# dleeim/Safe-Bayesian-Optimization

Hardware: AMD Instinct MI355X
Metric: candidate-points/sec, SafeOpt posterior+safe-set sweep (higher is better)
Workload: dtype f64

## Files before the change

### include/safebo.h

```cpp
#ifndef SAFEBO_H
#define SAFEBO_H

#include <stdint.h>

#ifdef __cplusplus
extern "C" {
#endif

#define SBO_ABI_VERSION 3
#define SBO_MAX_D 8
#define SBO_MAX_Q 8
#define SBO_MAX_N 2048

enum sbo_status {
  SBO_OK = 0,
  SBO_E_INVALID = -1,
  SBO_E_NOMEM = -2,
  SBO_E_HIP = -3,
  SBO_E_NO_MODEL = -4,
  SBO_E_NO_CANDIDATES = -5,
  SBO_E_EMPTY_SAFE_SET = -6,
  SBO_E_COMM = -7,
  SBO_E_UNSUPPORTED = -8
};
// ... 37 lines not shown
  double  expander_std;
  int32_t choose_minimizer;
  double  u_star;
  double  L[SBO_MAX_Q];
  int64_t count_S, count_U, count_M;
  int64_t count_G[SBO_MAX_Q];
  int64_t n_exact_rechecks;
  int64_t guard_band;
  int64_t guard_rechecks;
  int32_t guard_passes;
  int32_t reserved_g;
} sbo_safeopt_result;

typedef struct sbo_goose_result {
  int64_t safe_min_index;
  double  safe_min_x[SBO_MAX_D];
  double  safe_min_lcb;
  int64_t target_index_c[SBO_MAX_Q];
  double  target_lcb_c[SBO_MAX_Q];
  int32_t target_best_c;
  int64_t target_index;
  double  target_x[SBO_MAX_D];
  double  target_lcb;
  int64_t explore_index;
  double  explore_x[SBO_MAX_D];
  int32_t choose_safe_min;
  double  L[SBO_MAX_Q];
  int64_t count_S, count_U;
  int64_t count_O[SBO_MAX_Q];
  int64_t n_exact_rechecks;
  int64_t guard_band, guard_rechecks;
  int32_t guard_passes, reserved_g;
} sbo_goose_result;

typedef struct sbo_tr_result {
  int64_t index;
  double  x[SBO_MAX_D];
  double  lcb;
  int64_t count_S, count_T;
  int64_t guard_band, guard_rechecks;
  int32_t guard_passes, reserved_g;
} sbo_tr_result;

typedef struct sbo_robust_result {
  int64_t index;
  double  xc[SBO_MAX_D];
  double  value;
  int64_t worst_d_index;
  double  worst_d[SBO_MAX_D];
  int64_t candidate_index;
  int64_t count_control, count_disturbance, count_safe;
  int64_t guard_band, guard_rechecks;
  int32_t guard_passes, reserved_g;
} sbo_robust_result;

typedef struct sbo_profile {
  double posterior_ms;
  double classify_ms;
  double expander_ms;
  double argreduce_ms;
  double comm_ms;
  double total_ms;
  double posterior_flops;
  int64_t candidates;
  int32_t posterior_launches;
  int32_t posterior_kernel;
  double posterior_executed_flops;
  double posterior_setup_ms;
  int64_t fp64_rechecks;
  double recheck_ms;
  double set_phase_ms;
  int32_t host_syncs;
  int32_t comm_calls;
  int64_t comm_bytes;
  double guard_dm[SBO_MAX_Q], guard_dv[SBO_MAX_Q], guard_rl[SBO_MAX_Q];
  double guard_ms;
  int32_t halo_reruns;
  int32_t set_path;
  int64_t guard_audit_samples, guard_audit_violations;
  double guard_audit_worst;
  double guard_analytic_dm[SBO_MAX_Q], guard_analytic_dv[SBO_MAX_Q], guard_probe_dm[SBO_MAX_Q], guard_probe_dv[SBO_MAX_Q];
  int64_t k1_tiles_skipped;
  int64_t k1_tiles_skipped_safe;
  int64_t guard_audit_skipped;
  double list_index_build_ms;
  int64_t list_index_leaf_pairs, list_index_nodes_skipped;
  double fp32_band_dm[SBO_MAX_Q], fp32_band_dv[SBO_MAX_Q];
} sbo_profile;

int sbo_version(void);
const char* sbo_last_error(void);
int sbo_device_count(int* count);
int sbo_init(int device_id, sbo_ctx** out);
int sbo_shutdown(sbo_ctx* ctx);
int sbo_synchronize(sbo_ctx* ctx);

#define SBO_COMM_ID_BYTES 128
int sbo_comm_unique_id(void* id_out );
int sbo_comm_init(sbo_ctx* ctx, int world_size, int rank, const void* id);
int sbo_comm_barrier(sbo_ctx* ctx);
typedef int (*sbo_relay_allreduce_fn)(void* user, void* buf, int64_t count, int elem, int op);
typedef int (*sbo_relay_allgather_fn)(void* user, const void* send, void* recv, int64_t bytes_per_rank);
int sbo_comm_init_relay(sbo_ctx* ctx, int world_size, int rank, sbo_relay_allreduce_fn allreduce,
                        sbo_relay_allgather_fn allgather, void* user);

int sbo_model_set(sbo_ctx* ctx, int dtype, const char* kernel, int n, int d, int q,
                  const double* X_mean, const double* X_std, const double* Y_mean, const double* Y_std,
                  const double* X_norm, const double* Y_norm, const double* hypopt, const double* invK);

int sbo_model_set_list(sbo_ctx* ctx, int dtype, const char* kernel, int n, int d, int q, const double* X_mean,
                       const double* X_std, const double* Y_mean, const double* Y_std, const double* X_norm,
                       const double* Y_norm, const double* hypopt, const double* const* invK_list);

int sbo_model_set_prior(sbo_ctx* ctx, int dtype, const char* kernel, int n, int d, int q, const double* X_mean,
                        const double* X_std, const double* Y_mean, const double* Y_std, const double* X_norm,
                        const double* Y_norm, const double* hypopt, const double* const* invK_list, const double* mean_prior);

int sbo_model_append(sbo_ctx* ctx, const double* x_norm_new, const double* y_norm_new);

#define SBO_MAX_APPEND 64
int sbo_model_append_batch(sbo_ctx* ctx, int k, const double* x_norm_new , const double* y_norm_new );

int sbo_model_remove(sbo_ctx* ctx, int index);

typedef struct sbo_model_loo_result {
  int32_t n, q;
  double  logdet[SBO_MAX_Q];
  double  lpd[SBO_MAX_Q];
  double  z_max[SBO_MAX_Q];
  int32_t z_argmax[SBO_MAX_Q];
  int32_t outside[SBO_MAX_Q];
} sbo_model_loo_result;

int sbo_model_loo(sbo_ctx* ctx, double b, double* resid_out , double* var_out ,
                  sbo_model_loo_result* result );

int sbo_candidates_points(sbo_ctx* ctx, const void* points, int points_dtype, int64_t n_local, int d,
                          int64_t first_index);
int sbo_candidates_grid(sbo_ctx* ctx, int d, const double* lo, const double* hi, const int64_t* count,
                        int64_t first_index, int64_t n_local);

int sbo_candidates_grid_sharded(sbo_ctx* ctx, int d, const double* lo, const double* hi, const int64_t* count,
                                int64_t* first_index_out, int64_t* n_local_out);

int sbo_posterior_run(sbo_ctx* ctx);
int sbo_posterior_get(sbo_ctx* ctx, void* mean_out, void* var_out);
int sbo_bounds(sbo_ctx* ctx, double b, int index, int kind, void* out);
int sbo_sweep_safeopt(sbo_ctx* ctx, const sbo_sweep_opts* opts, sbo_safeopt_result* result);
int sbo_sweep_goose(sbo_ctx* ctx, const sbo_sweep_opts* opts, sbo_goose_result* result);
int sbo_sweep_tr(sbo_ctx* ctx, const sbo_sweep_opts* opts, const double* x_0, double r, sbo_tr_result* result);
int sbo_sweep_robust(sbo_ctx* ctx, const sbo_sweep_opts* opts, int n_control_axes, int kind, sbo_robust_result* result);
int sbo_robust_get(sbo_ctx* ctx, double* f_out, double* g_out);
int sbo_explore_safeset(sbo_ctx* ctx, const double* target, int64_t* index_out, double* x_out);
int sbo_masks_get(sbo_ctx* ctx, int which, int c, uint8_t* out);

int sbo_nll_batch(sbo_ctx* ctx, int n, int d, const double* X_norm, const double* y, int P, const double* hyper,
                  double* out);

int sbo_fit_de(sbo_ctx* ctx, int n, int d, const double* X_norm, const double* y, int P, const double* lo, const double* hi,
               const double* init_pop, uint64_t seed, int maxiter, double tol, double atol, double* best_x, double* best_energy,
               int* generations);

int sbo_nll_grad_batch(sbo_ctx* ctx, int n, int d, const double* X_norm, const double* y, int P, const double* hyper,
                       double* nll_out, double* grad_out);

enum sbo_fit_status {
// ... 263 lines not shown
```

### safe-bayesian-optimization_amd/_lib.py

```python
from __future__ import annotations

import ctypes as C
import os

SBO_MAX_D = 8
SBO_MAX_Q = 8
SBO_MAX_N = 2048
SBO_COMM_ID_BYTES = 128
SBO_ROBUST_MAX_SCEN = 8
SBO_MAX_BATCH = 64
SBO_MAX_APPEND = 64
SBO_EXPANDER_MAX_POINTS = 65536
SBO_EXPANDER_MAX_SCRATCH = 1 << 32
SBO_MAX_PATHS = 64
SBO_MAX_FEATURES = 8192
SBO_PATHS_MAX_POINTS = 1 << 24
SBO_PATHS_MAX_VALUES = 1 << 32
SBO_REFINE_PATHS_MAX_STARTS = 64
SBO_JOINT_MAX_POINTS = 2048

SBO_F64, SBO_F32 = 0, 1
SBO_MEAN, SBO_UCB, SBO_LCB, SBO_VAR = 0, 1, 2, 3
SBO_MASK_S, SBO_MASK_U, SBO_MASK_M, SBO_MASK_G, SBO_MASK_O = 0, 1, 2, 3, 4

# ... 96 lines not shown
    _fields_ = [("output_mask", C.c_uint32), ("top", C.c_int32), ("max_eval", C.c_int32), ("reserved", C.c_int32), ("tol", C.c_double),
                ("lo", C.c_double * SBO_MAX_D), ("hi", C.c_double * SBO_MAX_D)]


class LipschitzResult(C.Structure):
    _fields_ = [("L", C.c_double * SBO_MAX_Q), ("L_seed", C.c_double * SBO_MAX_Q), ("x", (C.c_double * SBO_MAX_D) * SBO_MAX_Q),
                ("axis", C.c_int32 * SBO_MAX_Q), ("sign", C.c_int32 * SBO_MAX_Q), ("seeds_used", C.c_int64), ("evaluations", C.c_int64),
                ("problems", C.c_int32), ("converged", C.c_int32)]


class FitOpts(C.Structure):
    _fields_ = [("P", C.c_int32), ("maxiter", C.c_int32), ("tol", C.c_double), ("atol", C.c_double), ("seed", C.c_uint64),
                ("polish", C.c_int32), ("polish_maxiter", C.c_int32), ("polish_ftol", C.c_double), ("polish_gtol", C.c_double),
                ("lo", C.c_double * (SBO_MAX_D + 2)), ("hi", C.c_double * (SBO_MAX_D + 2))]


class FitReport(C.Structure):
    _fields_ = [("de_nll", C.c_double * SBO_MAX_Q), ("nll", C.c_double * SBO_MAX_Q), ("generations", C.c_int32 * SBO_MAX_Q),
                ("polish_status", C.c_int32 * SBO_MAX_Q), ("polish_evals", C.c_int32 * SBO_MAX_Q), ("polished", C.c_int32 * SBO_MAX_Q),
                ("de_ms", C.c_double), ("polish_ms", C.c_double), ("build_ms", C.c_double), ("total_ms", C.c_double),
                ("host_syncs", C.c_int32), ("reserved", C.c_int32)]


class ModelLooResult(C.Structure):
    _fields_ = [("n", C.c_int32), ("q", C.c_int32), ("logdet", C.c_double * SBO_MAX_Q), ("lpd", C.c_double * SBO_MAX_Q),
                ("z_max", C.c_double * SBO_MAX_Q), ("z_argmax", C.c_int32 * SBO_MAX_Q), ("outside", C.c_int32 * SBO_MAX_Q)]


class BatchOpts(C.Structure):
    _fields_ = [("output", C.c_int32), ("k", C.c_int32), ("n_pending", C.c_int32), ("reserved", C.c_int32), ("min_std", C.c_double)]


class BatchResult(C.Structure):
    _fields_ = [("n_selected", C.c_int32), ("reserved", C.c_int32), ("index", C.c_int64 * SBO_MAX_BATCH),
                ("std", C.c_double * SBO_MAX_BATCH)]


class ExpanderOpts(C.Structure):
    _fields_ = [("b", C.c_double), ("constraint_mask", C.c_uint32), ("reserved", C.c_int32)]


class PathsOpts(C.Structure):
    _fields_ = [("output", C.c_int32), ("n_paths", C.c_int32), ("n_features", C.c_int32), ("maximize", C.c_int32)]


class PathsResult(C.Structure):
    _fields_ = [("index", C.c_int64 * SBO_MAX_PATHS), ("value", C.c_double * SBO_MAX_PATHS)]


class RefinePathsOpts(C.Structure):
    _fields_ = [("b", C.c_double), ("output", C.c_int32), ("n_paths", C.c_int32), ("n_features", C.c_int32), ("n_starts", C.c_int32),
                ("maximize", C.c_int32), ("constraint_mask", C.c_uint32), ("max_eval", C.c_int32), ("reserved", C.c_int32),
                ("lo", C.c_double * SBO_MAX_D), ("hi", C.c_double * SBO_MAX_D), ("tol", C.c_double)]


class RefinePathsResult(C.Structure):
    _fields_ = [("best", C.c_int64 * SBO_MAX_PATHS), ("best_x", (C.c_double * SBO_MAX_D) * SBO_MAX_PATHS),
                ("best_value", C.c_double * SBO_MAX_PATHS), ("evaluations", C.c_int64), ("converged", C.c_int32),
                ("reserved", C.c_int32)]


class JointOpts(C.Structure):
    _fields_ = [("output", C.c_int32), ("n_draws", C.c_int32), ("noise", C.c_int32), ("maximize", C.c_int32), ("jitter", C.c_double)]


class JointResult(C.Structure):
    _fields_ = [("index", C.c_int64 * SBO_MAX_PATHS), ("value", C.c_double * SBO_MAX_PATHS), ("pivot_min", C.c_double),
                ("pivot_row", C.c_int64)]


class Profile(C.Structure):
    _fields_ = [
        ("posterior_ms", C.c_double), ("classify_ms", C.c_double), ("expander_ms", C.c_double),
        ("argreduce_ms", C.c_double), ("comm_ms", C.c_double), ("total_ms", C.c_double),
        ("posterior_flops", C.c_double), ("candidates", C.c_int64), ("posterior_launches", C.c_int32),
        ("posterior_kernel", C.c_int32), ("posterior_executed_flops", C.c_double), ("posterior_setup_ms", C.c_double),
        ("fp64_rechecks", C.c_int64), ("recheck_ms", C.c_double),
        ("set_phase_ms", C.c_double), ("host_syncs", C.c_int32), ("comm_calls", C.c_int32), ("comm_bytes", C.c_int64),
        ("guard_dm", C.c_double * SBO_MAX_Q), ("guard_dv", C.c_double * SBO_MAX_Q), ("guard_rl", C.c_double * SBO_MAX_Q),
        ("guard_ms", C.c_double), ("halo_reruns", C.c_int32), ("set_path", C.c_int32),
        ("guard_audit_samples", C.c_int64), ("guard_audit_violations", C.c_int64), ("guard_audit_worst", C.c_double),
        ("guard_analytic_dm", C.c_double * SBO_MAX_Q), ("guard_analytic_dv", C.c_double * SBO_MAX_Q),
        ("guard_probe_dm", C.c_double * SBO_MAX_Q), ("guard_probe_dv", C.c_double * SBO_MAX_Q),
        ("k1_tiles_skipped", C.c_int64), ("k1_tiles_skipped_safe", C.c_int64), ("guard_audit_skipped", C.c_int64),
        ("list_index_build_ms", C.c_double), ("list_index_leaf_pairs", C.c_int64), ("list_index_nodes_skipped", C.c_int64),
        ("fp32_band_dm", C.c_double * SBO_MAX_Q), ("fp32_band_dv", C.c_double * SBO_MAX_Q),
    ]


RELAY_ALLREDUCE = C.CFUNCTYPE(C.c_int, C.c_void_p, C.c_void_p, C.c_int64, C.c_int, C.c_int)
RELAY_ALLGATHER = C.CFUNCTYPE(C.c_int, C.c_void_p, C.c_void_p, C.c_void_p, C.c_int64)

_P = C.c_void_p
_DP = C.POINTER(C.c_double)
SYMBOLS = [
    ("sbo_version", C.c_int, []),
    ("sbo_last_error", C.c_char_p, []),
    ("sbo_device_count", C.c_int, [C.POINTER(C.c_int)]),
    ("sbo_init", C.c_int, [C.c_int, C.POINTER(_P)]),
    ("sbo_shutdown", C.c_int, [_P]),
    ("sbo_synchronize", C.c_int, [_P]),
    ("sbo_comm_unique_id", C.c_int, [_P]),
    ("sbo_comm_init", C.c_int, [_P, C.c_int, C.c_int, _P]),
    ("sbo_comm_barrier", C.c_int, [_P]),
    ("sbo_comm_init_relay", C.c_int, [_P, C.c_int, C.c_int, RELAY_ALLREDUCE, RELAY_ALLGATHER, _P]),
    ("sbo_model_set", C.c_int, [_P, C.c_int, C.c_char_p, C.c_int, C.c_int, C.c_int, _P, _P, _P, _P, _P, _P, _P, _P]),
    ("sbo_model_set_list", C.c_int, [_P, C.c_int, C.c_char_p, C.c_int, C.c_int, C.c_int, _P, _P, _P, _P, _P, _P, _P, _P]),
    ("sbo_model_set_prior", C.c_int, [_P, C.c_int, C.c_char_p, C.c_int, C.c_int, C.c_int, _P, _P, _P, _P, _P, _P, _P, _P, _P]),
    ("sbo_model_append", C.c_int, [_P, _P, _P]),
    ("sbo_model_append_batch", C.c_int, [_P, C.c_int, _P, _P]),
    ("sbo_model_remove", C.c_int, [_P, C.c_int]),
    ("sbo_model_loo", C.c_int, [_P, C.c_double, _P, _P, C.POINTER(ModelLooResult)]),
    ("sbo_candidates_points", C.c_int, [_P, _P, C.c_int, C.c_int64, C.c_int, C.c_int64]),
    ("sbo_candidates_grid", C.c_int, [_P, C.c_int, _P, _P, _P, C.c_int64, C.c_int64]),
    ("sbo_candidates_grid_sharded", C.c_int, [_P, C.c_int, _P, _P, _P, C.POINTER(C.c_int64), C.POINTER(C.c_int64)]),
    ("sbo_posterior_run", C.c_int, [_P]),
    ("sbo_posterior_get", C.c_int, [_P, _P, _P]),
    ("sbo_bounds", C.c_int, [_P, C.c_double, C.c_int, C.c_int, _P]),
    ("sbo_sweep_safeopt", C.c_int, [_P, C.POINTER(SweepOpts), C.POINTER(SafeOptResult)]),
    ("sbo_sweep_goose", C.c_int, [_P, C.POINTER(SweepOpts), C.POINTER(GooseResult)]),
    ("sbo_sweep_tr", C.c_int, [_P, C.POINTER(SweepOpts), _P, C.c_double, C.POINTER(TRResult)]),
    ("sbo_sweep_robust", C.c_int, [_P, C.POINTER(SweepOpts), C.c_int, C.c_int, C.POINTER(RobustResult)]),
    ("sbo_robust_get", C.c_int, [_P, _P, _P]),
    ("sbo_explore_safeset", C.c_int, [_P, _P, C.POINTER(C.c_int64), _P]),
    ("sbo_masks_get", C.c_int, [_P, C.c_int, C.c_int, _P]),
    ("sbo_nll_batch", C.c_int, [_P, C.c_int, C.c_int, _P, _P, C.c_int, _P, _P]),
    ("sbo_fit_de", C.c_int, [_P, C.c_int, C.c_int, _P, _P, C.c_int, _P, _P, _P, C.c_uint64, C.c_int, C.c_double, C.c_double, _P, _P,
                             C.POINTER(C.c_int)]),
    ("sbo_nll_grad_batch", C.c_int, [_P, C.c_int, C.c_int, _P, _P, C.c_int, _P, _P, _P]),
    ("sbo_fit_local", C.c_int, [_P, C.c_int, C.c_int, C.c_int, _P, _P, C.c_int, _P, _P, _P, C.c_int, C.c_double, C.c_double, _P, _P,
                                _P, _P, _P, _P, _P, _P]),
    ("sbo_fit_de_batch", C.c_int, [_P, C.c_int, C.c_int, C.c_int, _P, _P, C.c_int, _P, _P, _P, _P, C.c_int, C.c_double, C.c_double, _P, _P,
                                   _P]),
    ("sbo_model_fit", C.c_int, [_P, C.c_int, C.c_char_p, C.c_int, C.c_int, C.c_int, _P, _P, _P, _P, _P, _P, _P, C.POINTER(FitOpts), _P, _P,
                                C.POINTER(FitReport)]),
    ("sbo_refine", C.c_int, [_P, C.POINTER(RefineOpts), C.c_int64, _P, _P, _P, _P, C.POINTER(RefineResult)]),
    ("sbo_refine_sets", C.c_int, [_P, C.POINTER(RefineSetsOpts), C.c_int64, _P, _P, _P, _P, _P, _P, C.POINTER(RefineSetsResult)]),
    ("sbo_refine_robust", C.c_int, [_P, C.POINTER(RefineRobustOpts), _P, _P, C.POINTER(RefineRobustResult)]),
    ("sbo_mean_grad", C.c_int, [_P, C.c_int64, _P, _P, _P]),
    ("sbo_lipschitz", C.c_int, [_P, C.POINTER(LipschitzOpts), C.c_int64, _P, C.POINTER(LipschitzResult)]),
    ("sbo_batch_select", C.c_int, [_P, C.POINTER(BatchOpts), C.c_int64, _P, _P, _P, C.POINTER(BatchResult)]),
    ("sbo_expander_gain", C.c_int, [_P, C.POINTER(ExpanderOpts), C.c_int64, _P, C.c_int64, _P, _P, _P, _P]),
    ("sbo_sample_paths", C.c_int, [_P, C.POINTER(PathsOpts), _P, _P, _P, _P, C.c_int64, _P, _P, C.POINTER(PathsResult)]),
    ("sbo_refine_paths", C.c_int, [_P, C.POINTER(RefinePathsOpts), _P, _P, _P, _P, _P, _P, _P, _P, C.POINTER(RefinePathsResult)]),
    ("sbo_posterior_joint", C.c_int, [_P, C.POINTER(JointOpts), C.c_int64, _P, _P, _P, _P, _P, _P, C.POINTER(JointResult)]),
    ("sbo_plant_wo", C.c_int, [_P, C.c_int64, _P, _P]),
    ("sbo_profile_get", C.c_int, [_P, C.POINTER(Profile)]),
    ("sbo_set_option", C.c_int, [_P, C.c_char_p, C.c_int64]),
]


class SafeBOError(RuntimeError):

    def __init__(self, code, msg):
        super().__init__(f"libsafebo error {code}: {msg}")
        self.code = code


class EmptySafeSetError(SafeBOError):
    """S_t is empty on the candidate set (the reference's DE would return an infeasible point)."""


def library_path() -> str:
    return os.path.join(os.path.dirname(os.path.abspath(__file__)), "libsafebo.so")


_lib = None
# ... 32 lines not shown
```

### safe-bayesian-optimization_amd/csrc/api.hip

```cpp
#include <algorithm>
#include <cmath>
#include <cstring>
#include <limits>
#include <memory>
#include <chrono>
#include "internal.hpp"
#include "device_common.hpp"

namespace sbo {

static thread_local std::string g_err;

int fail(int code, const std::string& msg) {
  g_err = msg;
  return code;
}
int hip_fail(hipError_t e, const char* what) {
  g_err = std::string("HIP: ") + hipGetErrorString(e) + " in " + what;
  return SBO_E_HIP;
}
int ensure(DevBuf& b, size_t bytes) {
  if (bytes == 0) bytes = 16;
  if (b.bytes >= bytes) return SBO_OK;
  b.reset();
// ... 170 lines not shown

int sbo_shutdown(sbo_ctx* c) {
  if (!c) return SBO_OK;
  (void)hipSetDevice(c->device);
  guard_audit_harvest(c, true);
  drain_streams(c);
  sbo_comm_destroy_internal(c);
  delete c;
  return SBO_OK;
}

int sbo_synchronize(sbo_ctx* c) {
  if (!c) return fail(SBO_E_INVALID, "ctx is NULL");
  SBO_HIP(hipStreamSynchronize(c->stream));
  if (c->stream2) SBO_HIP(hipStreamSynchronize(c->stream2));
  if (c->stream3) SBO_HIP(hipStreamSynchronize(c->stream3));
  if (c->stream4) SBO_HIP(hipStreamSynchronize(c->stream4));
  if (c->stream_audit) SBO_HIP(hipStreamSynchronize(c->stream_audit));
  return SBO_OK;
}

}

namespace {
enum OptTake {
  kTakeBool,
  kTakeInt,
  kTakeClamp,
  kTakeScaled
};
using Options = sbo_ctx::Options;
struct OptRow {
  const char* name;
  int Options::* ifield;
  double Options::* dfield;
  OptTake take;
  const char* reject;
  int64_t lo, hi;
  int fallback;
  double scale;
  OptEffect effect;
  int (*hook)(sbo_ctx*, int64_t);
};
int hook_halo(sbo_ctx* c, int64_t) { for (auto& g : c->dist.halo_guess) g = -1; return SBO_OK; }
int hook_tensor_guess(sbo_ctx* c, int64_t) { c->tn.bump = 0; return SBO_OK; }
int hook_audit(sbo_ctx* c, int64_t) { guard_audit_harvest(c, true); return SBO_OK; }
int hook_audit_scale(sbo_ctx* c, int64_t) {
  guard_audit_harvest(c, true);
  c->audit.samples = c->audit.violations = c->audit.skipped = 0;
  c->audit.worst = 0.0;
  return SBO_OK;
}
int hook_audit_every(sbo_ctx* c, int64_t) { c->audit.tick = 0; return SBO_OK; }
int hook_selftest(sbo_ctx* c, int64_t value) {
  if (value && !c->dist.comm && !c->dist.relay_allreduce)
    return fail(SBO_E_INVALID, "comm_selftest needs a communicator: call sbo_comm_init(ctx, 1, 0, id) with a unique id first");
  return SBO_OK;
}
#define OPT_BOOL(name, effect, hook) {#name, &Options::name, nullptr, kTakeBool, nullptr, 0, 0, 0, 0.0, effect, hook}
#define OPT_RANGE(name, lo, hi, msg, effect, hook) {#name, &Options::name, nullptr, kTakeInt, msg, lo, hi, 0, 0.0, effect, hook}
#define OPT_CLAMP(name, lo, hi, fallback, effect, hook) {#name, &Options::name, nullptr, kTakeClamp, nullptr, lo, hi, fallback, 0.0, effect, hook}
#define OPT_RAW(name, effect, hook) {#name, &Options::name, nullptr, kTakeInt, nullptr, 0, 0, 0, 0.0, effect, hook}
#define OPT_SCALED(key, field, scale, lo, hi, msg, effect, hook) {key, nullptr, &Options::field, kTakeScaled, msg, lo, hi, 0, scale, effect, hook}
const OptRow kOptions[] = {
    OPT_BOOL(halo_spec, kOptNothing, hook_halo),
    OPT_BOOL(comm_events, kOptNothing, nullptr),
    OPT_SCALED("cheb_tol_e17", cheb_tol, 1e-17, 0, 0, nullptr, kOptPlans, nullptr),
    OPT_RANGE(tensor_guess_pct, 10, 400, "tensor_guess_pct must be within 10 .. 400", kOptTensor, hook_tensor_guess),
    OPT_BOOL(tensor_cheb, kOptTensor, nullptr),
    OPT_CLAMP(exact_lazy, 0, 2, 1, kOptNothing, nullptr),
    OPT_BOOL(chol_async, kOptNothing, nullptr),
    OPT_RANGE(bilinear, 0, 2, "bilinear must be 0 (off), 1 (on; a model's first sweep by node interpolation) or 2 (on, K1b's plan from the first sweep)", kOptPlans, nullptr),
    OPT_BOOL(phase_events, kOptNothing, nullptr),
    OPT_RAW(scan_waves, kOptNothing, nullptr),
    OPT_BOOL(set_lanes, kOptNothing, nullptr),
    OPT_BOOL(result_mirror, kOptNothing, nullptr),
    OPT_BOOL(set_fuse, kOptNothing, nullptr),
    OPT_RANGE(col_path, 0, 2, "col_path must be 0 (never), 1 (auto) or 2 (whenever the grid's shape allows)", kOptNothing, nullptr),
    OPT_RANGE(guard_audit, 0, 1 << 20, "guard_audit: samples per sweep, 0 (off) .. 1048576", kOptNothing, hook_audit),
    OPT_SCALED("guard_audit_scale_ppm", audit_scale, 1e-6, 1, 1000000000, "guard_audit_scale_ppm: 1 .. 1e9", kOptNothing, hook_audit_scale),
    OPT_RANGE(guard_audit_every, 1, 1 << 20, "guard_audit_every: 1 .. 1048576 sweeps", kOptNothing, hook_audit_every),
    OPT_RANGE(grad_defer, 0, 3, "grad_defer must be 0 .. 3", kOptInterp, nullptr),
    OPT_BOOL(k1_sched, kOptNothing, nullptr),
    OPT_BOOL(k1_skip_safe, kOptNothing, nullptr),
    OPT_BOOL(col_overlap, kOptNothing, nullptr),
    OPT_RANGE(col_queue, 64, 128, "col_queue must be within 64 .. 128 (the default)", kOptNothing, nullptr),
    OPT_BOOL(scan_blocks, kOptNothing, nullptr),
    OPT_RANGE(fuse_classify, -1, 1, "fuse_classify must be -1 (auto), 0 or 1", kOptNothing, nullptr),
    OPT_BOOL(goose_pairs, kOptNothing, nullptr),
    OPT_RANGE(guard_band, 0, 2, "guard_band must be 0 (off), 1 (on) or 2 (re-evaluate on every sweep)", kOptPlansBand, nullptr),
    OPT_BOOL(fp64_recheck, kOptNothing, nullptr),
    OPT_BOOL(comm_selftest, kOptNothing, hook_selftest),
    OPT_RANGE(refine_lds, 0, 1, "refine_lds must be 0 (stream M) or 1 (LDS when it fits)", kOptNothing, nullptr),
    OPT_RANGE(lipschitz_lds, 0, 1, "lipschitz_lds must be 0 (stream X_norm and alpha) or 1 (LDS when they fit)", kOptNothing, nullptr),
    OPT_RANGE(list_index, -1, 1, "list_index must be -1 (auto), 0 (never) or 1 (always)", kOptNothing, nullptr),
    OPT_RANGE(posterior_path, 0, 2, "posterior_path must be 0 (auto), 1 (generic) or 2 (generic, chunked)", kOptPosterior, nullptr),
};
#undef OPT_BOOL
#undef OPT_RANGE
#undef OPT_CLAMP
#undef OPT_RAW
#undef OPT_SCALED
}

int sbo_set_option(sbo_ctx* c, const char* key, int64_t value) {
  if (!c || !key) return fail(SBO_E_INVALID, "ctx/key is NULL");
  for (const OptRow& r : kOptions) {
    if (strcmp(key, r.name)) continue;
    const bool inside = value >= r.lo && value <= r.hi;
    if (r.reject && !inside) return fail(SBO_E_INVALID, r.reject);
    if (r.hook) {
      const int rc = r.hook(c, value);
      if (rc) return rc;
    }
    switch (r.take) {
      case kTakeBool: c->opt.*r.ifield = value ? 1 : 0; break;
      case kTakeInt: c->opt.*r.ifield = (int)value; break;
      case kTakeClamp: c->opt.*r.ifield = inside ? (int)value : r.fallback; break;
      case kTakeScaled: c->opt.*r.dfield = (double)value * r.scale; break;
    }
    option_changed(c, r.effect);
    return SBO_OK;
  }
  return fail(SBO_E_INVALID, std::string("unknown option ") + key);
}

extern "C" {

static int model_set_impl(sbo_ctx* c, int dtype, const char* kernel, int n, int d, int q, const double* X_mean,
                          const double* X_std, const double* Y_mean, const double* Y_std, const double* X_norm,
                          const double* Y_norm, const double* hypopt, const double* const* invK, const double* mean_prior = nullptr) {
  if (c) guard_audit_harvest(c, true);
  if (!c) return fail(SBO_E_INVALID, "ctx is NULL");
  if (!kernel || strcmp(kernel, "RBF") != 0)
    return fail(SBO_E_INVALID, std::string("ERROR no kernel with name ") + (kernel ? kernel : "(null)"));
  if (dtype != SBO_F64 && dtype != SBO_F32) return fail(SBO_E_INVALID, "dtype must be SBO_F64 or SBO_F32");
  if (n < 1 || n > SBO_MAX_N) return fail(SBO_E_INVALID, "n out of range [1, SBO_MAX_N]");
  if (d < 1 || d > SBO_MAX_D) return fail(SBO_E_INVALID, "d out of range [1, SBO_MAX_D]");
  if (q < 1 || q > SBO_MAX_Q) return fail(SBO_E_INVALID, "q out of range [1, SBO_MAX_Q]");
  if (!X_mean || !X_std || !Y_mean || !Y_std || !X_norm || !Y_norm || !hypopt)
    return fail(SBO_E_INVALID, "NULL model array");
  SBO_HIP(hipSetDevice(c->device));
  c->has_model = false;
  model_changed(c);
  ModelConst& mc = c->mc;
  memset(&mc, 0, sizeof(mc));
  mc.n = n; mc.d = d; mc.q = q;
  mc.npad = (n + 15) / 16 * 16;
  mc.dpad = d <= 2 ? 2 : (d <= 4 ? 4 : 8);
  mc.factor = invK ? SBO_FACTOR_INVK : SBO_FACTOR_CHOL;
  for (int a = 0; a < kMaxD; ++a) { mc.X_mean[a] = a < d ? X_mean[a] : 0.0; mc.X_std[a] = a < d ? X_std[a] : 1.0; mc.X_rstd[a] = 1.0 / mc.X_std[a]; }
  c->h_Xnorm.assign(X_norm, X_norm + (size_t)n * d);
  c->h_Ynorm.assign(Y_norm, Y_norm + (size_t)n * q);
  const double f32eps = (double)std::numeric_limits<float>::epsilon();
  for (int o = 0; o < q; ++o) {
    mc.Y_mean[o] = Y_mean[o];
    mc.Y_std[o] = Y_std[o];
    mc.mp[o] = (o == 0) ? 0.0 : (-2.0 * Y_mean[o]) / Y_std[o];
    if (mean_prior) mc.mp[o] = mean_prior[o];
    mc.sf2[o] = std::exp(2.0 * hypopt[(size_t)d * q + o]);
    mc.sn2[o] = std::exp(2.0 * hypopt[(size_t)(d + 1) * q + o]) + f32eps;
    for (int a = 0; a < d; ++a) {
      const double ell = std::exp(2.0 * hypopt[(size_t)a * q + o]);
      mc.vinv[o][a] = std::pow(ell, -0.5);
      mc.inv_ell[o][a] = 1.0 / ell;
    }
// ... 435 lines not shown
```

### safe-bayesian-optimization_amd/csrc/bilinear.hip

```cpp
#include <stdio.h>
#include <stdlib.h>
#include <string.h>
#include <algorithm>
#include <chrono>
#include <cmath>
#include <vector>
#include <type_traits>
#include <hip/hip_ext.h>
#include "device_common.hpp"

namespace sbo {

template <int S, int TRI, int OMODE>
__global__ __launch_bounds__(256) void k_bgemm(const double* __restrict__ A, size_t a_stride_o, const double* __restrict__ Bf,
                                               size_t b_stride_o, int KB, int nrb, int ncs, double* __restrict__ out,
                                               size_t out_stride_o, double* __restrict__ out2, long long ld) {
  const int o = blockIdx.z;
  const int lane = threadIdx.x & 63, wave = threadIdx.x >> 6;
  const int rb = blockIdx.y * 4 + wave;
  if (rb >= nrb) return;
  const int cs0 = blockIdx.x * S;
  const double* Ablk = A + (size_t)o * a_stride_o + (TRI ? (size_t)rb * (rb + 1) / 2 : (size_t)rb * KB) * 256;
  const double* Bo = Bf + (size_t)o * b_stride_o;
  const int kend = TRI ? rb + 1 : KB;
// ... 1294 lines not shown
    const double x0 = axis_position(c, a, 0), x1 = axis_position(c, a, c->cs.count[a] - 1);
    ab[2 * a] = std::min(x0, x1);
    ab[2 * a + 1] = std::max(x0, x1);
    if (!(ab[2 * a + 1] > ab[2 * a])) return false;
  }
  return true;
}

int bilinear_basis_enqueue(sbo_ctx* c, hipStream_t st, bool force_big) {
  const ModelConst& mc = c->mc;
  const int n = mc.n, q = mc.q;
  double ab[4];
  c->bl_basis_ok = false;
  if (!basis_intervals(c, ab)) return SBO_OK;
  const BasisLayout L = basis_layout(n, q);
  int rc;
  if ((rc = ensure(c->bl_basis, sizeof(double) * L.total))) return rc;
  double* base = (double*)c->bl_basis.p;
  {
    BlJobs jb;
    memset(&jb, 0, sizeof(jb));
    jb.n = n;
    jb.dpad = mc.dpad;
    for (int o = 0; o < q; ++o)
      for (int a = 0; a < 2; ++a) jb.vinv[2 * o + a] = mc.vinv[o][a];
    for (int a = 0; a < 2; ++a) { jb.a[a] = ab[2 * a]; jb.b[a] = ab[2 * a + 1]; }
    const bool small = !force_big && n <= kBasisResLds / 64;
    const size_t dyn = sizeof(double) * (kBasisQLds + (small ? kBasisResLds : 0));
    DevBuf dbgbuf;
    const bool phases = getenv("SBO_BL_TIMING") != nullptr;
    long long* dbg = phases && ensure(dbgbuf, sizeof(long long) * 81) == SBO_OK ? (long long*)dbgbuf.p : nullptr;
    int* rcjob = (int*)(base + L.rcjob);
    SBO_HIP(hipMemsetAsync(rcjob, 0, sizeof(double) * 5 * q, st));
    hipLaunchKernelGGL(k_bl_degree, dim3((unsigned)((n + 63) / 64), (unsigned)(2 * q)), dim3(256), 0, st, jb, (const double*)c->Xn.p, rcjob);
    hipLaunchKernelGGL(k_bl_coef, dim3((unsigned)((n + kCoefRows - 1) / kCoefRows), (unsigned)(2 * q)), dim3(256), 0, st, jb,
                       (const double*)c->Xn.p, (const int*)rcjob, base + L.work, L.work_stride, base + L.eps);
    for (int rep = 0; rep < (dbg ? 2 : 1); ++rep) {
      long long* dg = rep ? dbg : nullptr;
      if (rep)
        hipLaunchKernelGGL(k_bl_coef, dim3((unsigned)((n + kCoefRows - 1) / kCoefRows), (unsigned)(2 * q)), dim3(256), 0, st, jb,
                           (const double*)c->Xn.p, (const int*)rcjob, base + L.work, L.work_stride, base + L.eps);
      if (small) {
        SBO_HIP(hipFuncSetAttribute(reinterpret_cast<const void*>(k_bl_basis<256, true>), hipFuncAttributeMaxDynamicSharedMemorySize, (int)dyn));
        hipLaunchKernelGGL((k_bl_basis<256, true>), dim3((unsigned)(2 * q)), dim3(256), dyn, st, jb, (const double*)c->Xn.p, base + L.work,
                           L.work_stride, base + L.U, base + L.Vs, base + L.sig, (int*)(base + L.info), dg, (const int*)rcjob, 0, base + L.eps);
      } else {
        SBO_HIP(hipFuncSetAttribute(reinterpret_cast<const void*>(k_bl_basis<1024, false>), hipFuncAttributeMaxDynamicSharedMemorySize, (int)dyn));
        hipLaunchKernelGGL((k_bl_basis<1024, false>), dim3((unsigned)(2 * q)), dim3(1024), dyn, st, jb, (const double*)c->Xn.p, base + L.work,
                           L.work_stride, base + L.U, base + L.Vs, base + L.sig, (int*)(base + L.info), dg, (const int*)rcjob, 0, base + L.eps);
      }
    }
    SBO_HIP(hipGetLastError());
    if (dbg) {
      long long h[81];
      if (hipMemcpyAsync(h, dbg, sizeof(h), hipMemcpyDeviceToHost, st) == hipSuccess && hipStreamSynchronize(st) == hipSuccess) {
        fprintf(stderr, "[k_bl_basis] job 0 phases (us):");
        for (int i = 1; i < (int)h[80]; ++i) fprintf(stderr, " %.1f", (double)(h[i] - h[i - 1]) / 100.0);
        fprintf(stderr, "\n");
      }
    }
  }
  SBO_HIP(hipMemcpyAsync(c->h_back->basis_info, base + L.info, sizeof(int) * 8 * q, hipMemcpyDeviceToHost, st));
  for (int t = 0; t < 4; ++t) c->bl_basis_ab[t] = ab[t];
  c->bl_basis_serial = c->model_serial;
  c->bl_basis_ok = true;
  return SBO_OK;
}

static bool basis_current(const sbo_ctx* c) {
  double ab[4];
  if (!c->bl_basis_ok || c->bl_basis_serial != c->model_serial || !basis_intervals(c, ab)) return false;
  for (int t = 0; t < 4; ++t)
    if (ab[t] != c->bl_basis_ab[t]) return false;
  return true;
}

int bilinear_setup(sbo_ctx* c) {
  BilinearPlan& pl = c->bl;
  pl.valid = true;
  pl.usable = false;
  pl.ops = GemmOps();
  GemmOps& g = pl.ops;
  pl.encl_ready = false;
  pl.bt_ready = false;
  pl.setup_ms = 0.0;
  const auto t_begin = std::chrono::steady_clock::now();
  const bool timing = getenv("SBO_BL_TIMING") != nullptr;
  auto lap = [&](const char* what) {
    if (timing) fprintf(stderr, "[K1b setup] %-12s %8.2f ms\n", what,
                        std::chrono::duration<double, std::milli>(std::chrono::steady_clock::now() - t_begin).count());
  };
  const ModelConst& mc = c->mc;
  const CandSpec& cs = c->cs;
  const int n = mc.n, q = mc.q;
  const long long cnt0 = cs.count[0], nlines = cs.n_local / cnt0, line0 = cs.first / cnt0;
  int rc;
  if (!basis_current(c)) {
    if ((rc = bilinear_basis_enqueue(c, c->stream, false))) return rc;
    if (!c->bl_basis_ok) return SBO_OK;
    SBO_HIP(hipStreamSynchronize(c->stream));
  }
  const int* inf = c->h_back->basis_info;
  for (int t = 0; t < 2 * q; ++t)
    if (inf[4 * t] == 2) {
      if ((rc = bilinear_basis_enqueue(c, c->stream, true))) return rc;
      SBO_HIP(hipStreamSynchronize(c->stream));
      break;
    }
  lap("bases");
  BlDims dm;
  memset(&dm, 0, sizeof(dm));
  int r0u = 0, r1u = 0, K0 = 0, K1 = 0, Rmax = 0, rc0m = 0, rc1m = 0;
  for (int o = 0; o < q; ++o) {
    if (inf[8 * o] != 1 || inf[8 * o + 4] != 1) return SBO_OK;
    dm.r0[o] = inf[8 * o + 1]; dm.rc0[o] = inf[8 * o + 2];
    dm.r1[o] = inf[8 * o + 5]; dm.rc1[o] = inf[8 * o + 6];
    if (dm.r0[o] < 1 || dm.r0[o] > kBlMaxR || dm.r1[o] < 1 || dm.r1[o] > kBlMaxR) return SBO_OK;
    r0u = std::max(r0u, dm.r0[o]);
    r1u = std::max(r1u, dm.r1[o]);
    K0 = std::max(K0, pair_count(dm.r0[o]));
    K1 = std::max(K1, pair_count(dm.r1[o]));
    Rmax = std::max(Rmax, dm.r0[o] * dm.r1[o]);
    rc0m = std::max(rc0m, dm.rc0[o]);
    rc1m = std::max(rc1m, dm.rc1[o]);
    dm.sf2[o] = mc.sf2[o];
    pl.r0[o] = dm.r0[o];
    pl.r1[o] = dm.r1[o];
    if (timing) fprintf(stderr, "[K1b setup] output %d: r0 %d (degree %d), r1 %d (degree %d)\n", o, dm.r0[o], dm.rc0[o], dm.r1[o], dm.rc1[o]);
  }
  const int K0m = K0, K1m = K1;
  K0 = 2 * rc0m - 1;
  K1 = 2 * rc1m - 1;
  const int KB0 = (K0 + 15) / 16, KB1 = (K1 + 15) / 16;
  const int ncs0 = (int)((cnt0 + 15) / 16), nrb = (int)((nlines + 15) / 16);
  {
    const double gemm = (double)nlines * KB0 * 16.0 * KB1 * 16.0 + (double)cs.n_local * (KB0 * 16.0 + 3.0 * r0u);
    const double tri = 0.5 * (double)mc.npad * (mc.npad + 16.0) * (double)cs.n_local;
    if (gemm > 0.7 * tri) return SBO_OK;
  }
  const long long nlines_pad = (long long)nrb * 16;
  pl.r0u = r0u; pl.nlines_pad = nlines_pad;
  g.KB0 = KB0; g.KB1 = KB1; g.ncs0 = ncs0; g.nrb = nrb;
  g.sP0f = g.sP1A = 0;
  const size_t nP0f = (size_t)ncs0 * KB0 * 4 * 64, nP1A = (size_t)nrb * KB1 * 256;
  g.sT4f = (size_t)KB0 * KB1 * 4 * 64;
  g.sBtA = g.sBt1 = (size_t)nrb * KB0 * 256;
  const int r0p = (r0u + 3) / 4 * 4;
  const int KBm = (r0p + 15) / 16, KBm2 = (2 * r0p + 15) / 16;
  g.KBm = KBm; g.KBm2 = KBm2; g.KSm = r0p / 4; g.KS0 = KB0 * 4;
  g.sVA = (size_t)nrb * (2 * KBm + KBm2) * 256;
  g.sSBf = (size_t)ncs0 * (KBm + KBm2) * 256;
  if ((rc = ensure(c->bl_P0f, sizeof(double) * nP0f))) return rc;
  if ((rc = ensure(c->bl_P1A, sizeof(double) * nP1A))) return rc;
  const size_t D0m = (size_t)KB0 * 16, D1m = (size_t)KB1 * 16;
  const int KBp0 = (K0m + 15) / 16, KBp1 = (K1m + 15) / 16;
  const size_t nPC0 = D0m * (size_t)KBp0 * 16, nPC1 = D1m * (size_t)KBp1 * 16, nT4p = (size_t)KBp0 * KBp1 * 256, nYt = D1m * (size_t)KBp0 * 16,
               nCh = D0m * D1m;
  if ((rc = ensure(c->bl_cheb, sizeof(double) * (size_t)q * (nPC0 + nPC1 + nT4p + nYt + nCh) + 256))) return rc;
  if ((rc = ensure(c->bl_T4f, sizeof(double) * g.sT4f * q))) return rc;
  if ((rc = ensure(c->bl_SBf, sizeof(double) * g.sSBf * q))) return rc;
  if ((rc = ensure(c->bl_VA, sizeof(double) * g.sVA * q))) return rc;
  if ((rc = ensure(c->bl_BtA, sizeof(double) * g.sBtA * q))) return rc;
  g.BtA = (double*)c->bl_BtA.p; g.P0f = (double*)c->bl_P0f.p; g.VA = (double*)c->bl_VA.p; g.SBf = (double*)c->bl_SBf.p;
  const int KBn = mc.npad / 16, ncsR = (Rmax + 15) / 16;
  const size_t nZf = (size_t)ncsR * KBn * 256;
  const size_t ldg = (size_t)ncsR * 16;
// ... 167 lines not shown
```

### safe-bayesian-optimization_amd/csrc/bilinear_post.inc.hpp

```cpp


constexpr int kFuseRow = 4 + 2 * kMaxQ;
constexpr int kFuseVmin = 4, kFuseRmax = 4 + kMaxQ;
struct PostCtx {
  double* lds;
  int tid, lane, wave, rb0, cs0, nrb, ncs;
  int st_rb, st_cs, st_off, a_lo, b_st, a_rd;
  unsigned int ucnt0;
  long long nlines;
  bool full;
  bool imode;
  const double* var_rd;
  uint8_t *S, *U;
  double bconf, bb;
  int cS, cU;
  double rmax;
  LcbBand lband;
  bool gb_on;
  double vminS;
  int cB;
  int role;
  unsigned int bw[8];
  unsigned int* lds_bits;
  double umin;
// ... 398 lines not shown
      rb0v = *reinterpret_cast<const d4_t*>(Bp + (size_t)(kb + 1) * 256);
      rb1v = *reinterpret_cast<const d4_t*>(Bp + (size_t)(kb + 1) * 256 + 4);
    }
    constexpr int BUF = RB == 2 ? 4096 : 3072, BOFF = RB == 2 ? 2048 : 1024;
    const double* LA = lds + cur * BUF + (RB * cx.wave) * 256 + cx.a_rd;
    const double* LB = lds + cur * BUF + BOFF + cx.lane;
    const int kkn = KS - kb * 4 < 4 ? KS - kb * 4 : 4;
    d4_t fa[2][RB];
    double fb[2][8];
    auto ld = [&](int kk, d4_t (&a)[RB], double (&b)[8]) {
#pragma unroll
      for (int i = 0; i < RB; ++i) {
        const d2_t l = *reinterpret_cast<const d2_t*>(LA + i * 256 + kk * 64), h = *reinterpret_cast<const d2_t*>(LA + i * 256 + kk * 64 + 32);
        a[i] = d4_t{l[0], l[1], h[0], h[1]};
      }
#pragma unroll
      for (int s2 = 0; s2 < 8; ++s2) b[s2] = LB[(s2 * 4 + kk) * 64];
    };
    auto mm = [&](const d4_t (&a)[RB], const double (&b)[8]) {
#pragma unroll
      for (int s2 = 0; s2 < 8; ++s2)
#pragma unroll
        for (int i = 0; i < RB; ++i) acc[i][s2] = MM<double>::mfma(a[i], b[s2], acc[i][s2]);
    };
    if constexpr (RB == 2) {
      ld(0, fa[0], fb[0]);
      int kk = 0;
#pragma unroll 1
      for (; kk + 1 < kkn; kk += 2) {
        ld(kk + 1, fa[1], fb[1]);
        mm(fa[0], fb[0]);
        if (kk + 2 < kkn) ld(kk + 2, fa[0], fb[0]);
        mm(fa[1], fb[1]);
      }
      if (kk < kkn) mm(fa[0], fb[0]);
    } else {
#pragma unroll 1
      for (int kk = 0; kk < kkn; ++kk) {
        ld(kk, fa[0], fb[0]);
        mm(fa[0], fb[0]);
      }
    }
    if (kb + 1 < nkb) stage(lds + (cur ^ 1) * BUF, ra0, ra1, rb0v, rb1v);
    __syncthreads();
  }
  if (RB == 2 && An) {
    const double* Apn = An + (size_t)cx.st_rb * KBn * 256 + cx.st_off;
    const double* Bpn = Bn + (size_t)cx.st_cs * KBn * 256 + cx.st_off;
    if (stage_a) { ra0 = *reinterpret_cast<const d4_t*>(Apn); ra1 = *reinterpret_cast<const d4_t*>(Apn + 4); }
    rb0v = *reinterpret_cast<const d4_t*>(Bpn);
    rb1v = *reinterpret_cast<const d4_t*>(Bpn + 4);
  }
  post_epilogue<PH, RB, ROLE>(cx, outp, c0, c1, c2, gmax, acc);
}

#ifdef SBO_PHASE_CLOCKS
constexpr int kPhaseClkRows = 1 << 14;
__device__ unsigned long long g_phase_clk[kPhaseClkRows][8];
constexpr int kWgTraceRows = 1 << 13;
__device__ unsigned long long g_wg_trace[2][kWgTraceRows][8];
__device__ __forceinline__ void wg_trace_row(int o, unsigned long long t0, unsigned long long t1, unsigned long long t2, unsigned int tile, unsigned int kind) {
  unsigned int hw, xcc;
  asm volatile("s_getreg_b32 %0, hwreg(HW_REG_HW_ID)" : "=s"(hw));
  asm volatile("s_getreg_b32 %0, hwreg(HW_REG_XCC_ID)" : "=s"(xcc));
  unsigned long long* r = g_wg_trace[o & 1][(blockIdx.y * gridDim.x + blockIdx.x) & (kWgTraceRows - 1)];
  r[0] = t0; r[1] = t1; r[2] = t2;
  r[3] = (unsigned long long)(tile & 0xffffffu) | ((unsigned long long)kind << 24) | (1ull << 31);
  r[4] = hw; r[5] = xcc;
}
#define SBO_CLK(i)                                                                                \
  do {                                                                                           \
    __syncthreads();                                                                             \
    if (threadIdx.x == 0) {                                                                      \
      const unsigned long long now_ = wall_clock64();                                            \
      g_phase_clk[clk_row_ & (kPhaseClkRows - 1)][i] += now_ - clk_;                             \
      clk_ = now_;                                                                               \
    }                                                                                            \
  } while (0)
#else
#define SBO_CLK(i) do { } while (0)
#endif

__global__ __launch_bounds__(128) void k_bl_enclose(const double* __restrict__ mean, const double* __restrict__ var, long long cnt0,
                                                    double* __restrict__ encl) {
  const int cell = threadIdx.x, cr = cell >> 4, cc = cell & 15;
  const size_t tile = (size_t)blockIdx.y * gridDim.x + blockIdx.x;
  const size_t base = ((size_t)blockIdx.y * 64 + (size_t)cr * 8) * (size_t)cnt0 + (size_t)blockIdx.x * 128 + (size_t)cc * 8;
  double mlo = 1e308, mhi = -1e308, vlo = 1e308, vhi = -1e308;
  bool fin = true;
  for (int r = 0; r < 8; ++r) {
#pragma unroll
    for (int k = 0; k < 8; ++k) {
      const double m = mean[base + (size_t)r * cnt0 + k], v = var[base + (size_t)r * cnt0 + k];
      fin = fin && fabs(m) <= 1e308 && fabs(v) <= 1e308;
      mlo = fmin(mlo, m); mhi = fmax(mhi, m); vlo = fmin(vlo, v); vhi = fmax(vhi, v);
    }
  }
  const double nan = __longlong_as_double(0x7ff8000000000000ll);
  double4 e = fin ? double4{mlo, mhi, vlo, vhi} : double4{nan, nan, nan, nan};
  reinterpret_cast<double4*>(encl)[tile * 128 + cell] = e;
}

constexpr int kSchedWaves = 8;
__global__ __launch_bounds__(64 * kSchedWaves) void k_bl_sched_tiles1(const ModelConst mc, const double* __restrict__ encl, int ntiles, int tgx, int tgy,
                                                         unsigned int cnt0, double bconf, const GuardBand* __restrict__ gb,
                                                         const double* __restrict__ gtmax, const unsigned long long* __restrict__ gkey, int q,
                                                         uint8_t* __restrict__ skip, unsigned int* __restrict__ list, int cap, unsigned long long* __restrict__ Sw,
                                                         unsigned long long* __restrict__ Uw, unsigned long long* __restrict__ Usum,
                                                         unsigned long long* __restrict__ slots, double* __restrict__ Lpart,
                                                         unsigned long long* __restrict__ cpart, int pcap, int skip_safe ) {
  __shared__ unsigned long long sh_key[kSchedWaves];
  __shared__ unsigned int sh_cnt[kSchedWaves];
  __shared__ unsigned long long sh_vmin[kSchedWaves], sh_rmax[kSchedWaves];
  const int lane = threadIdx.x & 63, wave = (int)(threadIdx.x >> 6), tile = (int)blockIdx.x * kSchedWaves + wave;
  unsigned long long my_key = 0ull, my_vmin = ~0ull, my_rmax = 0ull;
  unsigned int my_cnt = 0u;
  if (tile < ntiles) {
    const double bb = bconf * bconf;
    const bool gb_on = gb != nullptr;
    const LcbBand lb = gb_on ? lcb_band(bb, gb->dm[1], gb->dv[1]) : LcbBand{0.0, 0.0};
    bool ok = true, oks = skip_safe != 0;
    double kv = 1e300, ku = -1.0, kl = 1e300;
#pragma unroll
    for (int h = 0; h < 2; ++h) {
      const double4 e = reinterpret_cast<const double4*>(encl)[(size_t)tile * 128 + h * 64 + lane];
      ok = ok && encl_unsafe(e.x, e.y, e.z, e.w, bconf, bb, gb_on, lb);
      oks = oks && encl_safe(e.x, e.y, e.z, e.w, bconf, bb, gb_on, lb);
      if (oks) {
        const EnclKeys ek = encl_keys(e.x, e.y, e.z, e.w, bconf);
        kv = ek.vlo < kv ? ek.vlo : kv;
        ku = ek.up > ku ? ek.up : ku;
        kl = ek.lo < kl ? ek.lo : kl;
      }
    }
    const bool dec = __ballot(!ok) == 0ull;
    const bool sdec = !dec && __ballot(!oks) == 0ull;
    bool run2 = true, run3 = true;
    double gfold = 0.0;
    if (gtmax) {
      const size_t nt = (size_t)ntiles;
      const double* slack = gtmax + (size_t)q * 2 * nt;
      const double ystd = mc.Y_std[1];
      const double cg0 = ystd * mc.inv_ell[1][0] * mc.X_rstd[0], cg1 = ystd * mc.inv_ell[1][1] * mc.X_rstd[1];
      const double t0 = gtmax[(size_t)2 * nt + tile], t1 = gtmax[(size_t)3 * nt + tile];
      const double G0 = __longlong_as_double((long long)gkey[2]), G1 = __longlong_as_double((long long)gkey[3]);
      run2 = !(t0 + slack[2] < G0 * (1.0 - 1e-12));
      run3 = !(t1 + slack[3] < G1 * (1.0 - 1e-12));
      gfold = fmax(fabs(cg0 * t0), fabs(cg1 * t1));
    }
    const bool grad = run2 || run3;
    const unsigned int k = dec ? (grad ? 2u : 0u) : (sdec ? (grad ? 5u : 4u) : (grad ? 1u : 3u));
    if (lane == 0) skip[tile] = dec ? kSkipUnsafe : (sdec ? kSkipSafe : 0);
    my_cnt = k == 0u ? 3u : (k == 2u ? 2u : (k == 4u ? 12u : (k == 5u ? 8u : 0u)));
    if (k != 0u && k != 4u) {
      if (lane == 0) {
        const unsigned int sh = ((unsigned int)tile + 3u * ((unsigned int)tile >> kTlistShift)) & (kTlistShards - 1);
        const unsigned int p = atomicAdd(&list[sh * kTlistHead + (k == 3u ? 1 : 0)], 1u);
        if (p < (unsigned int)cap)
          list[kTlistShards * kTlistHead + sh * cap + (k == 3u ? (unsigned int)(cap - 1) - p : p)] =
              (unsigned int)tile | (k == 2u ? kTlistUnsafe : (k == 5u ? kTlistSafe : 0u));
      }
    } else if (k == 4u) {
#pragma unroll
      for (int off = 32; off > 0; off >>= 1) {
        const double ov = __shfl_xor(kv, off), ou = __shfl_xor(ku, off), ol = __shfl_xor(kl, off);
        kv = ov < kv ? ov : kv;
        ku = ou > ku ? ou : ku;
        kl = ol < kl ? ol : kl;
      }
      const int bx = tile % tgx, by = tile / tgx;
      const size_t w0 = (size_t)by * cnt0 + (size_t)bx * 128;
#pragma unroll
      for (int h = 0; h < 2; ++h) {
        Sw[w0 + h * 64 + lane] = ~0ull;
        Uw[w0 + h * 64 + lane] = 0ull;
      }
      const double lrow = fmax(0.0, gfold);
      my_key = (unsigned long long)__double_as_longlong(lrow);
      my_vmin = kv < 1e300 ? ord_key(kv) : ~0ull;
      my_rmax = ku >= 0.0 ? ord_key(ku) : 0ull;
      if (lane == 0) {
        Lpart[((size_t)tgy + by) * tgx + bx] = lrow;
        atomicOr(&slots[(size_t)kSlotRowMask * kColSlots + by], 1ull << bx);
      }
      if (lane < kFuseRow) {
        unsigned long long v = 0ull;
        if (lane == 0) v = kl < 1e300 ? ord_key(kl) : ~0ull;
        else if (lane == 1) v = 64ull * 128ull;
        else if (lane >= kFuseVmin && lane < kFuseRmax) v = lane == kFuseVmin + 1 ? my_vmin : ~0ull;
        else if (lane == kFuseRmax + 1) v = my_rmax;
        cpart[(size_t)lane * pcap + tile] = v;
      }
    } else {
      const int bx = tile % tgx, by = tile / tgx;
      const size_t w0 = (size_t)by * cnt0 + (size_t)bx * 128;
#pragma unroll
      for (int h = 0; h < 2; ++h) {
        Sw[w0 + h * 64 + lane] = 0ull;
        Uw[w0 + h * 64 + lane] = ~0ull;
        atomicOr(&Usum[(size_t)bx * 128 + h * 64 + lane], 1ull << by);
      }
      const double lrow = fmax(0.0, gfold);
      my_key = (unsigned long long)__double_as_longlong(lrow);
      if (lane == 0) Lpart[((size_t)tgy + by) * tgx + bx] = lrow;
      if (lane < kFuseRow) {
        unsigned long long v = 0ull;
        if (lane == 0) v = ~0ull;
        else if (lane == 2) v = 64ull * 128ull;
        else if (lane >= kFuseVmin && lane < kFuseRmax) v = ~0ull;
        cpart[(size_t)lane * pcap + tile] = v;
      }
    }
  }
  if (lane == 0) { sh_key[wave] = my_key; sh_cnt[wave] = my_cnt; sh_vmin[wave] = my_vmin; sh_rmax[wave] = my_rmax; }
  __syncthreads();
  if (threadIdx.x < 7) {
    unsigned long long key = 0ull, n0 = 0ull, nskip = 0ull, n4 = 0ull, nsafe = 0ull, vmin = ~0ull, rmax = 0ull;
#pragma unroll
    for (int w = 0; w < kSchedWaves; ++w) {
      key = sh_key[w] > key ? sh_key[w] : key;
      n0 += sh_cnt[w] & 1u;
      nskip += (sh_cnt[w] >> 1) & 1u;
      n4 += (sh_cnt[w] >> 2) & 1u;
      nsafe += (sh_cnt[w] >> 3) & 1u;
      vmin = sh_vmin[w] < vmin ? sh_vmin[w] : vmin;
      rmax = sh_rmax[w] > rmax ? sh_rmax[w] : rmax;
    }
    const int slot = (int)(blockIdx.x & (kColSlots - 1));
    if (threadIdx.x == 0 && n0) atomicAdd(&slots[(size_t)kSlotU * kColSlots + slot], 64ull * 128ull * n0);
    if (threadIdx.x == 1 && (n0 || n4)) atomicMax(&slots[(size_t)kSlotL1 * kColSlots + slot], key);
    if (threadIdx.x == 2 && nskip) atomicAdd(&slots[(size_t)kSlotSkip * kColSlots + slot], nskip);
    if (threadIdx.x == 3 && n4) atomicAdd(&slots[(size_t)kSlotS * kColSlots + slot], 64ull * 128ull * n4);
    if (threadIdx.x == 4 && nsafe) atomicAdd(&slots[(size_t)kSlotSkipSafe * kColSlots + slot], nsafe);
    if (threadIdx.x == 5 && vmin != ~0ull) atomicMin(&slots[(size_t)kSlotVmin1 * kColSlots + slot], vmin);
    if (threadIdx.x == 6 && rmax != 0ull) atomicMax(&slots[(size_t)kSlotRmax1 * kColSlots + slot], rmax);
  }
}

__device__ __forceinline__ unsigned int sched_rank3(int k, unsigned int (&base)[3], unsigned int* __restrict__ sh ) {
  const int lane = threadIdx.x & 63, wave = threadIdx.x >> 6;
  const unsigned long long below = (1ull << lane) - 1ull;
  unsigned int rank = 0u;
#pragma unroll
  for (int j = 0; j < 3; ++j) {
    const unsigned long long m = __ballot(k == j);
    if (k == j) rank = (unsigned int)__popcll(m & below);
    if (lane == 0) sh[j * 16 + wave] = (unsigned int)__popcll(m);
  }
  __syncthreads();
  unsigned int pos = 0u, tot[3] = {0u, 0u, 0u};
#pragma unroll
  for (int j = 0; j < 3; ++j)
    for (int w = 0; w < 16; ++w) {
      const unsigned int c = sh[j * 16 + w];
      if (k == j && w < wave) pos += c;
      tot[j] += c;
    }
  __syncthreads();
  const unsigned int r = k >= 0 ? base[k] + pos + rank : 0u;
#pragma unroll
  for (int j = 0; j < 3; ++j) base[j] += tot[j];
  return r;
}

__global__ __launch_bounds__(1024) void k_bl_sched_list2(unsigned long long* __restrict__ cpart, int pcap, int ntiles, unsigned int* __restrict__ list,
                                                         double* __restrict__ Lpart0, unsigned int* __restrict__ head1) {
  __shared__ unsigned int sh[3 * 16];
  const int t = threadIdx.x;
  const unsigned long long* nS = cpart + (size_t)1 * pcap;
  unsigned long long* orow = cpart + ntiles;
  unsigned int base[3] = {0u, 0u, 0u};
  for (int r = 0; r * 1024 < ntiles; ++r) {
    const int i = r * 1024 + t;
    const bool in = i < ntiles, has = in && nS[i] != 0ull;
    const unsigned int p = sched_rank3(has ? 0 : -1, base, sh);
    if (has) {
      list[kTlistHead + p] = (unsigned int)i;
    } else if (in) {
      Lpart0[i] = 0.0;
#pragma unroll
      for (int lane = 0; lane < kFuseRow; ++lane)
        orow[(size_t)lane * pcap + i] = (lane <= 1 || (lane >= kFuseVmin && lane < kFuseRmax)) ? ~0ull : 0ull;
    }
  }
  if (t == 0) {
    list[0] = base[0];
    list[1] = 0u;
  }
  if (t < kTlistShards) head1[t * kTlistHead] = head1[t * kTlistHead + 1] = 0u;
}

template <int RB, int ROLE = 0 >
__global__ __launch_bounds__(256, (RB == 2 ? 2 : 3)) void k_bpost(const ModelConst mc, const CandSpec cs, const double* __restrict__ BtA, size_t sBtA,
                                                  const double* __restrict__ P0f, size_t sP0f, const double* __restrict__ VA,
                                                  size_t sVA, const double* __restrict__ SBf, size_t sSBf, int KB0, int KS0, int KBm,
                                                  int KSm, int KBm2, int nrb, int ncs, long long nlines, double* __restrict__ mean_out,
                                                  double* __restrict__ var_out, double* __restrict__ Lpart,
                                                  const double* __restrict__ xn0, uint8_t* __restrict__ Sfuse, uint8_t* __restrict__ Ufuse,
                                                  double bconf, unsigned long long* __restrict__ cpart ,
                                                  int pcap,
                                                  const GuardBand* __restrict__ gb ,
                                                  const int* __restrict__ eff ,
                                                  const double* __restrict__ gtmax ,
                                                  const unsigned long long* __restrict__ gkey ,
                                                  int imode ,
                                                  const PostExtra px ) {
  extern __shared__ double lds[];
  const int o = px.o0 + (int)blockIdx.z;
  const bool listed = ROLE != 0 && px.tlist != nullptr;
  unsigned int ent = 0u;
  if (listed) {
    const unsigned int sh = blockIdx.x & ((1u << px.tshift) - 1u), at = blockIdx.x >> px.tshift;
    const unsigned int nfront = px.tlist[sh * kTlistHead], nback = px.tlist[sh * kTlistHead + 1];
    if (at >= nfront + nback) {
#ifdef SBO_PHASE_CLOCKS
      if (threadIdx.x == 0) { const unsigned long long t_ = wall_clock64(); wg_trace_row(o, t_, t_, t_, 0xffffffu, 3u); }
#endif
      return;
    }
    ent = px.tlist[(kTlistHead << px.tshift) + sh * (unsigned int)px.tcap + (at < nfront ? at : (unsigned int)px.tcap - 1u - (at - nfront))];
  }
  const unsigned int tgx = listed ? (unsigned int)px.tgx : gridDim.x, tgy = listed ? (unsigned int)px.tgy : gridDim.y;
  const unsigned int bx = listed ? (ent & 0xffffffu) % tgx : blockIdx.x, by = listed ? (ent & 0xffffffu) / tgx : blockIdx.y;
  PostCtx cx;
  cx.lds = lds;
  cx.tid = threadIdx.x; cx.lane = cx.tid & 63; cx.wave = cx.tid >> 6;
  cx.rb0 = by * (4 * RB); cx.cs0 = bx * 8; cx.nrb = nrb; cx.ncs = ncs;
  cx.ucnt0 = (unsigned int)cs.count[0];
  cx.nlines = nlines;
  cx.full = (long long)(cx.rb0 + 4 * RB) * 16 <= nlines && (long long)(cx.cs0 + 8) * 16 <= cs.count[0];
  cx.imode = imode != 0;
  const int st_i = cx.tid >> 5, st_j = cx.tid & 31;
  cx.st_off = st_j * 8;
  cx.st_rb = cx.rb0 + st_i < nrb ? cx.rb0 + st_i : nrb - 1;
  cx.st_cs = cx.cs0 + st_i < ncs ? cx.cs0 + st_i : ncs - 1;
  cx.a_lo = st_i < 4 * RB ? st_i * 256 + (st_j >> 3) * 64 + (st_j & 7) * 4 : -1;
  cx.b_st = (RB == 2 ? 2048 : 1024) + st_i * 256 + cx.st_off;
  cx.a_rd = (((cx.lane >> 4) << 2) + (cx.lane & 3)) * 2;
  const double* VAo = VA + (size_t)o * sVA;
  const double* SBo = SBf + (size_t)o * sSBf;
  const double sf2 = mc.sf2[o], ystd = mc.Y_std[o];
  double* const vo = var_out + (size_t)o * cs.n_local;
  double* const mo = mean_out + (size_t)o * cs.n_local;
  const bool fuse = Sfuse != nullptr && o >= 1;
  const bool fmulti = px.fstride != 0;
  cx.var_rd = vo;
  cx.S = fuse ? Sfuse + (size_t)(o - 1) * (size_t)px.fstride : nullptr;
  cx.U = fuse ? Ufuse + (size_t)(o - 1) * (size_t)px.fstride : Ufuse;
  cx.bconf = bconf;
  cx.bb = bconf * bconf;
  cx.cS = cx.cU = cx.cB = 0;
  cx.rmax = -1.0;
  const bool cbits = RB == 1 && ROLE == 1 && px.cb.Sw != nullptr && o == 1, obits = RB == 1 && ROLE == 2 && px.cb.Sw != nullptr && o == 0;
  const size_t ctile = (size_t)by * tgx + bx, ntile = (size_t)tgx * tgy;
  const unsigned long long tile_nS = obits ? cpart[(size_t)1 * pcap + ctile] : 0ull;
  cx.role = cbits ? 1 : ((obits && tile_nS != 0ull) ? 2 : 0);
  cx.skip_store = obits && tile_nS == 0ull && px.lean != 0;
  cx.lds_bits = reinterpret_cast<unsigned int*>(lds + 2 * (RB == 2 ? 4096 : 3072));
  cx.umin = 1e300;
  cx.xmin = 1e300;
#pragma unroll
  for (int s2 = 0; s2 < 8; ++s2) cx.bw[s2] = 0u;
  cx.gb_on = (fuse || cbits) && gb != nullptr;
  cx.lband = cx.gb_on ? lcb_band(cx.bb, gb->dm[o >= 1 ? o : 1], gb->dv[o >= 1 ? o : 1]) : LcbBand{0.0, 0.0};
  cx.vminS = 1e300;
  double gmax = 0.0;
  d4_t acc[RB][8];
  d4_t pre[4];
  const double* const A2 = VAo + (size_t)nrb * KBm * 256;
  const double* const B2 = imode ? SBo : SBo + (size_t)ncs * KBm * 256;
  const double* const A3 = VAo + (size_t)nrb * (KBm + KBm2) * 256;
  const int es = imode ? 4 : 1;
  const int KS1 = imode ? eff[4 * (4 * o + 1)] : KSm, KS2 = imode ? eff[4 * (4 * o + 2)] : KSm, KS3 = imode ? eff[4 * (4 * o + 3)] : KSm;
#ifdef SBO_PHASE_CLOCKS
  unsigned long long clk_ = wall_clock64();
  const unsigned long long clk_in_ = clk_;
  unsigned long long clk_part_ = clk_;
  const unsigned int clk_row_ = ((unsigned int)o * tgy + by) * tgx + bx;
#endif
  const double cg0 = ystd * mc.inv_ell[o][0] * mc.X_rstd[0], cg1 = ystd * mc.inv_ell[o][1] * mc.X_rstd[1];
  bool run2 = true, run3 = true;
  double gfold = 0.0;
  if (gtmax) {
    const size_t nt = ntile, tile = ctile;
    const double* slack = gtmax + (size_t)px.q * 2 * nt;
    const double t0 = gtmax[((size_t)o * 2 + 0) * nt + tile], t1 = gtmax[((size_t)o * 2 + 1) * nt + tile];
    const double G0 = __longlong_as_double((long long)gkey[2 * o + 0]), G1 = __longlong_as_double((long long)gkey[2 * o + 1]);
    run2 = !(t0 + slack[2 * o + 0] < G0 * (1.0 - 1e-12));
    run3 = !(t1 + slack[2 * o + 1] < G1 * (1.0 - 1e-12));
    const double f0 = fabs(cg0 * t0), f1 = fabs(cg1 * t1);
    gfold = fmax(f0, f1);
  }
  if (px.nograd) { run2 = run3 = false; gfold = 0.0; }
  if (ROLE == 2 && px.lean) { run2 = run3 = false; gfold = 0.0; }
  bool cskip = false, csafe = false;
  if (ROLE == 1 && cbits && px.lean >= 2 && px.encl != nullptr) {
    if (listed) {
      cskip = (ent & kTlistUnsafe) != 0u;
      csafe = (ent & kTlistSafe) != 0u;
    } else {
      bool dec = true, sdec = px.skip_safe != 0;
      if (cx.tid < 128) {
        const double4 e = reinterpret_cast<const double4*>(px.encl)[ctile * 128 + cx.tid];
        dec = encl_unsafe(e.x, e.y, e.z, e.w, cx.bconf, cx.bb, cx.gb_on, cx.lband);
        sdec = sdec && encl_safe(e.x, e.y, e.z, e.w, cx.bconf, cx.bb, cx.gb_on, cx.lband);
      }
      cskip = __syncthreads_and(dec ? 1 : 0) != 0;
      csafe = __syncthreads_and(sdec ? 1 : 0) != 0 && !cskip;
      if (cx.tid == 0) px.skip[ctile] = cskip ? kSkipUnsafe : (csafe ? kSkipSafe : 0);
      if (cskip && cx.tid == 0) atomicAdd(&px.cb.slots[(size_t)kSlotSkip * kColSlots + (ctile & (kColSlots - 1))], 1ull);
      if (csafe && cx.tid == 0) atomicAdd(&px.cb.slots[(size_t)kSlotSkipSafe * kColSlots + (ctile & (kColSlots - 1))], 1ull);
    }
    if (cskip) {
      cx.role = 0;
      cx.skip_store = true;
      cx.cU = 64 * 128 / 256;
      for (int i = cx.tid; i < 4 * 128; i += 256) cx.lds_bits[i] = 0xffff0000u;
    }
    if (csafe) {
      cx.role = 0;
      cx.skip_store = true;
      cx.cS = 64 * 128 / 256;
      for (int i = cx.tid; i < 4 * 128; i += 256) cx.lds_bits[i] = 0x0000ffffu;
      if (cx.tid < 128) {
        const double4 e = reinterpret_cast<const double4*>(px.encl)[ctile * 128 + cx.tid];
        const EnclKeys ek = encl_keys(e.x, e.y, e.z, e.w, cx.bconf);
        cx.vminS = ek.vlo;
        cx.rmax = ek.up;
        cx.xmin = ek.lo;
      }
    }
  }
  const bool skip_tile = (ROLE == 2 && obits && tile_nS == 0ull && px.lean >= 2) || cskip || csafe;
  if (!skip_tile)
    post_phase<0, RB, ROLE>(cx, BtA + (size_t)o * sBtA, P0f + (size_t)o * sP0f, KB0, eff ? eff[4 * o * es] : KS0, vo, sf2, ystd * ystd, 0.0, gmax, acc, xn0, pre,
                            VAo, SBo, KBm);
  SBO_CLK(0);
  if (ROLE == 2 && cx.role == 2) {
#pragma unroll
    for (int s2 = 0; s2 < 8; ++s2) {
      const unsigned long long w = px.cb.Sw[(size_t)by * cx.ucnt0 + (unsigned int)(cx.cs0 + s2) * 16u + (cx.lane & 15)];
      cx.bw[s2] = (unsigned int)(w >> (16 * cx.wave + (cx.lane >> 4))) & 0x1111u;
    }
  }
  if (!skip_tile || (run2 && !imode))
    post_phase<1, RB, ROLE>(cx, VAo, SBo, KBm, KS1, mo, mc.mp[o], ystd, mc.Y_mean[o], gmax, acc, xn0, pre, run2 ? A2 : A3, run2 ? B2 : SBo,
                            run2 ? KBm2 : KBm);
  SBO_CLK(1);
  if (run2) post_phase<2, RB, ROLE>(cx, A2, B2, KBm2, KS2, nullptr, cg0, 0.0, 0.0, gmax, acc, xn0, pre, A3, SBo, KBm);
  if (run3) post_phase<3, RB, ROLE>(cx, A3, SBo, KBm, KS3, nullptr, cg1, 0.0, 0.0, gmax, acc, xn0, pre, nullptr, nullptr, 0);
  gmax = fmax(gmax, gfold);
  SBO_CLK(2);
#ifdef SBO_PHASE_CLOCKS
  clk_part_ = clk_;
#endif
#pragma unroll
  for (int off = 32; off > 0; off >>= 1) {
    const double other = __shfl_xor(gmax, off);
    gmax = other > gmax ? other : gmax;
  }
  post_partials<4>(cx.lds, cx.lane, cx.wave, gmax, fuse || cbits, cx.cS, cx.cU, obits ? -cx.umin : cx.rmax, cx.cB, cx.vminS,
                   Lpart + ((size_t)o * tgy + by) * tgx + bx,
                   cpart + (obits ? ntile : (fmulti && o >= 1 ? (size_t)(o - 1) * ntile : (size_t)0)) + ctile, pcap, obits,
                   (cbits || obits) ? px.cb.slots : nullptr, (int)(ctile & (kColSlots - 1)), o, cbits ? (int)by : -1, (int)bx, cx.xmin, fmulti);
  if (cbits && cx.tid < 128) {
    unsigned long long sw = 0ull, uw = 0ull;
#pragma unroll
    for (int w = 0; w < 4; ++w) {
      const unsigned int pc = cx.lds_bits[w * 128 + cx.tid];
      sw |= (unsigned long long)(pc & 0xffffu) << (16 * w);
      uw |= (unsigned long long)(pc >> 16) << (16 * w);
    }
    const size_t col = (size_t)cx.cs0 * 16u + cx.tid;
    px.cb.Sw[(size_t)by * cx.ucnt0 + col] = sw;
    px.cb.Uw[(size_t)by * cx.ucnt0 + col] = uw;
    if (uw != 0ull) atomicOr(&px.cb.Usum[col], 1ull << by);
  }
  SBO_CLK(3);
#ifdef SBO_PHASE_CLOCKS
  if (threadIdx.x == 0) {
    g_phase_clk[clk_row_ & (kPhaseClkRows - 1)][4] += (unsigned long long)((run2 ? 1 : 0) + (run3 ? 1 : 0));
    g_phase_clk[clk_row_ & (kPhaseClkRows - 1)][5] += 1ull;
    if (ROLE != 0)
      wg_trace_row(o, clk_in_, clk_part_, clk_, (unsigned int)ctile, skip_tile ? ((!(cskip || csafe) || !(run2 || run3)) ? 1u : 2u) : 0u);
  }
#endif
}
#ifdef SBO_PHASE_CLOCKS
extern "C" int sbo_debug_phase_clocks(unsigned long long* out , int reset, int split) {
  std::vector<unsigned long long> h((size_t)kPhaseClkRows * 8);
  if (hipMemcpyFromSymbol(h.data(), HIP_SYMBOL(g_phase_clk), sizeof(unsigned long long) * h.size()) != hipSuccess) return 1;
  for (int k = 0; k < 16; ++k) out[k] = 0;
  for (size_t r = 0; r < (size_t)kPhaseClkRows; ++r)
    for (int k = 0; k < 8; ++k) out[(r < (size_t)split ? 0 : 8) + k] += h[r * 8 + k];
  if (reset) {
    std::fill(h.begin(), h.end(), 0ull);
    if (hipMemcpyToSymbol(HIP_SYMBOL(g_phase_clk), h.data(), sizeof(unsigned long long) * h.size()) != hipSuccess) return 1;
  }
  return 0;
}
extern "C" int sbo_debug_wg_trace(unsigned long long* out , int rows, int reset) {
  if (rows != kWgTraceRows) return 2;
  const size_t bytes = sizeof(unsigned long long) * 2 * kWgTraceRows * 8;
  if (hipDeviceSynchronize() != hipSuccess || hipMemcpyFromSymbol(out, HIP_SYMBOL(g_wg_trace), bytes) != hipSuccess) return 1;
  if (reset) {
    std::vector<unsigned long long> z(bytes / sizeof(unsigned long long), 0ull);
    if (hipMemcpyToSymbol(HIP_SYMBOL(g_wg_trace), z.data(), bytes) != hipSuccess) return 1;
  }
  return 0;
}
#endif


__global__ __launch_bounds__(256, 3) void k_bgrad(const ModelConst mc, const CandSpec cs, const double* __restrict__ VA, size_t sVA,
                                                  const double* __restrict__ P0f, int KB, int nrb, int ncs, long long nlines, int gx, int gy,
                                                  const int* __restrict__ eff, const double* __restrict__ gtmax,
                                                  const unsigned long long* __restrict__ gkey, const double* __restrict__ xn0, int q,
                                                  double* __restrict__ Lpart, unsigned long long* __restrict__ slots,
                                                  int o_first ) {
  extern __shared__ double lds[];
  PostCtx cx;
  cx.lds = lds;
  cx.tid = threadIdx.x; cx.lane = cx.tid & 63; cx.wave = cx.tid >> 6;
  cx.nrb = nrb; cx.ncs = ncs;
  cx.ucnt0 = (unsigned int)cs.count[0];
  cx.nlines = nlines;
  cx.imode = true;
  const int st_i = cx.tid >> 5, st_j = cx.tid & 31;
  cx.st_off = st_j * 8;
  cx.a_lo = st_i < 4 ? st_i * 256 + (st_j >> 3) * 64 + (st_j & 7) * 4 : -1;
  cx.b_st = 1024 + st_i * 256 + cx.st_off;
  cx.a_rd = (((cx.lane >> 4) << 2) + (cx.lane & 3)) * 2;
  cx.var_rd = nullptr; cx.S = nullptr; cx.U = nullptr;
  cx.bconf = 0.0; cx.bb = 0.0; cx.cS = cx.cU = cx.cB = 0; cx.rmax = -1.0;
  cx.lband = LcbBand{0.0, 0.0}; cx.gb_on = false; cx.vminS = 1e300;
  cx.role = 0; cx.lds_bits = nullptr; cx.umin = 1e300; cx.xmin = 1e300; cx.skip_store = false;
#pragma unroll
  for (int s2 = 0; s2 < 8; ++s2) cx.bw[s2] = 0u;
  const size_t nt = (size_t)gx * gy;
  const double* slack = gtmax ? gtmax + (size_t)q * 2 * nt : nullptr;
  d4_t acc[1][8];
  d4_t pre[4];
  for (size_t tile = blockIdx.x; o_first > 0 && tile < nt; tile += gridDim.x)
    if (cx.tid == 0) Lpart[tile] = 0.0;
  for (int o = o_first; o < q; ++o) {
    const double ystd = mc.Y_std[o];
    const double cg0 = ystd * mc.inv_ell[o][0] * mc.X_rstd[0], cg1 = ystd * mc.inv_ell[o][1] * mc.X_rstd[1];
    const double G0 = gtmax ? __longlong_as_double((long long)gkey[2 * o + 0]) : 0.0, G1 = gtmax ? __longlong_as_double((long long)gkey[2 * o + 1]) : 0.0;
    const double s0 = gtmax ? slack[2 * o + 0] : 0.0, s1 = gtmax ? slack[2 * o + 1] : 0.0;
    const int KS2 = eff[4 * (4 * o + 2)], KS3 = eff[4 * (4 * o + 3)];
    const double* VAo = VA + (size_t)o * sVA;
    const double* A2 = VAo + (size_t)nrb * KB * 256;
    const double* A3 = VAo + (size_t)nrb * (2 * KB) * 256;
    double wg_max = 0.0;
    for (size_t tile = blockIdx.x; tile < nt; tile += gridDim.x) {
      const double t0 = gtmax ? gtmax[((size_t)o * 2 + 0) * nt + tile] : 0.0, t1 = gtmax ? gtmax[((size_t)o * 2 + 1) * nt + tile] : 0.0;
      const bool run2 = !(t0 + s0 < G0 * (1.0 - 1e-12)), run3 = !(t1 + s1 < G1 * (1.0 - 1e-12));
      double g = fmax(fabs(cg0 * t0), fabs(cg1 * t1));
      if (run2 || run3) {
        const int bx = (int)(tile % (size_t)gx), by = (int)(tile / (size_t)gx);
        cx.rb0 = by * 4; cx.cs0 = bx * 8;
        cx.full = (long long)(cx.rb0 + 4) * 16 <= nlines && (long long)(cx.cs0 + 8) * 16 <= cs.count[0];
        cx.st_rb = cx.rb0 + st_i < nrb ? cx.rb0 + st_i : nrb - 1;
        cx.st_cs = cx.cs0 + st_i < ncs ? cx.cs0 + st_i : ncs - 1;
        double gmax = 0.0;
        if (run2) post_phase<2, 1, 0>(cx, A2, P0f, KB, KS2, nullptr, cg0, 0.0, 0.0, gmax, acc, xn0, pre, nullptr, nullptr, 0);
        if (run3) post_phase<3, 1, 0>(cx, A3, P0f, KB, KS3, nullptr, cg1, 0.0, 0.0, gmax, acc, xn0, pre, nullptr, nullptr, 0);
#pragma unroll
        for (int off = 32; off > 0; off >>= 1) {
          const double other = __shfl_xor(gmax, off);
          gmax = other > gmax ? other : gmax;
        }
        __syncthreads();
        if (cx.lane == 0) lds[cx.wave] = gmax;
        __syncthreads();
        gmax = fmax(fmax(lds[0], lds[1]), fmax(lds[2], lds[3]));
        __syncthreads();
        g = fmax(g, gmax);
      }
      if (cx.tid == 0) Lpart[(size_t)o * nt + tile] = g;
      wg_max = fmax(wg_max, g);
    }
    if (slots && cx.tid == 0)
      atomicMax(&slots[(size_t)(o == 0 ? kSlotL0 : kSlotL1) * kColSlots + (blockIdx.x & (kColSlots - 1))], (unsigned long long)__double_as_longlong(wg_max));
  }
}

__global__ __launch_bounds__(256) void k_lmax_reduce(const double* __restrict__ Lpart, int per_out, unsigned long long* __restrict__ Lmax) {
  __shared__ double sh[4];
  lmax_reduce_body((int)blockIdx.x, sh, Lpart, per_out, Lmax);
}

static bool col_words_ok(const sbo_ctx* c, const PostRequest& req, long long cnt0, long long nlines) {
  if (!req.col || !c->opt.col_path) return false;
  const bool shape = c->mc.q == 2 && c->cs.kind == 1 && c->cs.d == 2 && c->cs.first == 0 && cnt0 % 128 == 0 && nlines % 64 == 0 &&
                     nlines / 64 <= 64 && nlines >= 64 && cnt0 >= 128 && cnt0 <= 4096 && c->dist.world == 1 && !c->opt.comm_selftest;
  const long long tiles = (cnt0 / 128) * (nlines / 64);
  return shape && (c->opt.col_path == 2 || tiles >= 4ll * c->n_cu);
}
static_assert(kFuseRmax + 1 == kColRowRmax1, "ColPartRows::tumax is the radius key of constraint 1");

struct GemmLaunch {
  sbo_ctx* c;
  bool interp;
  const PostRequest& req;
  PostOutcome& out;
  const GemmOps& g;
  int q;
  long long cnt0, nlines;
  bool defer;
  bool run_stage1;
  unsigned gx = 0, gy = 0, rows_out = 0;
  size_t lds = 0, ntiles = 0;
  bool fuse = false, colw = false;
  PostExtra px;
  double* encl = nullptr;
  bool record_encl = false;
  unsigned int *sched_l1 = nullptr, *sched_l2 = nullptr;
  int sched_cap1 = 0;
  const GuardBand* gb_fused = nullptr;
  double* lrows = nullptr;
};

static void gemm_stage1(const GemmLaunch& L) {
  constexpr int S1 = 3;
  sbo_ctx* c = L.c;
  const GemmOps& g = L.g;
  const dim3 grid((unsigned)((g.KB0 + S1 - 1) / S1), (unsigned)((g.nrb + 3) / 4), (unsigned)(g.sets * L.q));
  if (L.defer)
    hipExtLaunchKernelGGL((k_bstage1<S1>), grid, dim3(256), 0, c->stream, nullptr, c->ev_grad[1], 0, (const double*)c->bl_P1A.p, g.sP1A,
                          (const double*)c->bl_T4f.p, g.sT4f, g.KB1, g.nrb, g.KB0, g.BtA, g.sBt1, (const int*)g.eff);
  else
    hipLaunchKernelGGL((k_bstage1<S1>), grid, dim3(256), 0, c->stream, (const double*)c->bl_P1A.p, g.sP1A, (const double*)c->bl_T4f.p,
                       g.sT4f, g.KB1, g.nrb, g.KB0, g.BtA, g.sBt1, (const int*)g.eff);
}

static int gemm_shape(GemmLaunch& L) {
  L.gx = (unsigned)((L.g.ncs0 + 7) / 8);
  L.gy = (unsigned)((L.g.nrb + 3) / 4);
  L.rows_out = L.gx * L.gy;
  L.ntiles = (size_t)L.gx * L.gy;
  L.lds = sizeof(double) * 2 * 3072 + 2048;
  return ensure(L.c->bl_lpart, sizeof(double) * (size_t)L.rows_out * L.q * (L.interp ? 2 : 1));
}

static int gemm_classify_plan(GemmLaunch& L) {
  sbo_ctx* c = L.c;
  const CandSpec& cs = c->cs;
  const int q = L.q;
  const bool fuse_wanted = L.req.fuse == 1 || (L.req.fuse == 2 && ((long long)L.gx * L.gy * q >= 4ll * c->n_cu || q > 2));
  L.fuse = fuse_wanted && q >= 2 && c->maskS.p && c->maskU.p && c->maskS.bytes >= (size_t)cs.n_local && c->maskU.bytes >= (size_t)cs.n_local &&
           (q == 2 || (c->fuseS.bytes >= (size_t)cs.n_local * (q - 1) && c->fuseU.bytes >= (size_t)cs.n_local * (q - 1)));
  L.colw = L.fuse && col_words_ok(c, L.req, L.cnt0, L.nlines);
  memset(&L.px, 0, sizeof(L.px));
  L.px.q = q;
  if (!L.fuse) return SBO_OK;
  L.out.fuse_rows = (int)L.rows_out * (L.colw ? 2 : (q - 1));
  L.px.fstride = q > 2 ? (long long)cs.n_local : 0ll;
  if (int rc = ensure(c->cpart, sizeof(unsigned long long) * kFuseRow * ((size_t)L.out.fuse_rows + 4 * (size_t)c->n_cu + 64))) return rc;
  c->cpart_cap = (int)(c->cpart.bytes / (sizeof(unsigned long long) * kFuseRow));
  if (L.colw) L.out.col_rows = ColPartRows{(unsigned long long*)c->cpart.p, c->cpart_cap, (int)L.rows_out};
  return SBO_OK;
}

static int col_words_prepare(sbo_ctx* c, long long cnt0, long long nlines, ColBits* cb) {
  const size_t words = (size_t)(nlines / 64) * (size_t)cnt0;
  int rc;
  if ((rc = ensure(c->col.S, 8 * words)) || (rc = ensure(c->col.U, 8 * words)) || (rc = ensure(c->col.M, 8 * words)) || (rc = ensure(c->col.G, 8 * words))) return rc;
  DevBuf& usum = c->col.Usum.buf;
  if ((rc = c->col.Usum.acquire(8 * (size_t)cnt0, [&]() -> int {
        SBO_HIP(hipMemsetAsync(usum.p, 0, usum.bytes, c->stream));
        return SBO_OK;
      })))
    return rc;
  const size_t sbytes = sizeof(unsigned long long) * kColSlotFields * kColSlots;
  if ((rc = c->col.slots.acquire(sbytes, [&]() -> int {
        unsigned long long init[kColSlotFields * kColSlots];
        for (int f = 0; f < kColSlotFields; ++f)
          for (int k = 0; k < kColSlots; ++k) init[f * kColSlots + k] = col_slot_is_min(f) ? ~0ull : 0ull;
        SBO_HIP(hipMemcpyAsync(c->col.slots.buf.p, init, sbytes, hipMemcpyHostToDevice, c->stream));
        SBO_HIP(hipStreamSynchronize(c->stream));
        return SBO_OK;
      })))
    return rc;
  cb->Sw = (unsigned long long*)c->col.S.p;
  cb->Uw = (unsigned long long*)c->col.U.p;
  cb->Usum = (unsigned long long*)usum.p;
  cb->slots = (unsigned long long*)c->col.slots.buf.p;
  return SBO_OK;
}

static int col_enclosures(GemmLaunch& L) {
  sbo_ctx* c = L.c;
  const size_t ebytes = sizeof(double) * 4 * 128 * L.ntiles;
  const void* was = c->bl_encl.p;
  if (int rc = ensure(c->bl_encl, ebytes + L.ntiles)) return rc;
  if (c->bl_encl.p != was) c->bl.encl_ready = false;
  L.encl = (double*)c->bl_encl.p;
  L.record_encl = !c->bl.encl_ready;
  c->k1_audit.encl_tiles = L.ntiles;
  c->k1_audit.encl_check = !L.record_encl;
  if (!L.record_encl && L.req.col_lean >= 2) {
    L.px.encl = L.encl;
    L.px.skip = (uint8_t*)c->bl_encl.p + ebytes;
    L.px.skip_safe = (c->opt.k1_skip_safe && c->bl.vals_ready) ? 1 : 0;
    c->k1_audit.skip_armed = true;
  }
  return SBO_OK;
}

static int col_tile_lists(GemmLaunch& L) {
  sbo_ctx* c = L.c;
  if (L.interp || !c->opt.k1_sched || L.req.col_lean < 2) {
    c->bl_sched.in_use();
    return SBO_OK;
  }
  L.sched_cap1 = (int)((L.ntiles + kTlistShards - 1) / kTlistShards);
  const size_t words1 = (size_t)kTlistShards * (kTlistHead + (size_t)L.sched_cap1);
  if (int rc = c->bl_sched.acquire(sizeof(unsigned int) * (words1 + kTlistHead + L.ntiles), [&]() -> int {
        if (L.px.encl) SBO_HIP(hipMemsetAsync(c->bl_sched.buf.p, 0, sizeof(unsigned int) * kTlistShards * kTlistHead, c->stream));
        return SBO_OK;
      }))
    return rc;
  L.sched_l1 = (unsigned int*)c->bl_sched.buf.p;
  L.sched_l2 = L.sched_l1 + words1;
  return SBO_OK;
}

static int gemm_grad_deferred(GemmLaunch& L) {
  sbo_ctx* c = L.c;
  const GemmOps& g = L.g;
  hipStream_t gs = c->stream3;
  SBO_HIP(hipStreamWaitEvent(gs, c->ev_grad[1], 0));
  SBO_HIP(hipFuncSetAttribute(reinterpret_cast<const void*>(k_bgrad), hipFuncAttributeMaxDynamicSharedMemorySize, (int)L.lds));
  hipLaunchKernelGGL(k_bgrad, dim3((unsigned)std::min<long long>((long long)L.rows_out, 2ll * c->n_cu)), dim3(256), L.lds, gs, c->mc, c->cs, g.VA,
                     g.sVA, g.P0f, g.KB0, g.nrb, g.ncs0, L.nlines, (int)L.gx, (int)L.gy, (const int*)g.eff, g.gtmax, g.gkey,
                     (const double*)c->bl_small.p, L.q, L.lrows, L.colw ? L.px.cb.slots : (unsigned long long*)nullptr, (L.req.sweep_lean && L.q >= 2) ? 1 : 0);
  SBO_HIP(hipEventRecord(c->ev_grad[2], gs));
  c->grad_pending = true;
  L.px.nograd = 1;
  return SBO_OK;
}

static void gemm_post_part(GemmLaunch& L, int part) {
  sbo_ctx* c = L.c;
  const GemmOps& g = L.g;
  const CandSpec& cs = c->cs;
  const bool colw = L.colw, fuse = L.fuse;
  const int q = L.q;
  const ColPartRows& rows = L.out.col_rows;
  PostExtra& px = L.px;
  px.o0 = colw ? 1 - part : 0;
  const bool last = !colw || part == 1;
  const decltype(&k_bpost<1, 0>) kposts[3] = {k_bpost<1, 0>, k_bpost<1, 1>, k_bpost<1, 2>};
  const auto kpost = kposts[colw ? 1 + part : 0];
  px.tlist = nullptr;
  if (L.sched_l1 && part == 0 && px.encl) {
    hipLaunchKernelGGL(k_bl_sched_tiles1, dim3((L.gx * L.gy + kSchedWaves - 1) / kSchedWaves), dim3(64 * kSchedWaves), 0, c->stream, c->mc, (const double*)px.encl, (int)(L.gx * L.gy), (int)L.gx,
                       (int)L.gy, (unsigned int)L.cnt0, L.req.fuse_b, L.gb_fused, g.gtmax, g.gkey, q, px.skip, L.sched_l1, L.sched_cap1, px.cb.Sw, px.cb.Uw,
                       px.cb.Usum, px.cb.slots, L.lrows, rows.base, rows.cap, px.skip_safe);
    px.tlist = L.sched_l1;
    px.tshift = kTlistShift;
    px.tcap = L.sched_cap1;
  }
  if (L.sched_l2 && part == 1) {
    hipLaunchKernelGGL(k_bl_sched_list2, dim3(1), dim3(1024), 0, c->stream, rows.base, rows.cap, (int)(L.gx * L.gy), L.sched_l2,
                       L.lrows, L.sched_l1);
    px.tlist = L.sched_l2;
    px.tshift = 0;
    px.tcap = (int)(L.gx * L.gy);
    L.out.col_sched = true;
  }
  px.tgx = (int)L.gx;
  px.tgy = (int)L.gy;
  const dim3 grid = px.tlist ? dim3((unsigned)px.tcap << px.tshift) : dim3(L.gx, L.gy, (unsigned)(colw ? 1 : q));
  hipExtLaunchKernelGGL(kpost, grid, dim3(256), L.lds, c->stream, nullptr,
                        (L.req.lmax_defer && last) ? c->ev[1] : ((colw && part == 0) ? c->col.ev[0] : nullptr), 0,
                        c->mc, cs, g.BtA, g.sBtA, g.P0f, g.sP0f, g.VA, g.sVA, g.SBf, g.sSBf, g.KB0, g.KS0, g.KBm, g.KSm, g.KBm2, g.nrb, g.ncs0,
                        L.nlines, (double*)c->mean.p, (double*)c->var.p, L.defer ? L.lrows + (size_t)L.rows_out * q : L.lrows,
                        (const double*)c->bl_small.p , fuse ? (uint8_t*)(q > 2 ? c->fuseS.p : c->maskS.p) : (uint8_t*)nullptr,
                        fuse ? (uint8_t*)(q > 2 ? c->fuseU.p : c->maskU.p) : (uint8_t*)nullptr, L.req.fuse_b, (unsigned long long*)c->cpart.p,
                        c->cpart_cap, L.gb_fused, (const int*)g.eff, g.gtmax, g.gkey, g.imode, px);
  if (colw && part == 0 && L.record_encl) {
    hipLaunchKernelGGL(k_bl_enclose, dim3(L.gx, L.gy), dim3(128), 0, c->stream, (const double*)c->mean.p + (size_t)cs.n_local,
                       (const double*)c->var.p + (size_t)cs.n_local, L.cnt0, L.encl);
    c->bl.encl_ready = true;
  }
  if (colw && part == 0 && !L.interp && c->bl.encl_ready && !px.encl) c->bl.vals_ready = true;
}

static void gemm_flops(const GemmLaunch& L) {
  sbo_ctx* c = L.c;
  const GemmOps& g = L.g;
  const int q = L.q;
  const double tiles2 = (double)g.nrb * g.ncs0;
  if (L.interp) {
    c->last_k1_flops = (double)q * 2.0 * 1024.0 * 4.0 * (4.0 * (double)g.nrb * g.KB0 * g.KB0 + tiles2 * g.KB0 * 4);
    return;
  }
  const double s1 = L.run_stage1 ? 1.0 : 0.0;
  c->last_k1_flops = (double)q * 2.0 * 1024.0 * (s1 * 4.0 * (double)g.nrb * g.KB0 * g.KB1 + tiles2 * (g.KS0 + 3 * g.KSm));
  const int* he = c->h_back->tile_eff;
  double f = 0.0;
  for (int o = 0; o < q; ++o) {
    const int ks = he[4 * o], kb0 = he[4 * o + 1], kb1 = he[4 * o + 2];
    if (ks < 1 || ks > g.KS0 || kb0 < 1 || kb0 > g.KB0 || kb1 < 1 || kb1 > g.KB1) return;
    f += 2.0 * 1024.0 * (s1 * 4.0 * (double)g.nrb * kb0 * kb1 + tiles2 * (ks + (g.gtmax ? 1 : 3) * g.KSm));
  }
  c->last_k1_flops = f;
}

int launch_posterior_gemm(sbo_ctx* c, bool interp, const PostRequest& req, PostOutcome& out) {
  GemmLaunch L{c, interp, req, out, interp ? c->bi.ops : c->bl.ops, c->mc.q, c->cs.count[0], c->cs.n_local / c->cs.count[0]};
  const GemmOps& g = L.g;
  if (interp) c->bi.used = true;
  L.defer = interp && c->bi.grad_deferred && c->stream3 != nullptr;
  L.run_stage1 = interp || !c->bl.bt_ready;
  if (interp) c->bl.bt_ready = false;
  if (!interp && L.run_stage1) {
    gemm_stage1(L);
    c->bl.bt_ready = true;
  }
  int rc;
  if ((rc = gemm_shape(L)) || (rc = gemm_classify_plan(L))) return rc;
  if (L.colw) {
    if ((rc = col_words_prepare(c, L.cnt0, L.nlines, &L.px.cb))) return rc;
    L.px.lean = req.col_lean;
    out.col_active = true;
    out.col_forked = true;
    out.col_lean = req.col_lean;
    L.fuse = false;
    if (!interp && (rc = col_enclosures(L))) return rc;
    if ((rc = col_tile_lists(L))) return rc;
  }
  if (!interp && !L.colw) post_regions_written(c);
  if (interp) gemm_stage1(L);
  if (L.defer && g.band_ready) SBO_HIP(hipStreamWaitEvent(c->stream, c->ev_grad[3], 0));
  L.gb_fused = (c->opt.guard_band && !c->is_shadow && g.band_ready && c->gb.buf.p) ? (const GuardBand*)c->gb.buf.p : nullptr;
  for (auto k : {k_bpost<1, 0>, k_bpost<1, 1>, k_bpost<1, 2>})
    SBO_HIP(hipFuncSetAttribute(reinterpret_cast<const void*>(k), hipFuncAttributeMaxDynamicSharedMemorySize, (int)L.lds));
  L.lrows = (double*)c->bl_lpart.p;
  if (L.defer && (rc = gemm_grad_deferred(L))) return rc;
  for (int part = 0; part < (L.colw ? 2 : 1); ++part) gemm_post_part(L, part);
  if (L.defer && !L.colw) {
    SBO_HIP(hipStreamWaitEvent(c->stream, c->ev_grad[2], 0));
    c->grad_pending = false;
  }
  if (req.lmax_defer) {
    out.lmax_pending = true;
    out.lmax_per_out = (int)L.rows_out;
  } else {
    hipExtLaunchKernelGGL(k_lmax_reduce, dim3((unsigned)L.q), dim3(256), 0, c->stream, nullptr, c->ev[1], 0, (const double*)L.lrows,
                          (int)L.rows_out, c->Lmax);
  }
  out.stop_attached = true;
  c->gb.active = c->opt.guard_band && !c->is_shadow && g.band_ready;
  gemm_flops(L);
  SBO_HIP(hipGetLastError());
  return SBO_OK;
}
```

### safe-bayesian-optimization_amd/csrc/internal.hpp

```cpp
#pragma once
#include <hip/hip_runtime.h>
#include <stddef.h>
#include <stdint.h>
#include <cmath>
#include <string>
#include <type_traits>
#include <vector>
#include "../../include/safebo.h"

namespace sbo {

constexpr int kGuardRefMaxNpad = 1008;
constexpr int kMaxD = SBO_MAX_D;
constexpr int kMaxQ = SBO_MAX_Q;

struct RcScal {
  unsigned long long ulo_key, uhi_key, vmax_key;
  long long count;
};
struct RcHead {
  RcScal sc;
  unsigned long long deferred;
  unsigned long long lmin_key;
  unsigned long long all_ranks;
// ... 46 lines not shown
  const void* pts;
  long long n_local, first;
  double lo[kMaxD], hi[kMaxD], step[kMaxD];
  long long count[kMaxD];
};

struct DevBuf;
int ensure(DevBuf& b, size_t bytes);
struct DevBuf {
  void* p = nullptr;
  size_t bytes = 0;
  DevBuf() = default;
  DevBuf(const DevBuf&) = delete;
  DevBuf& operator=(DevBuf&& o) noexcept {
    if (this != &o) { reset(); p = o.p; bytes = o.bytes; o.p = nullptr; o.bytes = 0; }
    return *this;
  }
  ~DevBuf() { reset(); }
  void reset() { if (p) (void)hipFree(p); p = nullptr; bytes = 0; }
};
struct ResetBuf {
  DevBuf buf;
  template <class Fill> int acquire(size_t bytes, Fill&& fill, long long key = 0) {
    const bool fresh = buf.bytes < bytes;
    if (int rc = ensure(buf, bytes)) return rc;
    const bool stale = fresh || !neutral_ || key != key_;
    neutral_ = false;
    key_ = key;
    return stale ? fill() : SBO_OK;
  }
  void reset_enqueued() { neutral_ = true; }
  void in_use() { neutral_ = false; }

 private:
  bool neutral_ = false;
  long long key_ = 0;
};
struct Event {
  hipEvent_t e = nullptr;
  Event() = default;
  Event(const Event&) = delete;
  ~Event() { if (e) (void)hipEventDestroy(e); }
};
struct Stream {
  hipStream_t s = nullptr;
  Stream() = default;
  Stream(const Stream&) = delete;
  ~Stream() { if (s) (void)hipStreamDestroy(s); }
};
struct Pinned {
  void* p = nullptr;
  size_t bytes = 0;
  Pinned() = default;
  Pinned(const Pinned&) = delete;
  ~Pinned() { reset(); }
  void reset() { if (p) (void)hipHostFree(p); p = nullptr; bytes = 0; }
};

struct ListIndex {
  bool valid = false;
  bool built_now = false;
  bool ran = false;
  long long n = 0;
  int d = 0;
  int perm_half = 0;
  DevBuf box;
  DevBuf keys, vals, hist;
  DevBuf xs;
  DevBuf stats;
  Event ev0, ev1;
};

struct ColBits {
  unsigned long long* Sw;
  unsigned long long* Uw;
  unsigned long long* Usum;
  unsigned long long* slots;
};
constexpr int kColSlots = 64;
enum ColSlotField { kSlotUmin = 0 , kSlotS, kSlotU, kSlotB , kSlotVmin0, kSlotVmin1 ,
                    kSlotRmax1 , kSlotL0, kSlotL1 ,
                    kSlotRowMask ,
                    kSlotSkip ,
                    kSlotSkipSafe , kColSlotFields };
__host__ __device__ inline bool col_slot_is_min(int f) { return f == kSlotUmin || f == kSlotVmin0 || f == kSlotVmin1; }
constexpr unsigned int kTlistUnsafe = 0x80000000u, kTlistSafe = 0x40000000u;
constexpr unsigned char kSkipUnsafe = 1, kSkipSafe = 2;
constexpr int kTlistShift = 5, kTlistShards = 1 << kTlistShift, kTlistHead = 32;
struct PostExtra {
  int o0;
  int q;
  int lean;
  long long fstride;
  int nograd;
  ColBits cb;
  const double* encl;
  uint8_t* skip;
  int skip_safe;
  const unsigned int* tlist;
  int tshift, tcap;
  int tgx, tgy;
};

struct GemmOps {
  int sets = 1;
  int KB1 = 0;
  size_t sP1A = 0, sT4f = 0, sBt1 = 0;
  double *BtA = nullptr, *P0f = nullptr, *VA = nullptr, *SBf = nullptr;
  size_t sBtA = 0, sP0f = 0, sVA = 0, sSBf = 0;
  int KB0 = 0, KS0 = 0, KBm = 0, KSm = 0, KBm2 = 0;
  int ncs0 = 0, nrb = 0;
  int* eff = nullptr;
  const double* gtmax = nullptr;
  const unsigned long long* gkey = nullptr;
  bool band_ready = false;
  int imode = 0;
};

struct BilinearPlan {
  bool valid = false;
  bool usable = false;
  int r0u = 0;
  long long nlines_pad = 0;
  int r0[kMaxQ] = {0}, r1[kMaxQ] = {0};
  double setup_ms = 0.0;
  GemmOps ops;
  bool encl_ready = false;
  bool vals_ready = false;
  bool bt_ready = false;
};

struct PostRequest {
  int fuse = 0;
  double fuse_b = 0.0;
  bool lmax_defer = false;
  bool col = false;
  int col_lean = 0;
  int sweep_lean = 0;
  bool exact = false;
};

constexpr int kColRowRmax1 = 4 + kMaxQ + 1;
struct ColPartRows {
  unsigned long long* base = nullptr;
  int cap = 0;
  int tiles = 0;
  int count() const { return 2 * tiles; }
  const unsigned long long* field(int f) const { return base + (size_t)f * cap; }
  const unsigned long long* tumin() const { return field(0); }
  const unsigned long long* tumax() const { return field(kColRowRmax1); }
  const unsigned long long* olmin() const { return field(1) + tiles; }
};

struct PostOutcome {
  bool col_active = false;
  bool col_forked = false;
  int col_lean = 0;
  bool col_sched = false;
  int fuse_rows = 0;
  ColPartRows col_rows;
  bool lmax_pending = false;
  int lmax_per_out = 0;
  bool stop_attached = false;
};

struct InterpPlan {
  bool valid = false;
  bool usable = false;
  bool used = false;
  unsigned long long serial = 0;
  GemmOps ops;
  bool grad_deferred = false;
};

struct TensorPlan {
  DevBuf pts, vals, work, W0t, W1t, probe, scr;
  DevBuf gather;
  DevBuf W[SBO_MAX_D];
  size_t work_half = 0;
  double flops = 0.0;
  bool valid = false, usable = false;
  unsigned long long model = 0;
  long long first = 0, nlocal = 0, count[4] = {0, 0, 0, 0};
  double lo[4] = {0, 0, 0, 0}, hi[4] = {0, 0, 0, 0};
  int level[4] = {0, 0, 0, 0};
  int dn[4] = {0, 0, 0, 0};
  DevBuf tail;
  double band[7 * SBO_MAX_Q] = {0};
  int bump = 0;
  bool lean_probe = false;
  void invalidate() { valid = false; }
};

struct ResidentBand {
  bool active = false;
  DevBuf buf;
  long long first = 0;
  bool mirrored = false;
  bool host_valid = false;
  double host[7 * SBO_MAX_Q] = {0};
  DevBuf pts, vals;
  DevBuf part;
  DevBuf probe;
  unsigned long long plan_model = 0;
  long long plan_first = -1, plan_n = -1;
};

struct Audit {
  long long tick = 0;
  DevBuf pts, val, part, cnt;
  hipEvent_t ev[2]{};
// ... 45 lines not shown
  int halo_reruns = 0;
};

struct Recheck {
  sbo_ctx* shadow = nullptr;
  static constexpr unsigned long long kNoSerial = ~0ull;
  unsigned long long serial = kNoSerial;
  DevBuf mean, var;
  DevBuf list;
  DevBuf refined;
  DevBuf probe;
  bool band_valid = false;
  double band_dm[kMaxQ] = {}, band_dv[kMaxQ] = {};
  long long probe_round = 0;
  void invalidate() { band_valid = false; }
  ~Recheck();
};

struct Robust {
  DevBuf vals, mask, part;
  long long nc = 0;
  int q = 0;
  bool valid = false;
  void invalidate() { valid = false; }
};

struct LooSummary {
  double logdet, lpd, z_max;
  int z_argmax, outside;
};
struct Loo {
  DevBuf part;
  DevBuf out;
  Pinned h_out;
};

struct ResidentFactor {
  const double *F() const { return (const double*)F_.p; }  const double *alpha() const { return (const double*)alpha_.p; }
  double *F_mut() { return (double*)F_.p; }                double *alpha_mut() { return (double*)alpha_.p; }
  double *spare_F() { return (double*)Fspare_.p; }         double *spare_alpha() { return (double*)aspare_.p; }
  int ld() const { return ld_; }                           int a_ld() const { return a_ld_; }
  bool present() const { return F_.p != nullptr && alpha_.p != nullptr; }
  int build(int n, int npad, int q);
  int reserve(sbo_ctx* c, int rows);
  int spare_ensure_zeroed(sbo_ctx* c);
  void adopt_spare() { std::swap(F_.p, Fspare_.p); std::swap(F_.bytes, Fspare_.bytes); std::swap(alpha_.p, aspare_.p); std::swap(alpha_.bytes, aspare_.bytes); }

 private:
  DevBuf F_, alpha_, Fspare_, aspare_;
  int ld_ = 0, a_ld_ = 0;
};

}

struct sbo_ctx {
  struct Owned {
    sbo::Stream stream, stream2, stream3, stream_audit, stream4;
    sbo::Event ev_factor, ev_w, ev[8], ev_join[SBO_MAX_Q], ev_col[3], ev_grad[4], ev_audit[2];
    sbo::Pinned h_c1, h_back;
  } own;
  int device = 0;
  hipStream_t stream = nullptr;
  hipStream_t stream2 = nullptr;
  hipStream_t stream_audit = nullptr;
  hipStream_t stream4 = nullptr;
  hipStream_t stream3 = nullptr;
  int n_cu = 256;
  int decide_wg_per_cu = 1;
  struct Options {
    int chol_async = 1;
    int exact_lazy = 1;
    double cheb_tol = 4e-15;
    int tensor_cheb = 1;
    int tensor_guess_pct = 100;
    int guard_band = 1;
    int guard_audit = 1024;
    int guard_audit_every = 16;
    double audit_scale = 1.0;
    int set_lanes = 1;
    int refine_lds = 1;
    int lipschitz_lds = 1;
    int list_index = -1;
    int k1_sched = 1;
    int k1_skip_safe = 1;
    int comm_events = 0;
    int col_path = 1;
    int col_overlap = 1;
    int col_queue = 128;
    int grad_defer = 1;
    int halo_spec = 1;
    int scan_waves = 1;
    int scan_blocks = 1;
    int result_mirror = 1;
    int set_fuse = 1;
    int fuse_classify = -1;
    int goose_pairs = 0;
    int phase_events = 0;
    int bilinear = 1;
    int posterior_path = 0;
    int fp64_recheck = 1;
    int comm_selftest = 0;
  } opt;
  bool has_model = false;
  int dtype = SBO_F64;
  sbo::ModelConst mc{};
  sbo::DevBuf Fpk;
  sbo::DevBuf As;
  sbo::DevBuf sqA;
  sbo::DevBuf alpha;
  sbo::DevBuf Xn;
  sbo::DevBuf E0f;
  sbo::DevBuf Er;
  sbo::DevBuf AXg;
  size_t fpk_stride = 0;
  std::vector<double> h_Xnorm;
  std::vector<double> h_Ynorm;
  sbo::ResidentFactor factor;
  sbo::DevBuf mwork;
  sbo::DevBuf appendbuf;
  sbo::DevBuf removebuf;
  sbo::Loo loo;
  sbo::DevBuf invk_img;
  bool invk_img_valid = false;
  bool invk_w_valid = false;
  const double* invk_plain = nullptr;
  bool factor_todo = false;
  bool factor_pending = false;
  hipEvent_t ev_factor = nullptr, ev_w = nullptr;
  unsigned long long model_serial = 0;
  sbo::BilinearPlan bl;
  sbo::DevBuf bl_P0f, bl_P1A, bl_T4f, bl_BtA, bl_SBf, bl_VA, bl_small, bl_work, bl_cheb;
  sbo::DevBuf bl_basis;
  bool bl_basis_ok = false;
  unsigned long long bl_basis_serial = 0;
  double bl_basis_ab[4] = {0, 0, 0, 0};
  sbo::DevBuf bl_grad;
  sbo::DevBuf bl_lpart;
  sbo::DevBuf bl_encl;
  sbo::ResetBuf bl_sched;
  sbo::Pinned h_stage;
  struct K1AuditRecord {
    bool skip_armed = false;
    bool encl_check = false;
    size_t encl_tiles = 0;
  } k1_audit;
  sbo::InterpPlan bi;
  sbo::DevBuf bi_params;
  sbo::Pinned h_bi_params;
  sbo::Event ev_bi_params;
  hipEvent_t ev_grad[4]{};
  bool grad_pending = false;
  sbo::TensorPlan tn;
  sbo::ResidentBand gb;
  sbo::Audit audit;
  sbo::DevBuf list_scr;
  bool has_cand = false;
  sbo::CandSpec cs{};
  sbo::DevBuf pts;
  sbo::DevBuf mean, var;
  bool posterior_valid = false;
  bool post_l0_missing = false;
  int last_k1 = 0;
  double last_k1_flops = 0.0;
  unsigned long long* Lmax = nullptr;
  sbo::DevBuf maskS, maskU, maskM, maskG, maskO;
  sbo::DevBuf fitbuf, fitwork;
  sbo::DevBuf refbuf;
  sbo::DevBuf lipbuf;
  sbo::DevBuf batchbuf;
  sbo::DevBuf expbuf;
  sbo::DevBuf pathbuf;
  sbo::DevBuf jointbuf;
  struct SetLane {
    hipStream_t stream = nullptr;
    sbo::DevBuf dist2, dist2b;
    sbo::DevBuf coarse;
    sbo::DevBuf blockmin;
    sbo::DevBuf blockmax;
    sbo::DevBuf scanlist;
    sbo::DevBuf amb;
    sbo::DevBuf gw;
    sbo::DevBuf runmeta;
    sbo::DevBuf lxtree;
    sbo::DevBuf scal;
    bool amb_clean = false;
  } lane[2];
  sbo::DevBuf partial;
  sbo::ListIndex lx;
  sbo::DevBuf cpart;
  int cpart_cap = 0;
  int host_syncs = 0;
  sbo::DevBuf fuseS, fuseU;
  sbo::ColPath col;
  sbo::MultiRank dist;
  sbo::PinnedBack* h_back = nullptr;
  int last_sweep = 0;
  bool masks_valid = false;
  sbo_profile prof{};
  hipEvent_t ev[8]{};
  hipEvent_t ev_join[SBO_MAX_Q]{};
  bool is_shadow = false;
  sbo::Recheck recheck;
  sbo::Robust rob;
};

inline sbo::Recheck::~Recheck() { delete shadow; }

namespace sbo {
inline bool multi_rank(const sbo_ctx* c) { return c->dist.world > 1 || c->opt.comm_selftest; }
inline bool twin_current(const sbo_ctx* c) {
  return c->dtype == SBO_F32 && c->recheck.shadow && c->recheck.shadow->has_model && c->recheck.serial == c->model_serial;
}
inline ScalBlock* scal_block(const sbo_ctx* c) { return (ScalBlock*)c->lane[0].scal.p; }
struct GuardBand;
inline const GuardBand* resident_band(const sbo_ctx* c) {
  return (c->gb.active && c->opt.guard_band && c->gb.buf.p) ? (const GuardBand*)c->gb.buf.p : nullptr;
}
int fail(int code, const std::string& msg);
int hip_fail(hipError_t e, const char* what);
int ensure(DevBuf& b, size_t bytes);
hipError_t stream_wait(const sbo_ctx* c, hipStream_t st);
void release(DevBuf& b);
void drain_streams(sbo_ctx* c);
int col_decide_resident(int* wg_per_cu);
int factor_sync(sbo_ctx* c);

int model_reader_check(const sbo_ctx* c, const char* who, bool need_f64);
int model_reader_begin(sbo_ctx* c, const char* who, bool need_f64);
inline bool all_finite(const double* p, size_t count) {
  for (size_t t = 0; t < count; ++t)
    if (!std::isfinite(p[t])) return false;
  return true;
}

struct Carve {
  unsigned char* base;
  size_t off = 0, floor = 1;
  template <class T> void take(T*& p, size_t count, size_t align = alignof(T)) {
    align = align > floor ? align : floor;
    off = (off + align - 1) / align * align;
    p = base ? reinterpret_cast<T*>(base + off) : nullptr;
    off += sizeof(T) * count;
  }
};
template <class F> int carve(DevBuf& buf, F&& layout, size_t floor = 1) {
  const size_t bytes = layout(Carve{nullptr, 0, floor});
  if (int rc = ensure(buf, bytes)) return rc;
  if (layout(Carve{(unsigned char*)buf.p, 0, floor}) != bytes) return fail(SBO_E_INVALID, "a scratch layout changed between its two passes");
  return SBO_OK;
}

template <class F> auto with_dpad(int dpad, F&& f) {
  switch (dpad) {
    case 2: return f(std::integral_constant<int, 2>{});
    case 4: return f(std::integral_constant<int, 4>{});
    default: return f(std::integral_constant<int, 8>{});
  }
}
inline int spad_of(int S) { return S <= 16 ? 16 : S <= 32 ? 32 : 64; }
template <class F> auto with_spad(int Spad, F&& f) {
  switch (Spad) {
    case 16: return f(std::integral_constant<int, 1>{});
    case 32: return f(std::integral_constant<int, 2>{});
    default: return f(std::integral_constant<int, 4>{});
  }
}

int posterior_enqueue(sbo_ctx* c, const PostRequest& req, PostOutcome* out);
inline hipError_t k1_stop(sbo_ctx* c, const PostOutcome& out) { return out.stop_attached ? hipSuccess : hipEventRecord(c->ev[1], c->stream); }

int launch_posterior(sbo_ctx* c, const PostRequest& req, PostOutcome& out);
int launch_bound(sbo_ctx* c, double b, int index, int kind, void* dev_out);
int model_build(sbo_ctx* c, const double* const* host_invK, const double* X_norm, const double* Y_norm);
int model_prep(sbo_ctx* c, const double* X_norm);
struct FitBatchResult {
  double x[kMaxQ][kMaxD + 2], de_x[kMaxQ][kMaxD + 2], nll[kMaxQ], de_nll[kMaxQ];
  int generations[kMaxQ], polish_status[kMaxQ], polish_evals[kMaxQ], polished[kMaxQ];
  int host_syncs;
  double de_ms, polish_ms;
};
int fit_batch(sbo_ctx* c, int n, int d, int q, const double* X_norm, const double* Y_norm, int P, const double* lo, const double* hi,
              const double* init_pop, const uint64_t* seeds, int maxiter, double tol, double atol, int polish, int polish_maxiter,
              double ftol, double gtol, FitBatchResult& out);
int model_factor_enqueue(sbo_ctx* c);
int model_pack_invk(sbo_ctx* c);
struct ModelUpdate {
  int rows = 0, index = -1, ld = 0;
  unsigned long long serial = 0;
  const double *rho = nullptr, *scratch = nullptr, *sk = nullptr;
  const double *U = nullptr, *G = nullptr, *w = nullptr;
};
int model_append_stage(sbo_ctx* c, const double* x_norm_new, const double* y_norm_new, ModelUpdate& u);
int model_append_block_stage(sbo_ctx* c, int k, const double* x_norm_new, const double* y_norm_new, ModelUpdate& u);
ModelUpdate model_update_staged(const sbo_ctx* c, int rows, int index = -1);
int model_update_commit(sbo_ctx* c, const ModelUpdate& u);
int model_loo(sbo_ctx* c, double b, bool arrays, const unsigned char** host);
int model_repack(sbo_ctx* c);
bool bilinear_applicable(const sbo_ctx* c);
int bilinear_basis_enqueue(sbo_ctx* c, hipStream_t st, bool force_big);
bool interp_applicable(const sbo_ctx* c);
int interp_setup(sbo_ctx* c);
int guard_probe_gradients(sbo_ctx* c, hipStream_t st, double* ppts, double* grad_out, const sbo::ModelConst* mcp = nullptr);
int bilinear_setup(sbo_ctx* c);
int launch_posterior_gemm(sbo_ctx* c, bool interp, const PostRequest& req, PostOutcome& out);
inline void post_regions_written(sbo_ctx* c) { c->bl.encl_ready = c->bl.vals_ready = false; }
inline void post_values_patched(sbo_ctx* c) { c->bl.vals_ready = false; }
inline void plans_invalidate(sbo_ctx* c) {
  c->bl.valid = false;
  c->bi.valid = false;
  c->posterior_valid = false;
  c->recheck.invalidate();
}
inline void model_changed(sbo_ctx* c) {
  c->masks_valid = false;
  c->rob.invalidate();
  plans_invalidate(c);
}
enum CandKind { kCandPoints, kCandGrid, kCandGridSharded };
inline void candidates_changed(sbo_ctx* c, CandKind kind) {
  if (kind == kCandPoints) c->lx.valid = false;
  else for (auto& g : c->dist.halo_guess) g = -1;
  c->dist.sharded = kind == kCandGridSharded;
  c->rob.invalidate();
  plans_invalidate(c);
  c->masks_valid = false;
}
enum OptEffect {
  kOptNothing,
  kOptPlans,
  kOptPlansBand,
  kOptTensor,
  kOptInterp,
  kOptPosterior
};
inline void option_changed(sbo_ctx* c, OptEffect effect) {
  switch (effect) {
    case kOptNothing: break;
    case kOptPlans: plans_invalidate(c); break;
    case kOptPlansBand: plans_invalidate(c); c->tn.invalidate(); break;
    case kOptTensor: c->tn.invalidate(); c->posterior_valid = false; break;
    case kOptInterp: c->bi.valid = false; break;
    case kOptPosterior: c->posterior_valid = false; c->recheck.invalidate(); break;
  }
}
bool tensor_applicable(const sbo_ctx* c);
int launch_posterior_tensor(sbo_ctx* c, const PostRequest& req, bool* declined);
int launch_posterior_on_axes(sbo_ctx* c, int d, const long long* count, const double* axc, double* mean_out, double* var_out, double* grad_out,
                             unsigned long long* lmax);
int launch_posterior_on_list(sbo_ctx* c, const double* pts, long long N, double* mean_out, double* var_out);
struct PathDraws {
  int output, S, F;
  const double *omega, *phase, *weights, *noise;
  std::vector<double> omega_padded;
};
struct PathImage {
  const double* Bt;
  const double *om, *ph;
  const double *B, *As, *sq;
  double *pts, *vals;
  int F, S, output;
  long long m;
};
int paths_check_draws(const sbo_ctx* c, const PathDraws& dr);
int paths_prepare_list(sbo_ctx* c, PathDraws& dr, long long m, PathImage* img);
int paths_eval_list(sbo_ctx* c, const PathImage& img);
int guard_exact_list(sbo_ctx* c, const double* pts, long long N, double* mean_out, double* var_out);
int guard_exact_grad_list(sbo_ctx* c, const double* pts, long long N, double* grad_out );
int guard_probe_reference(sbo_ctx* c, hipStream_t side, double** ref_m, double** ref_v, const sbo::ModelConst* mcp = nullptr);
struct GbAnalytic {
  const double* axis_eps;
  const double* alpha;
  int a_ld, n;
  int rc[sbo::kMaxQ][2];
  const double* Xn;
  int dpad, pad;
  double ab[4];
  const double* ref_g;
};
int guard_band_from_probes(sbo_ctx* c, const double* pm, const double* pv, const double* ref_m, const double* ref_v, const double* tail, const GbAnalytic& an);
int guard_band_host(sbo_ctx* c, const double* dm, const double* dv, const double* rl, const double* parts = nullptr );
int guard_audit_enqueue(sbo_ctx* c, const PostOutcome& out);
void guard_audit_harvest(sbo_ctx* c, bool wait);
}

#define SBO_HIP(x)                                                   \
  do {                                                               \
    hipError_t e__ = (x);                                            \
    if (e__ != hipSuccess) return sbo::hip_fail(e__, #x);            \
  } while (0)
// ... 1 lines not shown
```

### safe-bayesian-optimization_amd/csrc/posterior.hip

```cpp
#include <algorithm>
#include <cstring>
#include <type_traits>
#include "device_common.hpp"

namespace sbo {

constexpr int kWaves = 4;

template <typename T> __device__ __forceinline__ T exp_t(T x);
template <> __device__ __forceinline__ double exp_t<double>(double x) { return exp(x); }
template <> __device__ __forceinline__ float exp_t<float>(float x) { return __expf(x); }

__device__ __forceinline__ int row_block_of(int r, int w) {
  const int base = (r >> 1) * (2 * kWaves);
  return (r & 1) ? base + 2 * kWaves - 1 - w : base + w;
}

template <typename T, int S, int D>
__global__ __launch_bounds__(256) void k_posterior(const ModelConst mc, const CandSpec cs,
                                                   const T* __restrict__ Fpk, size_t fpk_stride,
                                                   const T* __restrict__ As, const T* __restrict__ sqA,
                                                   const T* __restrict__ alpha, const T* __restrict__ Xn,
                                                   T* __restrict__ mean_out, T* __restrict__ var_out,
                                                   unsigned long long* __restrict__ Lmax) {
// ... 759 lines not shown
  const size_t per_strip = sizeof(T) * (size_t)c->mc.npad * 16;
  const size_t budget = 144 * 1024;
  if (per_strip * 4 <= budget) return launch_posterior_d<T, 4>(c, t);
  if (per_strip * 2 <= budget) return launch_posterior_d<T, 2>(c, t);
  if (per_strip <= budget) return launch_posterior_d<T, 1>(c, t);
  return fail(SBO_E_UNSUPPORTED, "n too large for the LDS-resident cross-covariance tile");
}

template <typename T, int D, int S>
static int launch_posterior_grid_ts(sbo_ctx* c, const PostTarget& t) {
  constexpr int P = 16 * S;
  const ModelConst& mc = c->mc;
  const CandSpec& cs = t.cs;
  const int npad = mc.npad, nfr = npad / 4, q = mc.q, d = cs.d;
  const long long cnt0 = cs.count[0];
  const long long ntile0 = (cnt0 + 15) / 16;
  GridTables gt;
  memset(&gt, 0, sizeof(gt));
  gt.e0_stride = (size_t)ntile0 * nfr * 64;
  size_t off = 0;
  for (int a = 1; a < d; ++a) {
    gt.er_off[a] = off;
    off += (size_t)cs.count[a] * npad;
  }
  gt.er_stride_o = off;
  gt.nlines = cs.n_local / cnt0;
  gt.line0 = cs.first / cnt0;
  int rc;
  if ((rc = ensure(c->E0f, sizeof(T) * (gt.e0_stride * q + 512)))) return rc;
  if ((rc = ensure(c->Er, sizeof(T) * std::max<size_t>(gt.er_stride_o, 1) * q))) return rc;
  const long long total = (long long)gt.e0_stride + (long long)gt.er_stride_o;
  hipLaunchKernelGGL((k_build_tables<T>), dim3((unsigned)std::min<long long>((total + 255) / 256, 4096), q), dim3(256), 0,
                     c->stream, mc, cs, (const T*)c->As.p, mc.dpad, (T*)c->E0f.p, gt.e0_stride, (T*)c->Er.p, gt.er_stride_o,
                     gt.er_off[1], gt.er_off[2], gt.er_off[3], gt.er_off[4], gt.er_off[5], gt.er_off[6], gt.er_off[7], t.axc);
  if ((rc = ensure(c->AXg, sizeof(T) * (size_t)q * npad * (1 + D)))) return rc;
  hipLaunchKernelGGL((k_build_ax<T>), dim3(1, q), dim3(256), 0, c->stream, mc, (const T*)c->alpha.p, (const T*)c->Xn.p, D,
                     (T*)c->AXg.p);
  const size_t lds = sizeof(T) * ((size_t)S * npad + 8 + (size_t)(2 + D) * kWaves * 4 * P);
  const bool ax = t.axc != nullptr;
  if (ax && !(sizeof(T) == 8 && D == 4 && S == 4)) return fail(SBO_E_UNSUPPORTED, "internal: explicit axes are an fp64 path of three / four axes");
  auto kern = ax ? k_posterior_grid<T, S, D, (sizeof(T) == 8 && D == 4 && S == 4)> : k_posterior_grid<T, S, D, false>;
  SBO_HIP(hipFuncSetAttribute(reinterpret_cast<const void*>(kern), hipFuncAttributeMaxDynamicSharedMemorySize, (int)lds));
  const long long tiles = ntile0 * ((gt.nlines + S - 1) / S);
  if (tiles > 0x7fffffffLL) return fail(SBO_E_UNSUPPORTED, "too many candidate tiles for one launch");
  int per_cu = 0;
  SBO_HIP(hipOccupancyMaxActiveBlocksPerMultiprocessor(&per_cu, kern, 256, lds));
  per_cu = std::max(1, std::min(per_cu, 4));
  const long long wgs = std::min<long long>(tiles, ((long long)c->n_cu * per_cu + q - 1) / q);
  hipLaunchKernelGGL(kern, dim3((unsigned)std::max<long long>(wgs, 1), (unsigned)q), dim3(256), lds, c->stream, mc, cs, gt,
                     (const T*)c->Fpk.p, c->fpk_stride, (const T*)c->E0f.p, (const T*)c->Er.p, (const T*)c->AXg.p,
                     (unsigned int)tiles, (T*)t.mean, (T*)t.var, t.Lmax, t.axc, (T*)t.grad);
  SBO_HIP(hipGetLastError());
  return SBO_OK;
}

template <typename T, int D>
static int launch_posterior_grid_t(sbo_ctx* c, const PostTarget& t) {
  return launch_posterior_grid_ts<T, D, 4>(c, t);
}

template <typename T>
static int launch_posterior_grid(sbo_ctx* c, const PostTarget& t) {
  return with_dpad(c->mc.dpad, [&](auto D) { return launch_posterior_grid_t<T, D()>(c, t); });
}

static bool grid_path_ok(const sbo_ctx* c) {
  const CandSpec& cs = c->cs;
  if (c->opt.posterior_path != 0) return false;
  if (cs.kind != 1 || cs.n_local <= 0) return false;
  const long long cnt0 = cs.count[0];
  return cs.first % cnt0 == 0 && cs.n_local % cnt0 == 0;
}

static bool generic_chunked(const sbo_ctx* c) {
  const size_t tile_bytes = (c->dtype == SBO_F64 ? 8u : 4u) * (size_t)c->mc.npad * 64;
  return c->opt.posterior_path == 2 || tile_bytes > 64 * 1024;
}
static int launch_generic(sbo_ctx* c, const PostTarget& t);

int launch_posterior(sbo_ctx* c, const PostRequest& req, PostOutcome& out) {
  c->gb.active = false;
  c->k1_audit = {};
  const bool encl_kept = c->bl.valid && c->bl.encl_ready, vals_kept = encl_kept && c->bl.vals_ready;
  post_regions_written(c);
  const double tri_flops = (double)c->mc.q * c->mc.npad * (c->mc.npad + 16.0) * (double)c->cs.n_local;
  const PostTarget t{c->cs, c->mean.p, c->var.p, c->Lmax};
  if (grid_path_ok(c)) {
    if (!req.exact && bilinear_applicable(c)) {
      int rc;
      if (!c->bl.valid && interp_applicable(c)) {
        if (!(c->bi.valid && c->bi.serial == c->model_serial) && (rc = interp_setup(c))) return rc;
        if (c->bi.usable && !c->bi.used) {
          c->last_k1 = 6;
          return launch_posterior_gemm(c, true, req, out);
        }
      }
      if (!c->bl.valid && (rc = bilinear_setup(c))) return rc;
      if (c->bl.usable) {
        c->last_k1 = 4;
        c->bl.encl_ready = encl_kept;
        c->bl.vals_ready = vals_kept;
        return launch_posterior_gemm(c, false, req, out);
      }
    }
    if (!req.exact && tensor_applicable(c)) {
      bool declined = true;
      const int rct = launch_posterior_tensor(c, req, &declined);
      if (rct || !declined) return rct;
    }
    { const int rcf = factor_sync(c); if (rcf) return rcf; }
    SBO_HIP(hipMemsetAsync(t.Lmax, 0, sizeof(unsigned long long) * kMaxQ, c->stream));
    c->last_k1 = 3;
    c->last_k1_flops = tri_flops;
    return c->dtype == SBO_F64 ? launch_posterior_grid<double>(c, t) : launch_posterior_grid<float>(c, t);
  }
  { const int rcf = factor_sync(c); if (rcf) return rcf; }
  c->last_k1_flops = tri_flops;
  c->last_k1 = generic_chunked(c) ? 2 : 1;
  return launch_generic(c, t);
}

static int launch_generic(sbo_ctx* c, const PostTarget& t) {
  SBO_HIP(hipMemsetAsync(t.Lmax, 0, sizeof(unsigned long long) * kMaxQ, c->stream));
  if (generic_chunked(c)) return c->dtype == SBO_F64 ? launch_posterior_chunked<double>(c, t) : launch_posterior_chunked<float>(c, t);
  return c->dtype == SBO_F64 ? launch_posterior_s<double>(c, t) : launch_posterior_s<float>(c, t);
}

int launch_posterior_on_axes(sbo_ctx* c, int d, const long long* count, const double* axc, double* mean_out, double* var_out, double* grad_out,
                             unsigned long long* lmax) {
  if (c->dtype != SBO_F64) return fail(SBO_E_UNSUPPORTED, "internal: explicit axes are an fp64 path");
  { const int rcf = factor_sync(c); if (rcf) return rcf; }
  PostTarget t{};
  t.cs.kind = 1;
  t.cs.d = d;
  long long N = 1;
  for (int a = 0; a < d; ++a) { t.cs.count[a] = count[a]; N *= count[a]; }
  for (int a = d; a < kMaxD; ++a) t.cs.count[a] = 1;
  t.cs.n_local = N;
  t.mean = mean_out;
  t.var = var_out;
  t.Lmax = lmax;
  t.axc = axc;
  t.grad = grad_out;
  SBO_HIP(hipMemsetAsync(lmax, 0, sizeof(unsigned long long) * kMaxQ, c->stream));
  return launch_posterior_grid<double>(c, t);
}

int launch_posterior_on_list(sbo_ctx* c, const double* pts, long long N, double* mean_out, double* var_out) {
  if (c->dtype != SBO_F64) return fail(SBO_E_UNSUPPORTED, "internal: exact lists are an fp64 path");
  int rc;
  if ((rc = ensure(c->list_scr, 512))) return rc;
  PostTarget t{};
  t.cs.kind = 0;
  t.cs.d = c->mc.d;
  t.cs.pts_dtype = SBO_F64;
  t.cs.pts = pts;
  t.cs.n_local = N;
  t.cs.first = 0;
  t.mean = mean_out;
  t.var = var_out;
  t.Lmax = (unsigned long long*)c->list_scr.p;
  { const int rcf = factor_sync(c); if (rcf) return rcf; }
  return launch_generic(c, t);
}

int launch_bound(sbo_ctx* c, double b, int index, int kind, void* dev_out) {
  const long long n = c->cs.n_local;
  const int blocks = (int)std::min<long long>((n + 255) / 256, 4096);
  if (c->dtype == SBO_F64) {
    const double* m = (const double*)c->mean.p + (size_t)index * n;
    const double* v = (const double*)c->var.p + (size_t)index * n;
    hipLaunchKernelGGL(k_bound<double>, dim3(blocks), dim3(256), 0, c->stream, m, v, n, b, kind, (double*)dev_out);
  } else {
    const float* m = (const float*)c->mean.p + (size_t)index * n;
    const float* v = (const float*)c->var.p + (size_t)index * n;
    hipLaunchKernelGGL(k_bound<float>, dim3(blocks), dim3(256), 0, c->stream, m, v, n, (float)b, kind, (float*)dev_out);
  }
  SBO_HIP(hipGetLastError());
  return SBO_OK;
}

int launch_soa_to_aos(sbo_ctx* c, const void* soa, void* aos) {
  const long long n = c->cs.n_local;
  const int q = c->mc.q;
// ... 11 lines not shown
```

### safe-bayesian-optimization_amd/csrc/sets.hip

```cpp
#include <algorithm>
#include <cstdio>
#include <cstdlib>
#include <cmath>
#include <cstring>
#include <type_traits>
#include <hip/hip_ext.h>
#include "device_common.hpp"

namespace sbo {

int comm_allreduce_max_u64(sbo_ctx* c, unsigned long long* dev, int count);
int comm_allreduce_min_u64(sbo_ctx* c, unsigned long long* dev, int count);
int comm_allreduce_sum_f64(sbo_ctx* c, double* dev, int count);
int comm_allgather_bytes(sbo_ctx* c, const void* send, void* recv, size_t bytes_per_rank);

constexpr double kInfD = 1.0e300;
constexpr int kArgSlots = 16;

struct SweepScalars {
  unsigned long long ustar_key;
  unsigned long long rmax_key[kMaxQ];
  long long count_S, count_U, count_M;
  long long count_set[kMaxQ];
  long long n_amb, n_amb_total;
  long long n_scan;
  long long halo_short;
  double arg_val[kArgSlots];
  long long arg_idx[kArgSlots];
  double arg_d[kArgSlots];
  long long n_guard;
  long long guard_slot[kArgSlots];
  long long tiles_skipped;
  long long tiles_skipped_safe;
  unsigned long long ticket;
  long long n_guard_cls;
  long long guard_nb0;
  unsigned long long vmin_key[kMaxQ];
  double gb_du[kMaxQ];
  double gb_rl[kMaxQ];
  double arg_e1[kArgSlots], arg_e2[kArgSlots];
  long long arg_ei[kArgSlots];
};
constexpr size_t kScalHost = offsetof(SweepScalars, ticket);
static_assert(sizeof(SweepScalars) <= sizeof(ScalBlock::scalars) && sizeof(SweepScalars) <= sizeof(PinnedBack::scalars), "SweepScalars fits its region of the scalar block and of the pinned block");

struct Best {
  double v;
  long long i;
  double d;
  double e1, e2;
  long long ei;
};
template <bool MAX>
__host__ __device__ __forceinline__ Best best_none() { return Best{0.0, -1, 0.0, MAX ? -kInfD : kInfD, MAX ? -kInfD : kInfD, -1}; }

template <bool MAX>
__host__ __device__ __forceinline__ bool better(const Best& a, const Best& b) {
  if (a.i < 0) return false;
  if (b.i < 0) return true;
  if (MAX ? (a.v > b.v) : (a.v < b.v)) return true;
  return a.v == b.v && a.i < b.i;
}
template <bool MAX>
__host__ __device__ __forceinline__ void ends_take(Best& B, double end, long long i) {
  if (MAX ? (end > B.e1) : (end < B.e1)) { B.e2 = B.e1; B.e1 = end; B.ei = i; }
  else if (MAX ? (end > B.e2) : (end < B.e2)) B.e2 = end;
}
template <bool MAX>
__host__ __device__ __forceinline__ void best_take(Best& B, double v, double d, long long i) {
  if (B.i < 0 || (MAX ? (v > B.v) : (v < B.v)) || (v == B.v && i < B.i)) { B.v = v; B.i = i; B.d = d; }
  ends_take<MAX>(B, MAX ? v + d : v - d, i);
}
template <bool MAX>
__host__ __device__ __forceinline__ Best best_merge(const Best& a, const Best& b) {
  Best r = a;
  if (better<MAX>(b, a)) { r.v = b.v; r.i = b.i; r.d = b.d; }
  ends_take<MAX>(r, b.e1, b.ei);
  if (MAX ? (b.e2 > r.e2) : (b.e2 < r.e2)) r.e2 = b.e2;
  return r;
}
template <bool MAX>
__host__ __device__ __forceinline__ bool arg_near(const Best& w) {
  if (w.i < 0) return false;
  const double other = w.ei == w.i ? w.e2 : w.e1;
  return MAX ? !(other < w.v - w.d) : !(other > w.v + w.d);
}

template <bool MAX>
__device__ __forceinline__ Best wave_best(Best x) {
#pragma unroll
  for (int o = 32; o > 0; o >>= 1) {
    Best y;
    y.v = __shfl_xor(x.v, o);
    y.i = __shfl_xor(x.i, o);
    y.d = __shfl_xor(x.d, o);
    y.e1 = __shfl_xor(x.e1, o);
    y.e2 = __shfl_xor(x.e2, o);
    y.ei = __shfl_xor(x.ei, o);
    x = best_merge<MAX>(x, y);
  }
  return x;
}

template <bool MAX>
__device__ __forceinline__ Best block_best(Best x) {
  __shared__ Best sh[16];
  x = wave_best<MAX>(x);
  const int lane = threadIdx.x & 63, wave = threadIdx.x >> 6, nw = (blockDim.x + 63) >> 6;
  __syncthreads();
  if (lane == 0) sh[wave] = x;
  __syncthreads();
  if (wave == 0) {
    Best y = lane < nw ? sh[lane] : best_none<MAX>();
    y = wave_best<MAX>(y);
    x = y;
  }
// ... 1776 lines not shown
  hipLaunchKernelGGL((k_arg_masked_multi<T, true, ValArray<T>>), dim3((unsigned)nb, 1u), dim3(256), 0, c->stream,
                     ValArray<T>{(const T*)v.var->p, 0.0}, (const uint8_t*)nullptr, (const uint8_t*)c->maskG.p, n, (long long)c->cs.first, pbase,
                     pstride, 1, gb_of<T>(c, v));
  hipLaunchKernelGGL(k_sweep_clear_slot, dim3(1), dim3(1), 0, c->stream, sc, 1);
  hipExtLaunchKernelGGL(k_sweep_finals<true>, dim3((unsigned)q), dim3(256), 0, c->stream, nullptr, c->ev[4], 0,
                        (const unsigned char*)pbase, pstride, nb, sc, (const SweepScalars*)nullptr, (unsigned char*)c->h_back,
                        c->Lmax, gb_of<T>(c, v) ? 1 : 0);
  SBO_HIP(hipGetLastError());
  return sweep_exchange_back(c, h, AllMax().v, Lk, c->ev[4], true);
}

#include "sets_colpath.inc.hpp"

template <typename T>
static int sweep_safeopt_t(sbo_ctx* c, const sbo_sweep_opts* o, const SetView& v, sbo_safeopt_result* res) {
  const long long n = c->cs.n_local;
  const int q = c->mc.q;
  int rc;
  bool reuse;
  PostOutcome post;
  if ((rc = sweep_open<T>(c, o, v, kSafeOpt, &reuse, post))) return rc;
  SweepScalars h;
  unsigned long long Lk[kMaxQ];
  const bool colpath = post.col_active;
  if (colpath) {
    if (post.col_lean) c->posterior_valid = false;
    if ((rc = col_set_phase(c, o, v, post, h, Lk))) return rc;
  } else {
  MinimizerJob mj;
  const int nb = reduce_blocks(c);
  const bool lazy_exact = c->opt.exact_lazy && q == 2 && !multi_rank(c) && !v.refined && c->opt.result_mirror && n > 0 &&
                          whole_planes(c);
  const size_t pstride = partial_stride(nb);
  if ((rc = ensure(c->partial, pstride * (size_t)q))) return rc;
  unsigned char* pbase = (unsigned char*)c->partial.p;
  const bool lanes = lanes_on(c);
  {
    const bool defer = q >= 2 && !multi_rank(c) && c->opt.set_fuse && n > 0 && !lanes;
    if ((rc = sweep_common_front<T>(c, o, v, post, defer ? &mj.fin : nullptr))) return rc;
    if ((rc = sweep_exchange_front<T>(c, o, true))) return rc;
    mj.pending = n > 0;
    mj.nb = nb;
    mj.partial = (Best*)pbase;
    if (q < 2 || multi_rank(c)) launch_minimizer<T>(c, c->lane[0], o, v, &mj);
    if (c->opt.phase_events) SBO_HIP(hipEventRecord(c->ev[2], c->stream));
    if (lanes && (rc = lanes_fork(c))) return rc;
    for (int cc = 1; cc < q; ++cc) {
      uint8_t* G = (uint8_t*)c->maskG.p + (size_t)(cc - 1) * n;
      const bool side = lanes && ((cc - 1) & 1);
      if ((rc = expander_set<T>(c, c->lane[side], o, v, cc, G, side ? nullptr : &mj, lazy_exact))) return rc;
    }
    launch_minimizer<T>(c, c->lane[0], o, v, &mj);
    if (lanes && (rc = lanes_join(c))) return rc;
  }
  SweepScalars* sc = (SweepScalars*)c->lane[0].scal.p;
  if (c->opt.phase_events) SBO_HIP(hipEventRecord(c->ev[3], c->stream));
  if (n > 0 && q > 1) {
    hipLaunchKernelGGL((k_arg_masked_multi<T, true, ValArray<T>>), dim3((unsigned)nb, (unsigned)(q - 1)), dim3(256), 0, c->stream,
                       ValArray<T>{(const T*)v.var->p, 0.0}, (const uint8_t*)nullptr, (const uint8_t*)c->maskG.p, n, (long long)c->cs.first, pbase,
                       pstride, 1, gb_of<T>(c, v));
  }
  const bool mirrored = !multi_rank(c) && c->opt.result_mirror;
  hipExtLaunchKernelGGL(k_sweep_finals<true>, dim3((unsigned)q), dim3(256), 0, c->stream, nullptr, mirrored ? c->ev[4] : nullptr, 0,
                        (const unsigned char*)pbase, pstride, n > 0 ? nb : 0, sc,
                        lanes ? (const SweepScalars*)c->lane[1].scal.p : (const SweepScalars*)nullptr,
                        mirrored ? (unsigned char*)c->h_back : (unsigned char*)nullptr, c->Lmax, gb_of<T>(c, v) ? 1 : 0);
  SBO_HIP(hipGetLastError());
  if ((rc = sweep_exchange_back(c, h, AllMax().v, Lk, c->ev[4], mirrored))) return rc;
  if (lazy_exact && (h.n_amb > 0 || c->opt.exact_lazy == 2) && (rc = late_exact_pass<T>(c, o, v, nb, h, Lk, launch_exact_d<T>))) return rc;
  if (multi_rank(c)) {
    sbo_sweep_opts o2 = *o;
    SetView v2 = v;
    if (halo_rerun(c, h, Lk, o2, v2)) return sweep_safeopt_t<T>(c, &o2, v2, res);
  }
  }
  c->masks_valid = true;
  c->last_sweep = 1;
  if (getenv("SBO_DEBUG_SCAN")) fprintf(stderr, "[safebo] open candidates scanned (last constraint) %lld, exact rechecks %lld\n", h.n_scan, h.n_amb_total);

  if ((rc = sweep_profile(c, kSafeOpt, reuse))) return rc;
  c->prof.set_path = colpath ? 1 : 0;
  c->prof.k1_tiles_skipped = colpath ? h.tiles_skipped : 0;
  c->prof.k1_tiles_skipped_safe = colpath ? h.tiles_skipped_safe : 0;

  memset(res, 0, sizeof(*res));
  res->count_S = h.count_S;
  res->count_U = h.count_U;
  res->count_M = h.count_M;
  res->n_exact_rechecks = h.n_amb_total;
  res->guard_band = h.n_guard;
  c->gb.first = h.n_guard;
  for (int i = 0; i < q; ++i) memcpy(&res->L[i], &Lk[i], 8);
  if (o->lean && q >= 2) res->L[0] = 0.0;
  res->minimizer_index = -1;
  res->expander_index = -1;
  for (int cc = 1; cc <= kMaxQ; ++cc) res->expander_index_c[cc - 1] = -1;
  if (h.count_S == 0) return fail(SBO_E_EMPTY_SAFE_SET, "safe set S_t is empty on this candidate set");
  res->u_star = ord_val(h.ustar_key);
  res->minimizer_index = h.arg_idx[0];
  res->minimizer_std = std::sqrt(h.arg_val[0]);
  coords_of(c, res->minimizer_index, res->minimizer_x);
  double best_std = 0.0;
  int best_c = 0;
  for (int cc = 1; cc < q; ++cc) {
    res->count_G[cc - 1] = h.count_set[cc - 1];
    res->expander_index_c[cc - 1] = h.arg_idx[cc];
    res->expander_std_c[cc - 1] = h.arg_idx[cc] >= 0 ? std::sqrt(h.arg_val[cc]) : 0.0;
    if (h.arg_idx[cc] >= 0 && (best_c == 0 || res->expander_std_c[cc - 1] > best_std)) {
      best_std = res->expander_std_c[cc - 1];
      best_c = cc;
    }
  }
  res->expander_best_c = best_c;
  if (best_c) {
    res->expander_index = res->expander_index_c[best_c - 1];
    res->expander_std = best_std;
    coords_of(c, res->expander_index, res->expander_x);
  }
  res->choose_minimizer = res->minimizer_std > res->expander_std;
  if (gb_of<T>(c, v)) {
    long long near = 0;
    for (int cc = 1; cc < q && best_c; ++cc)
      if (cc != best_c && h.arg_idx[cc] >= 0 && h.arg_idx[cc] != h.arg_idx[best_c] &&
          !(h.arg_val[cc] + h.arg_d[cc] < h.arg_val[best_c] - h.arg_d[best_c])) ++near;
    if (best_c && h.arg_idx[0] >= 0 && h.arg_idx[0] != h.arg_idx[best_c] &&
        std::fabs(h.arg_val[0] - h.arg_val[best_c]) <= h.arg_d[0] + h.arg_d[best_c]) ++near;
    res->guard_band += near;
    c->gb.first += near;
  }
  return SBO_OK;
}

template <typename T>
static int sweep_goose_t(sbo_ctx* c, const sbo_sweep_opts* o, const SetView& v, sbo_goose_result* res);
template <typename T>
static int sweep_tr_t(sbo_ctx* c, const sbo_sweep_opts* o, const SetView& v, const double* x0, double r, sbo_tr_result* res);
#include "sets_recheck.inc.hpp"

template <typename T>
struct GooseSources {
  CandSpec css; const T* W;
  long long run_lo, run_hi;
  bool w_is_window;
};
template <typename T>
static int goose_exchange(const SetCall<T>& a, const SetWindow& w, long long maxlocal, GooseSources<T>& s) {
  sbo_ctx* c = a.c;
  const long long n = c->cs.n_local, plane = w.plane, H = w.halo;
  int rc;
  long long min_planes = w.planes_total;
  for (int r = 0; r < c->dist.world; ++r) min_planes = std::min(min_planes, (c->dist.first_of[r + 1] - c->dist.first_of[r]) / plane);
  const bool slabs = c->dist.sharded && H <= min_planes;
  if (getenv("SBO_DEBUG_COMM"))
    fprintf(stderr, "[rank %d] GoOSE sources c=%d: halo %lld planes, smallest shard %lld planes -> %s\n", c->dist.rank, a.cidx, H, min_planes,
            slabs ? "slab exchange" : "full all-gather");
  if (slabs) {
    const size_t slab = (size_t)H * plane;
    if ((rc = ensure(c->dist.gather, sizeof(T) * slab * 2 * (c->dist.world + 1)))) return rc;
    if ((rc = ensure(c->dist.Wfull, sizeof(T) * (size_t)w.nt))) return rc;
    T *send = (T*)c->dist.gather.p, *recv = send + 2 * slab;
    SBO_HIP(hipMemcpyAsync(send, a.ln.gw.p, sizeof(T) * slab, hipMemcpyDeviceToDevice, a.ln.stream));
    SBO_HIP(hipMemcpyAsync(send + slab, (const T*)a.ln.gw.p + (size_t)n - slab, sizeof(T) * slab, hipMemcpyDeviceToDevice, a.ln.stream));
    if ((rc = comm_allgather_bytes(c, send, recv, sizeof(T) * slab * 2))) return rc;
    T* win = (T*)c->dist.Wfull.p;
    size_t at = 0;
    if (w.own0 > w.w0) {
// ... 511 lines not shown
```

### safe-bayesian-optimization_amd/csrc/sets_colpath.inc.hpp

```cpp
#pragma once

struct ColGeom {
  int W, H, NS, NB;
  int NBp;
  int CW, CH;
  int CNB, CNBp, CWp;
  int gxt;
  double h0, h1;
  double delta;
};
constexpr int kColBig = 1 << 20;

typedef unsigned short us2_t __attribute__((ext_vector_type(2)));
__device__ __forceinline__ void col_fine_item(long long item, const ColGeom gm, const ColBits cb, unsigned short* __restrict__ tile,
                                              unsigned short* __restrict__ img, unsigned short* __restrict__ bmin,
                                              unsigned long long* __restrict__ Mw, unsigned long long* __restrict__ Gw) {
  const int lane = threadIdx.x & 63;
  const int ncg = gm.W >> 6;
  const int s = (int)(item / ncg), cgp = (int)(item % ncg);
  const int i = cgp * 64 + lane;
  Mw[(size_t)s * gm.W + i] = 0ull;
  Gw[(size_t)s * gm.W + i] = 0ull;
  const unsigned long long m = cb.Uw[(size_t)s * gm.W + i];
  const unsigned long long us = cb.Usum[i];
// ... 59 lines not shown
    if (half == 0) *reinterpret_cast<unsigned int*>(bmin + ((size_t)(64 * s + r)) * gm.NBp + (size_t)cgp * 2) = mine | (other << 16);
  }
  __builtin_amdgcn_wave_barrier();
}

__device__ __forceinline__ void col_coarse_job(int blk, const ColGeom gm, const unsigned long long* __restrict__ Uw, unsigned long long* lds_words,
                                               unsigned short* __restrict__ cimg, unsigned short* __restrict__ cbmin) {
  const int cl = threadIdx.x & 31, Sg = threadIdx.x >> 5;
  const int ci = blk * 32 + cl;
  const int CNS = (gm.CH + 63) >> 6;
  unsigned long long word = 0ull;
  if (ci < gm.CW && Sg < CNS) {
#pragma unroll
    for (int f = 0; f < 8; ++f) {
      const int s = 8 * Sg + f;
      if (s < gm.NS) {
        const unsigned long long* w = Uw + (size_t)s * gm.W + (size_t)ci * 8;
        unsigned long long x = 0ull;
#pragma unroll
        for (int k = 0; k < 8; ++k) x |= w[k];
        x |= x >> 4;
        x |= x >> 2;
        x |= x >> 1;
        x &= 0x0101010101010101ull;
        word |= ((x * 0x0102040810204080ull) >> 56) << (8 * f);
      }
    }
  }
  lds_words[Sg * 32 + cl] = word;
  __syncthreads();
  if (Sg >= CNS) return;
  int f = kColBig, dn = kColBig;
  for (int sp = Sg - 1; sp >= 0; --sp) {
    const unsigned long long w = lds_words[sp * 32 + cl];
    if (w) { f = 64 * Sg - 1 - (64 * sp + 63 - __clzll((long long)w)); break; }
  }
  for (int sn = Sg + 1; sn < CNS; ++sn) {
    const unsigned long long w = lds_words[sn * 32 + cl];
    if (w) { dn = (64 * sn + __ffsll((long long)w) - 1) - (64 * Sg + 64); break; }
  }
  const unsigned int nlo = ~(unsigned int)word, nhi = ~(unsigned int)(word >> 32);
  int F[64];
#pragma unroll
  for (int r = 0; r < 64; ++r) {
    const unsigned int h = r < 32 ? nlo : nhi;
    const int keep = (int)(h << (31 - (r & 31))) >> 31;
    f = (f + 1) & keep;
    F[r] = f;
  }
  unsigned int pk[32];
#pragma unroll
  for (int r = 63; r >= 0; --r) {
    const unsigned int h = r < 32 ? nlo : nhi;
    const int keep = (int)(h << (31 - (r & 31))) >> 31;
    dn = (dn + 1) & keep;
    int t = F[r] < dn ? F[r] : dn;
    t = t > 0xffff ? 0xffff : t;
    cimg[(size_t)(64 * Sg + r) * gm.CWp + ci] = (unsigned short)t;
    if (r & 1) pk[r >> 1] = (unsigned int)t << 16;
    else pk[r >> 1] |= (unsigned int)t;
  }
#pragma unroll
  for (int k = 0; k < 32; ++k) {
    us2_t v;
    v[0] = (unsigned short)(pk[k] & 0xffffu);
    v[1] = (unsigned short)(pk[k] >> 16);
#pragma unroll
    for (int o = 16; o > 0; o >>= 1) {
      const unsigned int y = (unsigned int)__shfl_xor((int)((unsigned int)v[0] | ((unsigned int)v[1] << 16)), o);
      us2_t w2;
      w2[0] = (unsigned short)(y & 0xffffu);
      w2[1] = (unsigned short)(y >> 16);
      v = __builtin_elementwise_min(v, w2);
    }
    if (cl == k) {
      cbmin[(size_t)(64 * Sg + 2 * k) * gm.CNBp + blk] = v[0];
      cbmin[(size_t)(64 * Sg + 2 * k + 1) * gm.CNBp + blk] = v[1];
    }
  }
}

__device__ __forceinline__ unsigned long long col_slot_reduce(const unsigned long long* __restrict__ slots, int field) {
  unsigned long long v = slots[(size_t)field * kColSlots + (threadIdx.x & 63)];
  const bool is_min = col_slot_is_min(field), is_sum = field == kSlotS || field == kSlotU || field == kSlotB || field == kSlotSkip || field == kSlotSkipSafe;
#pragma unroll
  for (int o = 32; o > 0; o >>= 1) {
    const unsigned long long y = __shfl_xor(v, o);
    v = is_sum ? v + y : (is_min ? (y < v ? y : v) : (y > v ? y : v));
  }
  return v;
}
__device__ __forceinline__ void col_merge1_body(const unsigned long long* __restrict__ slots, SweepScalars* sc, unsigned long long* Lmax,
                                                const GuardBand* gb, double b) {
  unsigned long long* w = reinterpret_cast<unsigned long long*>(sc);
  for (unsigned i = threadIdx.x; i < sizeof(SweepScalars) / 8; i += blockDim.x) w[i] = 0ull;
  __syncthreads();
  if (threadIdx.x < 64) {
    const unsigned long long cS = col_slot_reduce(slots, kSlotS), cU = col_slot_reduce(slots, kSlotU), cB = col_slot_reduce(slots, kSlotB);
    const unsigned long long vmin = col_slot_reduce(slots, kSlotVmin1), rmax = col_slot_reduce(slots, kSlotRmax1), l1 = col_slot_reduce(slots, kSlotL1);
    const unsigned long long nskip = col_slot_reduce(slots, kSlotSkip), nsafe = col_slot_reduce(slots, kSlotSkipSafe);
    if (threadIdx.x == 0) {
      Lmax[1] = l1;
      sc->tiles_skipped = (long long)nskip;
      sc->tiles_skipped_safe = (long long)nsafe;
      sc->ustar_key = ~0ull;
      sc->count_S = (long long)cS;
      sc->count_U = (long long)cU;
      sc->rmax_key[1] = rmax;
      if (gb) {
        sc->n_guard = (long long)cB;
        sc->n_guard_cls = (long long)cB;
        sc->vmin_key[1] = vmin;
        const bool any = vmin != ~0ull;
        const double vm = any ? fmax(0.0, ord_val(vmin)) : 0.0;
        sc->gb_du[1] = gb->dm[1] + (any ? b * gb_dsqrt(vm, gb->dv[1]) : 0.0);
        sc->gb_rl[0] = gb->rl[0];
        sc->gb_rl[1] = gb->rl[1];
      }
    }
  }
  if (threadIdx.x >= 64 && threadIdx.x < 64 + kArgSlots) sc->arg_idx[threadIdx.x - 64] = -1;
}
struct ColScal2 {
  unsigned long long ustar_key, vmin0_key;
  double gb_du0;
};
__device__ __forceinline__ void col_merge2_body(const unsigned long long* __restrict__ slots, unsigned long long& ustar_key,
                                                unsigned long long& vmin0_key) {
  ustar_key = col_slot_reduce(slots, kSlotUmin);
  vmin0_key = col_slot_reduce(slots, kSlotVmin0);
}

struct ColMergeJob {
  const unsigned long long* slots;
  SweepScalars* sc;
  unsigned long long* Lmax;
  const GuardBand* gb;
  double b;
};
__global__ __launch_bounds__(256) void k_col_a(const ColGeom gm, const ColBits cb, const ColMergeJob mg, int ncoarse, unsigned short* __restrict__ cimg,
                                               unsigned short* __restrict__ cbmin, unsigned short* __restrict__ img, unsigned short* __restrict__ bmin,
                                               unsigned long long* __restrict__ Mw, unsigned long long* __restrict__ Gw) {
  constexpr size_t kTileBytes = 4 * 64 * 64 * sizeof(unsigned short);
  __shared__ __attribute__((aligned(16))) unsigned char mem[kTileBytes];
  const int bid = (int)blockIdx.x;
  if (bid == 0) {
    col_merge1_body(mg.slots, mg.sc, mg.Lmax, mg.gb, mg.b);
  } else if (bid < 1 + ncoarse) {
    col_coarse_job(bid - 1, gm, cb.Uw, reinterpret_cast<unsigned long long*>(mem), cimg, cbmin);
  } else {
    const int nfine = (int)gridDim.x - 1 - ncoarse;
    unsigned short* tile = reinterpret_cast<unsigned short*>(mem) + (threadIdx.x >> 6) * 64 * 64;
    const long long nitems = (long long)gm.NS * (gm.W >> 6);
    for (long long item = (long long)(bid - 1 - ncoarse) * 4 + (threadIdx.x >> 6); item < nitems; item += (long long)nfine * 4)
      col_fine_item(item, gm, cb, tile, img, bmin, Mw, Gw);
  }
}
__device__ __forceinline__ void lcb_bounds(double m, double v, double b, double& lo, double& hi) {
  const float sf = __fsqrt_rn((float)v);
  const double s_up = (double)sf * (1.0 + 0x1p-20) + 1e-18;
  double s_lo = (double)sf * (1.0 - 0x1p-20) - 1e-18;
  s_lo = s_lo > 0.0 ? s_lo : 0.0;
  const double x = m - b * s_up, y = m - b * s_lo;
  lo = x - (x < 0 ? -x : x) * 0x1p-50;
  hi = y + (y < 0 ? -y : y) * 0x1p-50;
  if (!(sf < 3.0e38f)) { lo = -kInfD; hi = kInfD; }
}

struct F32Bound {
  float u, amax, del;
  bool ok;
};
__device__ __forceinline__ F32Bound f32_bound(double m, double v, float bf ) {
  const float mf = (float)m, sf = __builtin_amdgcn_sqrtf((float)v);
  F32Bound r;
  r.amax = fmaf(fabsf(bf), sf, fabsf(mf));
  r.u = fmaf(bf, sf, mf);
  r.del = r.amax * 1.0e-6f;
  r.ok = r.amax > 1.0e-25f && r.amax < 1.0e25f;
  return r;
}
template <bool E2>
__device__ __forceinline__ void take_max(bool on, double v, unsigned int g, double& bv, unsigned int& bg, double& e2) {
  const bool c = on && (v > bv || (v == bv && g < bg));
  if (E2) {
    const double loser = c ? bv : (on ? v : -kInfD);
    e2 = loser > e2 ? loser : e2;
  }
  bv = c ? v : bv;
  bg = c ? g : bg;
}
__device__ __forceinline__ Best best_from(double bv, unsigned int bg, double e2) {
  Best b = best_none<true>();
  if (bg != 0xffffffffu) { b.v = bv; b.i = (long long)bg; b.e2 = e2; }
  return b;
}

struct ColUnitMap {
  unsigned int mask;
  int cnt, pre;
  long long total;
};
template <int HALVES>
__device__ __forceinline__ ColUnitMap col_unit_map(const unsigned long long* __restrict__ slots, int NS) {
  const int lane = threadIdx.x & 63;
  ColUnitMap um;
  um.mask = lane < NS ? (unsigned int)slots[(size_t)kSlotRowMask * kColSlots + lane] : 0u;
  um.cnt = 8 * HALVES * __popc(um.mask);
  int inc = um.cnt;
#pragma unroll
  for (int o = 1; o < 64; o <<= 1) { const int t = __shfl_up(inc, o); if (lane >= o) inc += t; }
  um.pre = inc - um.cnt;
  um.total = __shfl(inc, 63);
  return um;
}
struct ColUnit {
  int s, c, oct;
  int tile;
  int c0;
  size_t w0;
  size_t g0;
};
template <int HALVES>
__device__ __forceinline__ ColUnit col_unit(const ColGeom& gm, const ColUnitMap& um, long long u, int lane) {
  const unsigned long long at = __ballot(um.cnt > 0 && (long long)um.pre <= u);
  const int s = 63 - __clzll((long long)at);
  const unsigned int mask = (unsigned int)__builtin_amdgcn_readlane((int)um.mask, s);
  const int pc = __builtin_amdgcn_readlane(um.cnt, s) >> 3;
  const int local = __builtin_amdgcn_readfirstlane((int)u) - __builtin_amdgcn_readlane(um.pre, s);
  const int oct = local / pc, rem = local - oct * pc;
  const int t = HALVES == 2 ? rem >> 1 : rem, half = HALVES == 2 ? rem & 1 : 0;
  const unsigned long long hit = __ballot(lane < 32 && ((mask >> lane) & 1u) && __popc(mask & ((1u << lane) - 1u)) == t);
  const int tc = (int)__ffsll((long long)hit) - 1;
  ColUnit x;
  x.oct = oct;
  x.s = s;
  x.tile = s * gm.gxt + tc;
  x.c0 = tc * 128 + 64 * half;
  x.c = x.c0 + (HALVES == 2 ? lane : 2 * lane);
  x.w0 = (size_t)x.s * gm.W + x.c;
  x.g0 = ((size_t)(64 * x.s + 8 * x.oct)) * gm.W + x.c;
  return x;
}
typedef double d2c_t __attribute__((ext_vector_type(2)));
typedef unsigned long long u2c_t __attribute__((ext_vector_type(2)));

struct ColMinJob {
  ColGeom gm;
  const unsigned long long* slots;
  unsigned long long* Lmax;
  ColScal2* sc2;
  const unsigned long long* olmin;
  const unsigned long long* Sw;
  const double* mean0;
  const double* var0;
  double b;
  unsigned long long* Mw;
  const unsigned long long* Gw;
  Best* partial;
  Best* gpartial;
  const GuardBand* gb;
};
template <int PART>
__global__ __launch_bounds__(256) void k_col_min(const ColMinJob j) {
  unsigned long long ukey, vkey;
  col_merge2_body(j.slots, ukey, vkey);
  const ColUnitMap um = col_unit_map<1>(j.slots, j.gm.NS);
  const long long nunits = um.total;
  double du0 = 0.0;
  if (j.gb) {
    const bool any = vkey != ~0ull;
    const double vm = any ? fmax(0.0, ord_val(vkey)) : 0.0;
    du0 = j.gb->dm[0] + (any ? j.b * gb_dsqrt(vm, j.gb->dv[0]) : 0.0);
  }
  if (blockIdx.x == 0 && threadIdx.x < 64) {
    const unsigned long long l0 = PART == 1 ? col_slot_reduce(j.slots, kSlotL0) : 0ull;
    if (threadIdx.x == 0) {
      if (PART == 0) { j.sc2->ustar_key = ukey; j.sc2->vmin0_key = vkey; j.sc2->gb_du0 = du0; }
      else j.Lmax[0] = l0;
    }
  }
  const ColGeom& gm = j.gm;
  const double ustar = ord_val(ukey), b = j.b;
  const bool anyS = ukey != ~0ull;
  const GuardBand* gb = j.gb;
  const bool e2on = gb != nullptr;
  double bvM = -kInfD, e2M = -kInfD, bvG = -kInfD, e2G = -kInfD;
  unsigned int bgM = 0xffffffffu, bgG = 0xffffffffu;
  long long cM = 0, cB = 0, cG = 0;
  const double dM = gb ? 2.0 * du0 * (1.0 + 0x1p-40) : -1.0, dv0 = gb ? gb->dv[0] : 0.0;
  const double mg = dM > 0.0 ? dM : 0.0;
  const float bf = -(float)b, ulo_f = __double2float_rd(ustar - mg), uhi_f = __double2float_ru(ustar + mg);
  const int lane = threadIdx.x & 63;
  const long long wave = ((long long)blockIdx.x * blockDim.x + threadIdx.x) >> 6, nwaves = ((long long)gridDim.x * blockDim.x) >> 6;
  uint8_t* Mb = reinterpret_cast<uint8_t*>(j.Mw);
  for (long long u = wave; u < nunits && anyS; u += nwaves) {
    const ColUnit x = col_unit<1>(gm, um, u, lane);
    const u2c_t sw = PART == 0 ? *reinterpret_cast<const u2c_t*>(j.Sw + x.w0) : u2c_t{0ull, 0ull};
    const u2c_t gw = PART == 1 ? *reinterpret_cast<const u2c_t*>(j.Gw + x.w0) : u2c_t{0ull, 0ull};
    const unsigned int sb[2] = {(unsigned int)(sw[0] >> (8 * x.oct)) & 0xffu, (unsigned int)(sw[1] >> (8 * x.oct)) & 0xffu};
    const unsigned int gbt[2] = {(unsigned int)(gw[0] >> (8 * x.oct)) & 0xffu, (unsigned int)(gw[1] >> (8 * x.oct)) & 0xffu};
    unsigned int mb[2] = {0u, 0u}, und[2] = {0u, 0u};
    const unsigned long long lk = PART == 0 ? j.olmin[x.tile] : ~0ull;
    const bool mposs = PART == 0 && lk != ~0ull && !(ord_val(lk) > ustar + mg);
    const unsigned int any8 = mposs ? (sb[0] | sb[1]) : (gbt[0] | gbt[1]);
    if (__ballot(any8 != 0u) != 0ull) {
      d2c_t mu[8], va[8];
#pragma unroll
      for (int k = 0; k < 8; ++k) {
        const bool on = (any8 >> k) & 1u;
        const size_t g = x.g0 + (size_t)k * gm.W;
        mu[k] = (on && mposs) ? *reinterpret_cast<const d2c_t*>(j.mean0 + g) : d2c_t{0.0, 0.0};
        va[k] = on ? *reinterpret_cast<const d2c_t*>(j.var0 + g) : d2c_t{0.0, 0.0};
      }
      const unsigned int g32 = (unsigned int)x.g0;
#pragma unroll
      for (int k = 0; k < 8; ++k) {
#pragma unroll
        for (int e = 0; e < 2; ++e) {
          const double v = va[k][e];
          const unsigned int g = g32 + (unsigned int)(k * gm.W + e);
          if (PART == 0) {
            const bool on = mposs && ((sb[e] >> k) & 1u);
            const F32Bound fb = f32_bound(mu[k][e], v, bf);
            const bool sureM = fb.ok && fb.u + fb.del < ulo_f, sureN = fb.ok && fb.u - fb.del > uhi_f;
            const bool mm = on && sureM;
            und[e] |= (on && !sureM && !sureN) ? (1u << k) : 0u;
            mb[e] |= mm ? (1u << k) : 0u;
            if (__ballot(mm) != 0ull) {
              cM += mm;
              if (e2on) take_max<true>(mm, v, g, bvM, bgM, e2M);
              else take_max<false>(mm, v, g, bvM, bgM, e2M);
            }
          } else {
            const bool gg = (gbt[e] >> k) & 1u;
            if (__ballot(gg) != 0ull) {
              cG += gg;
              if (e2on) take_max<true>(gg, v, g, bvG, bgG, e2G);
              else take_max<false>(gg, v, g, bvG, bgG, e2G);
            }
          }
        }
      }
      while (__ballot((und[0] | und[1]) != 0u) != 0ull) {
        const bool act = (und[0] | und[1]) != 0u;
        const int e = und[0] ? 0 : 1;
        const int k = act ? (int)(__ffs((int)und[e]) - 1) : 0;
        if (act) und[e] &= und[e] - 1u;
        const size_t g = x.g0 + (size_t)k * gm.W + e;
        const double m = act ? j.mean0[g] : 0.0, v = act ? j.var0[g] : 0.0;
        bool mm = false;
        if (act) {
          double lcb, ucb;
          lcb_ucb(m, v, b, lcb, ucb);
          mm = lcb <= ustar;
          const double gap = lcb - ustar;
          cB += (gap < 0 ? -gap : gap) <= dM;
        }
        mb[e] |= mm ? (1u << k) : 0u;
        cM += mm;
        if (e2on) take_max<true>(mm, v, (unsigned int)g, bvM, bgM, e2M);
// ... 325 lines not shown
      bool out = false;
      if (best_d < 0.5 * kInfD) {
        const double dm = sqrt(best_d);
        const double eps = eps_abs + 1e-11 * dm;
        const double tol = 1e-12 * (fabs(ucb) + du + L * dm);
        const double lo = ucb - du - L * (dm + eps), hi = ucb + du - L * (dm - eps);
        if (lo > tol) out = true;
        else if (hi >= -tol) amb[atomicAdd((unsigned long long*)&sc->n_amb, 1ull)] = g;
      }
      if (out) atomicOr(&Gh[2 * ((size_t)(j >> 6) * gm.W + i) + ((j >> 5) & 1)], 1u << (j & 31));
    }
  }
}

constexpr int kColFinParts = 8;
struct ColFinRow { Best b; long long cnt, nb; };
__global__ __launch_bounds__(256) void k_col_finals(const Best* __restrict__ reg0, int n0, const Best* __restrict__ reg1, int n1, SweepScalars* sc,
                                                    const ColScal2* sc2, ColFinRow* fin, unsigned long long* tickets, unsigned char* mirror,
                                                    const unsigned long long* Lkeys, int gb_on, unsigned long long* slots) {
  const int slot = blockIdx.y, p = blockIdx.x;
  const Best* reg = slot == 0 ? reg0 : reg1;
  const int n = slot == 0 ? n0 : n1;
  const int i0 = (int)((long long)n * p / (int)gridDim.x), i1 = (int)((long long)n * (p + 1) / (int)gridDim.x);
  Best best = best_none<true>();
  long long cnt = 0, nb = 0;
  {
    const long long* pc = (const long long*)(reg + n);
#pragma unroll 4
    for (int i = i0 + (int)threadIdx.x; i < i1; i += blockDim.x) {
      best = best_merge<true>(best, reg[i]);
      cnt += pc[i];
      nb += pc[n + i];
    }
    best = block_best<true>(best);
    cnt = block_sum_ll(cnt);
    nb = block_sum_ll(nb);
  }
  const int parts = (int)gridDim.x;
  __shared__ int last;
  if (parts > 1) {
    if (threadIdx.x == 0) {
      fin[slot * kColFinParts + p] = ColFinRow{best, cnt, nb};
      __threadfence();
      const unsigned long long t = atomicAdd(&tickets[slot], 1ull);
      last = t == (unsigned long long)(parts - 1);
      if (last) tickets[slot] = 0ull;
    }
    __syncthreads();
    if (!last) return;
    __threadfence();
  }
  if (slot == 1)
    for (int i = threadIdx.x; i < kColSlotFields * kColSlots; i += blockDim.x) slots[i] = col_slot_is_min(i / kColSlots) ? ~0ull : 0ull;
  if (threadIdx.x == 0) {
    if (parts > 1) {
    best = best_none<true>();
    cnt = nb = 0;
    for (int k = 0; k < parts; ++k) {
      const ColFinRow r{Best{__hip_atomic_load(&fin[slot * kColFinParts + k].b.v, __ATOMIC_RELAXED, __HIP_MEMORY_SCOPE_AGENT),
                             __hip_atomic_load(&fin[slot * kColFinParts + k].b.i, __ATOMIC_RELAXED, __HIP_MEMORY_SCOPE_AGENT),
                             __hip_atomic_load(&fin[slot * kColFinParts + k].b.d, __ATOMIC_RELAXED, __HIP_MEMORY_SCOPE_AGENT),
                             __hip_atomic_load(&fin[slot * kColFinParts + k].b.e1, __ATOMIC_RELAXED, __HIP_MEMORY_SCOPE_AGENT),
                             __hip_atomic_load(&fin[slot * kColFinParts + k].b.e2, __ATOMIC_RELAXED, __HIP_MEMORY_SCOPE_AGENT),
                             __hip_atomic_load(&fin[slot * kColFinParts + k].b.ei, __ATOMIC_RELAXED, __HIP_MEMORY_SCOPE_AGENT)},
                        __hip_atomic_load(&fin[slot * kColFinParts + k].cnt, __ATOMIC_RELAXED, __HIP_MEMORY_SCOPE_AGENT),
                        __hip_atomic_load(&fin[slot * kColFinParts + k].nb, __ATOMIC_RELAXED, __HIP_MEMORY_SCOPE_AGENT)};
      best = best_merge<true>(best, r.b);
      cnt += r.cnt;
      nb += r.nb;
    }
    }
    store_slot<true>(sc, slot, best, nb, gb_on != 0);
    if (slot == 0) sc->count_M += cnt;
    else sc->count_set[slot - 1] += cnt;
    SweepScalars* hm = reinterpret_cast<SweepScalars*>(mirror);
    hm->arg_val[slot] = best.v;
    hm->arg_idx[slot] = best.i;
    hm->arg_d[slot] = best.d;
    hm->guard_slot[slot] = sc->guard_slot[slot];
    if (slot == 0) {
      hm->count_M = sc->count_M;
      sc->ustar_key = sc2->ustar_key;
      hm->ustar_key = sc2->ustar_key;
      for (int t = 2; t < kArgSlots; ++t) hm->guard_slot[t] = 0;
    } else {
      hm->count_set[slot - 1] = sc->count_set[slot - 1];
      hm->count_S = sc->count_S;
      hm->count_U = sc->count_U;
      hm->n_amb = sc->n_amb;
      hm->n_amb_total = sc->n_amb_total;
      hm->n_scan = sc->n_scan;
      hm->n_guard = sc->n_guard;
      hm->tiles_skipped = sc->tiles_skipped;
      hm->tiles_skipped_safe = sc->tiles_skipped_safe;
      for (int t = 0; t < kMaxQ; ++t) {
        hm->rmax_key[t] = sc->rmax_key[t];
        reinterpret_cast<unsigned long long*>(mirror + offsetof(PinnedBack, lip_keys))[t] = Lkeys[t];
      }
    }
  }
}

__global__ __launch_bounds__(256) void k_col_expand(const unsigned long long* __restrict__ Wd, int W, long long n, uint8_t* __restrict__ out) {
  for (long long g = (long long)blockIdx.x * blockDim.x + threadIdx.x; g < n; g += (long long)gridDim.x * blockDim.x) {
    const long long j = g / W;
    const int i = (int)(g - j * W);
    out[g] = (uint8_t)((Wd[(size_t)(j >> 6) * W + i] >> (j & 63)) & 1ull);
  }
}
static void col_expand(sbo_ctx* c, const DevBuf& words, uint8_t* out) {
  const long long n = c->cs.n_local;
  hipLaunchKernelGGL(k_col_expand, dim3((unsigned)std::min<long long>((n + 255) / 256, 1 << 16)), dim3(256), 0, c->stream,
                     (const unsigned long long*)words.p, (int)c->cs.count[0], n, out);
}

int col_decide_resident(int* wg_per_cu) {
  SBO_HIP(hipOccupancyMaxActiveBlocksPerMultiprocessor(wg_per_cu, k_col_decide, 256, 0));
  return SBO_OK;
}
static_assert(kRowRmax + 1 == kColRowRmax1, "ColPartRows::tumax is the radius key of constraint 1");

static ColGeom col_geometry(const CandSpec& cs) {
  ColGeom gm;
  gm.W = (int)cs.count[0];
  gm.H = (int)(cs.n_local / gm.W);
  gm.NS = gm.H / 64;
  gm.NB = gm.W / 32;
  gm.NBp = (gm.NB + 7) & ~7;
  gm.CW = gm.W / kCoarse;
  gm.CH = gm.H / kCoarse;
  gm.gxt = gm.W / 128;
  gm.CNB = (gm.CW + 31) / 32;
  gm.CNBp = 16;
  gm.CWp = gm.CNB * 32;
  gm.h0 = cs.step[0];
  gm.h1 = cs.step[1];
  double h2 = 0.0;
  for (int a = 0; a < 2; ++a) h2 += cs.step[a] * cs.step[a];
  gm.delta = (kCoarse - 1) * std::sqrt(h2) * (1.0 + 1e-9);
  return gm;
}

struct ColScratch {
  SweepScalars* sc;
  ColScal2* sc2;
  unsigned long long* tickets;
  ColFinRow* fin;
  int nb;
  Best *reg0, *reg1;
  unsigned short *img, *bmin, *cimg, *cbmin;
  unsigned long long *Mw, *Gw;
  ColBits cb;
};
static int col_scratch(sbo_ctx* c, const ColGeom& gm, hipStream_t es, ColScratch& s) {
  const long long n = c->cs.n_local;
  sbo_ctx::SetLane& ln = c->lane[0];
  int rc;
  if ((rc = ensure(ln.scal, sizeof(SweepScalars)))) return rc;
  s.sc = (SweepScalars*)ln.scal.p;
  static_assert(128 + 2 * kColFinParts * sizeof(ColFinRow) <= 4096, "column path scalar block");
  DevBuf& fin = c->col.fin.buf;
  if ((rc = c->col.fin.acquire(4096, [&]() -> int {
        SBO_HIP(hipMemsetAsync(fin.p, 0, 4096, es));
        return SBO_OK;
      })))
    return rc;
  s.sc2 = (ColScal2*)fin.p;
  s.tickets = (unsigned long long*)((char*)fin.p + 64);
  s.fin = (ColFinRow*)((char*)fin.p + 128);
  s.nb = reduce_blocks(c);
  const size_t pstride = partial_stride(s.nb);
  if ((rc = ensure(c->partial, pstride * 3))) return rc;
  s.reg0 = (Best*)c->partial.p;
  s.reg1 = (Best*)((unsigned char*)c->partial.p + 2 * pstride);
  if ((rc = ensure(ln.amb, sizeof(long long) * (size_t)n))) return rc;
  if ((rc = ensure(ln.scanlist, 2 * sizeof(long long) * (size_t)n))) return rc;
  if ((rc = ensure(c->col.img, sizeof(unsigned short) * (size_t)n + 64))) return rc;
// ... 140 lines not shown
```

Measured before the change: 73.12 billion.

## Reuse recorded per-tile Lipschitz rows and objective map across sweeps in K1

Records each tile's Lipschitz row bound during enclosure and keeps a per-tile objective-map byte array across sweeps. When the rows are still valid, the scheduler skips gradient work for classify-only tiles and routes them through a new lightweight k_bres kernel that classifies from the stored mean and variance. Tiles already known to hold objective work are placed at the back of the list. Invalidation flags tie this cache to region and value rewrites; the risks are stale-cache correctness and added bookkeeping and launches.

New measurement: 82.81 billion, median of 6. 1.13x the previous value.

```diff
diff --git a/include/safebo.h b/include/safebo.h
--- a/include/safebo.h
+++ b/include/safebo.h
@@ -143,6 +143,7 @@
   double guard_analytic_dm[SBO_MAX_Q], guard_analytic_dv[SBO_MAX_Q], guard_probe_dm[SBO_MAX_Q], guard_probe_dv[SBO_MAX_Q];
   int64_t k1_tiles_skipped;
   int64_t k1_tiles_skipped_safe;
+  int64_t k1_tiles_resident_c, k1_tiles_resident_o;
   int64_t guard_audit_skipped;
   double list_index_build_ms;
   int64_t list_index_leaf_pairs, list_index_nodes_skipped;
diff --git a/safe-bayesian-optimization_amd/_lib.py b/safe-bayesian-optimization_amd/_lib.py
--- a/safe-bayesian-optimization_amd/_lib.py
+++ b/safe-bayesian-optimization_amd/_lib.py
@@ -202,7 +202,8 @@
         ("guard_audit_samples", C.c_int64), ("guard_audit_violations", C.c_int64), ("guard_audit_worst", C.c_double),
         ("guard_analytic_dm", C.c_double * SBO_MAX_Q), ("guard_analytic_dv", C.c_double * SBO_MAX_Q),
         ("guard_probe_dm", C.c_double * SBO_MAX_Q), ("guard_probe_dv", C.c_double * SBO_MAX_Q),
-        ("k1_tiles_skipped", C.c_int64), ("k1_tiles_skipped_safe", C.c_int64), ("guard_audit_skipped", C.c_int64),
+        ("k1_tiles_skipped", C.c_int64), ("k1_tiles_skipped_safe", C.c_int64),
+        ("k1_tiles_resident_c", C.c_int64), ("k1_tiles_resident_o", C.c_int64), ("guard_audit_skipped", C.c_int64),
         ("list_index_build_ms", C.c_double), ("list_index_leaf_pairs", C.c_int64), ("list_index_nodes_skipped", C.c_int64),
         ("fp32_band_dm", C.c_double * SBO_MAX_Q), ("fp32_band_dv", C.c_double * SBO_MAX_Q),
     ]
diff --git a/safe-bayesian-optimization_amd/csrc/api.hip b/safe-bayesian-optimization_amd/csrc/api.hip
--- a/safe-bayesian-optimization_amd/csrc/api.hip
+++ b/safe-bayesian-optimization_amd/csrc/api.hip
@@ -276,6 +276,7 @@
     OPT_RANGE(guard_audit_every, 1, 1 << 20, "guard_audit_every: 1 .. 1048576 sweeps", kOptNothing, hook_audit_every),
     OPT_RANGE(grad_defer, 0, 3, "grad_defer must be 0 .. 3", kOptInterp, nullptr),
     OPT_BOOL(k1_sched, kOptNothing, nullptr),
+    OPT_BOOL(k1_resident, kOptNothing, nullptr),
     OPT_BOOL(k1_skip_safe, kOptNothing, nullptr),
     OPT_BOOL(col_overlap, kOptNothing, nullptr),
     OPT_RANGE(col_queue, 64, 128, "col_queue must be within 64 .. 128 (the default)", kOptNothing, nullptr),
diff --git a/safe-bayesian-optimization_amd/csrc/bilinear.hip b/safe-bayesian-optimization_amd/csrc/bilinear.hip
--- a/safe-bayesian-optimization_amd/csrc/bilinear.hip
+++ b/safe-bayesian-optimization_amd/csrc/bilinear.hip
@@ -1400,6 +1400,8 @@
   pl.ops = GemmOps();
   GemmOps& g = pl.ops;
   pl.encl_ready = false;
+  pl.lrows_ready = false;
+  pl.omap_dirty = true;
   pl.bt_ready = false;
   pl.setup_ms = 0.0;
   const auto t_begin = std::chrono::steady_clock::now();
diff --git a/safe-bayesian-optimization_amd/csrc/bilinear_post.inc.hpp b/safe-bayesian-optimization_amd/csrc/bilinear_post.inc.hpp
--- a/safe-bayesian-optimization_amd/csrc/bilinear_post.inc.hpp
+++ b/safe-bayesian-optimization_amd/csrc/bilinear_post.inc.hpp
@@ -504,9 +504,10 @@
 #endif
 
 __global__ __launch_bounds__(128) void k_bl_enclose(const double* __restrict__ mean, const double* __restrict__ var, long long cnt0,
-                                                    double* __restrict__ encl) {
+                                                    double* __restrict__ encl, const double* __restrict__ lrow1 , double* __restrict__ lrec ) {
   const int cell = threadIdx.x, cr = cell >> 4, cc = cell & 15;
   const size_t tile = (size_t)blockIdx.y * gridDim.x + blockIdx.x;
+  if (cell == 0 && lrec) lrec[tile] = lrow1[tile];
   const size_t base = ((size_t)blockIdx.y * 64 + (size_t)cr * 8) * (size_t)cnt0 + (size_t)blockIdx.x * 128 + (size_t)cc * 8;
   double mlo = 1e308, mhi = -1e308, vlo = 1e308, vhi = -1e308;
   bool fin = true;
@@ -530,7 +531,9 @@
                                                          uint8_t* __restrict__ skip, unsigned int* __restrict__ list, int cap, unsigned long long* __restrict__ Sw,
                                                          unsigned long long* __restrict__ Uw, unsigned long long* __restrict__ Usum,
                                                          unsigned long long* __restrict__ slots, double* __restrict__ Lpart,
-                                                         unsigned long long* __restrict__ cpart, int pcap, int skip_safe ) {
+                                                         unsigned long long* __restrict__ cpart, int pcap, int skip_safe ,
+                                                         const double* __restrict__ lrec ,
+                                                         int count_res ) {
   __shared__ unsigned long long sh_key[kSchedWaves];
   __shared__ unsigned int sh_cnt[kSchedWaves];
   __shared__ unsigned long long sh_vmin[kSchedWaves], sh_rmax[kSchedWaves];
@@ -570,10 +573,10 @@
       run3 = !(t1 + slack[3] < G1 * (1.0 - 1e-12));
       gfold = fmax(fabs(cg0 * t0), fabs(cg1 * t1));
     }
-    const bool grad = run2 || run3;
+    const bool grad = !lrec && (run2 || run3);
     const unsigned int k = dec ? (grad ? 2u : 0u) : (sdec ? (grad ? 5u : 4u) : (grad ? 1u : 3u));
     if (lane == 0) skip[tile] = dec ? kSkipUnsafe : (sdec ? kSkipSafe : 0);
-    my_cnt = k == 0u ? 3u : (k == 2u ? 2u : (k == 4u ? 12u : (k == 5u ? 8u : 0u)));
+    my_cnt = k == 0u ? 3u : (k == 2u ? 2u : (k == 4u ? 12u : (k == 5u ? 8u : ((k == 3u && count_res) ? 16u : 0u))));
     if (k != 0u && k != 4u) {
       if (lane == 0) {
         const unsigned int sh = ((unsigned int)tile + 3u * ((unsigned int)tile >> kTlistShift)) & (kTlistShards - 1);
@@ -597,7 +600,7 @@
         Sw[w0 + h * 64 + lane] = ~0ull;
         Uw[w0 + h * 64 + lane] = 0ull;
       }
-      const double lrow = fmax(0.0, gfold);
+      const double lrow = lrec ? lrec[tile] : fmax(0.0, gfold);
       my_key = (unsigned long long)__double_as_longlong(lrow);
       my_vmin = kv < 1e300 ? ord_key(kv) : ~0ull;
       my_rmax = ku >= 0.0 ? ord_key(ku) : 0ull;
@@ -622,7 +625,7 @@
         Uw[w0 + h * 64 + lane] = ~0ull;
         atomicOr(&Usum[(size_t)bx * 128 + h * 64 + lane], 1ull << by);
       }
-      const double lrow = fmax(0.0, gfold);
+      const double lrow = lrec ? lrec[tile] : fmax(0.0, gfold);
       my_key = (unsigned long long)__double_as_longlong(lrow);
       if (lane == 0) Lpart[((size_t)tgy + by) * tgx + bx] = lrow;
       if (lane < kFuseRow) {
@@ -636,8 +639,8 @@
   }
   if (lane == 0) { sh_key[wave] = my_key; sh_cnt[wave] = my_cnt; sh_vmin[wave] = my_vmin; sh_rmax[wave] = my_rmax; }
   __syncthreads();
-  if (threadIdx.x < 7) {
-    unsigned long long key = 0ull, n0 = 0ull, nskip = 0ull, n4 = 0ull, nsafe = 0ull, vmin = ~0ull, rmax = 0ull;
+  if (threadIdx.x < 8) {
+    unsigned long long key = 0ull, n0 = 0ull, nskip = 0ull, n4 = 0ull, nsafe = 0ull, nres = 0ull, vmin = ~0ull, rmax = 0ull;
 #pragma unroll
     for (int w = 0; w < kSchedWaves; ++w) {
       key = sh_key[w] > key ? sh_key[w] : key;
@@ -645,6 +648,7 @@
       nskip += (sh_cnt[w] >> 1) & 1u;
       n4 += (sh_cnt[w] >> 2) & 1u;
       nsafe += (sh_cnt[w] >> 3) & 1u;
+      nres += (sh_cnt[w] >> 4) & 1u;
       vmin = sh_vmin[w] < vmin ? sh_vmin[w] : vmin;
       rmax = sh_rmax[w] > rmax ? sh_rmax[w] : rmax;
     }
@@ -656,6 +660,7 @@
     if (threadIdx.x == 4 && nsafe) atomicAdd(&slots[(size_t)kSlotSkipSafe * kColSlots + slot], nsafe);
     if (threadIdx.x == 5 && vmin != ~0ull) atomicMin(&slots[(size_t)kSlotVmin1 * kColSlots + slot], vmin);
     if (threadIdx.x == 6 && rmax != 0ull) atomicMax(&slots[(size_t)kSlotRmax1 * kColSlots + slot], rmax);
+    if (threadIdx.x == 7 && nres) atomicAdd(&slots[(size_t)kSlotResC * kColSlots + slot], nres);
   }
 }
 
@@ -686,7 +691,9 @@
 }
 
 __global__ __launch_bounds__(1024) void k_bl_sched_list2(unsigned long long* __restrict__ cpart, int pcap, int ntiles, unsigned int* __restrict__ list,
-                                                         double* __restrict__ Lpart0, unsigned int* __restrict__ head1) {
+                                                         double* __restrict__ Lpart0, unsigned int* __restrict__ head1,
+                                                         const uint8_t* __restrict__ omap ,
+                                                         unsigned long long* __restrict__ slots) {
   __shared__ unsigned int sh[3 * 16];
   const int t = threadIdx.x;
   const unsigned long long* nS = cpart + (size_t)1 * pcap;
@@ -694,10 +701,10 @@
   unsigned int base[3] = {0u, 0u, 0u};
   for (int r = 0; r * 1024 < ntiles; ++r) {
     const int i = r * 1024 + t;
-    const bool in = i < ntiles, has = in && nS[i] != 0ull;
-    const unsigned int p = sched_rank3(has ? 0 : -1, base, sh);
+    const bool in = i < ntiles, has = in && nS[i] != 0ull, res = has && omap && omap[i] != 0;
+    const unsigned int p = sched_rank3(has ? (res ? 1 : 0) : -1, base, sh);
     if (has) {
-      list[kTlistHead + p] = (unsigned int)i;
+      list[kTlistHead + (res ? (unsigned int)(ntiles - 1) - p : p)] = (unsigned int)i;
     } else if (in) {
       Lpart0[i] = 0.0;
 #pragma unroll
@@ -707,7 +714,8 @@
   }
   if (t == 0) {
     list[0] = base[0];
-    list[1] = 0u;
+    list[1] = base[1];
+    if (base[1]) atomicAdd(&slots[(size_t)kSlotResO * kColSlots], (unsigned long long)base[1]);
   }
   if (t < kTlistShards) head1[t * kTlistHead] = head1[t * kTlistHead + 1] = 0u;
 }
@@ -733,10 +741,10 @@
   unsigned int ent = 0u;
   if (listed) {
     const unsigned int sh = blockIdx.x & ((1u << px.tshift) - 1u), at = blockIdx.x >> px.tshift;
-    const unsigned int nfront = px.tlist[sh * kTlistHead], nback = px.tlist[sh * kTlistHead + 1];
+    const unsigned int nfront = px.tlist[sh * kTlistHead], nback = px.front_only ? 0u : px.tlist[sh * kTlistHead + 1];
     if (at >= nfront + nback) {
 #ifdef SBO_PHASE_CLOCKS
-      if (threadIdx.x == 0) { const unsigned long long t_ = wall_clock64(); wg_trace_row(o, t_, t_, t_, 0xffffffu, 3u); }
+      if (threadIdx.x == 0 && !px.front_only) { const unsigned long long t_ = wall_clock64(); wg_trace_row(o, t_, t_, t_, 0xffffffu, 3u); }
 #endif
       return;
     }
@@ -854,6 +862,7 @@
     }
   }
   const bool skip_tile = (ROLE == 2 && obits && tile_nS == 0ull && px.lean >= 2) || cskip || csafe;
+  if (ROLE == 2 && obits && px.omap != nullptr && !cx.skip_store && cx.tid == 0) px.omap[ctile] = 1;
   if (!skip_tile)
     post_phase<0, RB, ROLE>(cx, BtA + (size_t)o * sBtA, P0f + (size_t)o * sP0f, KB0, eff ? eff[4 * o * es] : KS0, vo, sf2, ystd * ystd, 0.0, gmax, acc, xn0, pre,
                             VAo, SBo, KBm);
@@ -932,6 +941,123 @@
   return 0;
 }
 #endif
+
+template <int ROLE>
+__global__ __launch_bounds__(256) void k_bres(const CandSpec cs, const double* __restrict__ mean, const double* __restrict__ var,
+                                              double* __restrict__ Lpart, double bconf, unsigned long long* __restrict__ cpart, int pcap,
+                                              const GuardBand* __restrict__ gb, const double* __restrict__ lrec, const PostExtra px) {
+  __shared__ double sh[4 * 6];
+  __shared__ unsigned int bits[4 * 128];
+  const int o = px.o0;
+  const unsigned int shd = blockIdx.x & ((1u << px.tshift) - 1u), at = blockIdx.x >> px.tshift;
+  const unsigned int nfront = ROLE == 2 ? 0u : px.tlist[shd * kTlistHead], nback = px.tlist[shd * kTlistHead + 1];
+#ifdef SBO_PHASE_CLOCKS
+  const unsigned long long clk_in_ = wall_clock64();
+  unsigned long long clk_ld_ = clk_in_;
+#endif
+  if (at >= nfront + nback) {
+#ifdef SBO_PHASE_CLOCKS
+    if (threadIdx.x == 0) wg_trace_row(o, clk_in_, clk_in_, clk_in_, 0xffffffu, 3u);
+#endif
+    return;
+  }
+  const unsigned int ent = px.tlist[(kTlistHead << px.tshift) + shd * (unsigned int)px.tcap + (at < nfront ? at : (unsigned int)px.tcap - 1u - (at - nfront))];
+  const unsigned int tgx = (unsigned int)px.tgx, tgy = (unsigned int)px.tgy;
+  const unsigned int bx = (ent & 0xffffffu) % tgx, by = (ent & 0xffffffu) / tgx;
+  const size_t ctile = (size_t)by * tgx + bx, ntile = (size_t)tgx * tgy;
+  PostCtx cx;
+  cx.lds = sh;
+  cx.tid = threadIdx.x; cx.lane = cx.tid & 63; cx.wave = cx.tid >> 6;
+  cx.rb0 = by * 4; cx.cs0 = bx * 8;
+  cx.ucnt0 = (unsigned int)cs.count[0];
+  cx.var_rd = nullptr; cx.S = nullptr; cx.U = nullptr;
+  cx.bconf = bconf;
+  cx.bb = bconf * bconf;
+  cx.cS = cx.cU = cx.cB = 0;
+  cx.rmax = -1.0;
+  cx.role = ROLE;
+  cx.lds_bits = bits;
+  cx.umin = 1e300;
+  cx.xmin = 1e300;
+  cx.vminS = 1e300;
+  cx.skip_store = true;
+#pragma unroll
+  for (int s2 = 0; s2 < 8; ++s2) cx.bw[s2] = 0u;
+  cx.gb_on = ROLE == 1 && gb != nullptr;
+  cx.lband = cx.gb_on ? lcb_band(cx.bb, gb->dm[1], gb->dv[1]) : LcbBand{0.0, 0.0};
+  const unsigned int col_in = cx.lane & 15, row_in = cx.lane >> 4;
+  const double* const mo = mean + (size_t)o * cs.n_local;
+  const double* const vo = var + (size_t)o * cs.n_local;
+  double mv[4][8], vr[4][8];
+#pragma unroll
+  for (int t = 0; t < 4; ++t) {
+    const unsigned int line = (unsigned int)(cx.rb0 + cx.wave) * 16u + 4u * t + row_in;
+    const size_t g0 = (size_t)line * cx.ucnt0 + (unsigned int)cx.cs0 * 16u + col_in;
+#pragma unroll
+    for (int s2 = 0; s2 < 8; ++s2) {
+      mv[t][s2] = mo[g0 + s2 * 16];
+      vr[t][s2] = vo[g0 + s2 * 16];
+    }
+  }
+  if (ROLE == 2) {
+#pragma unroll
+    for (int s2 = 0; s2 < 8; ++s2) {
+      const unsigned long long w = px.cb.Sw[(size_t)by * cx.ucnt0 + (unsigned int)(cx.cs0 + s2) * 16u + col_in];
+      cx.bw[s2] = (unsigned int)(w >> (16 * cx.wave + (int)row_in)) & 0x1111u;
+    }
+  }
+#ifdef SBO_PHASE_CLOCKS
+  {
+    double sum_ = 0.0;
+#pragma unroll
+    for (int t = 0; t < 4; ++t)
+#pragma unroll
+      for (int s2 = 0; s2 < 8; ++s2) sum_ += mv[t][s2] + vr[t][s2];
+    if (__syncthreads_or(sum_ == 0x1p-1070 ? 1 : 0) == 0) clk_ld_ = wall_clock64();
+  }
+#endif
+#pragma unroll
+  for (int t = 0; t < 4; ++t) {
+    if (ROLE == 1) {
+      post_classify_row(cx, 4u * t + row_in, mv[t], vr[t]);
+    } else {
+#pragma unroll
+      for (int s2 = 0; s2 < 8; ++s2) post_objective(cx, ((cx.bw[s2] >> (4 * t)) & 1u) != 0u, mv[t][s2], vr[t][s2]);
+    }
+  }
+  if (ROLE == 1) {
+#pragma unroll
+    for (int s2 = 0; s2 < 8; ++s2) { cx.cS += __popc(cx.bw[s2] & 0xffffu); cx.cU += __popc(cx.bw[s2] >> 16); }
+#pragma unroll
+    for (int s2 = 0; s2 < 8; ++s2) {
+      unsigned int w = cx.bw[s2];
+      w |= (unsigned int)__shfl_xor((int)w, 16);
+      w |= (unsigned int)__shfl_xor((int)w, 32);
+      if (cx.lane < 16) bits[cx.wave * 128 + s2 * 16 + cx.lane] = w;
+    }
+  }
+  const double gmax = ROLE == 1 ? lrec[ctile] : 0.0;
+  post_partials<4>(sh, cx.lane, cx.wave, gmax, ROLE == 1, cx.cS, cx.cU, ROLE == 2 ? -cx.umin : cx.rmax, cx.cB, cx.vminS,
+                   Lpart + ((size_t)o * tgy + by) * tgx + bx, cpart + (ROLE == 2 ? ntile : (size_t)0) + ctile, pcap, ROLE == 2, px.cb.slots,
+                   (int)(ctile & (kColSlots - 1)), o, ROLE == 1 ? (int)by : -1, (int)bx, cx.xmin, false);
+  if (ROLE == 1 && cx.tid < 128) {
+    unsigned long long sw = 0ull, uw = 0ull;
+#pragma unroll
+    for (int w = 0; w < 4; ++w) {
+      const unsigned int pc = bits[w * 128 + cx.tid];
+      sw |= (unsigned long long)(pc & 0xffffu) << (16 * w);
+      uw |= (unsigned long long)(pc >> 16) << (16 * w);
+    }
+    const size_t col = (size_t)cx.cs0 * 16u + cx.tid;
+    px.cb.Sw[(size_t)by * cx.ucnt0 + col] = sw;
+    px.cb.Uw[(size_t)by * cx.ucnt0 + col] = uw;
+    if (uw != 0ull) atomicOr(&px.cb.Usum[col], 1ull << by);
+  }
+#ifdef SBO_PHASE_CLOCKS
+  __syncthreads();
+  if (threadIdx.x == 0) wg_trace_row(o, clk_in_, clk_ld_, wall_clock64(), (unsigned int)ctile, 4u);
+#endif
+}
 
 
 __global__ __launch_bounds__(256, 3) void k_bgrad(const ModelConst mc, const CandSpec cs, const double* __restrict__ VA, size_t sVA,
@@ -1038,6 +1164,10 @@
   PostExtra px;
   double* encl = nullptr;
   bool record_encl = false;
+  double* lrec = nullptr;
+  uint8_t* omap = nullptr;
+  bool res_rows = false;
+  bool res_c = false, res_o = false;
   unsigned int *sched_l1 = nullptr, *sched_l2 = nullptr;
   int sched_cap1 = 0;
   const GuardBand* gb_fused = nullptr;
@@ -1149,6 +1279,33 @@
   return SBO_OK;
 }
 
+static int col_resident(GemmLaunch& L) {
+  sbo_ctx* c = L.c;
+  const size_t rbytes = sizeof(double) * L.ntiles;
+  const void* was = c->bl_res.p;
+  if (int rc = ensure(c->bl_res, rbytes + L.ntiles)) return rc;
+  if (c->bl_res.p != was) {
+    c->bl.lrows_ready = false;
+    c->bl.omap_dirty = true;
+  }
+  L.lrec = (double*)c->bl_res.p;
+  if (!c->opt.k1_resident) {
+    c->bl.omap_dirty = true;
+    return SBO_OK;
+  }
+  const bool on = L.sched_l1 != nullptr && L.sched_l2 != nullptr && L.px.encl != nullptr;
+  L.res_rows = on && c->bl.lrows_ready;
+  L.res_c = L.res_rows && c->bl.vals_ready;
+  L.res_o = on;
+  L.omap = (uint8_t*)c->bl_res.p + rbytes;
+  if (c->bl.omap_dirty) {
+    SBO_HIP(hipMemsetAsync(L.omap, 0, L.ntiles, c->stream));
+    c->bl.omap_dirty = false;
+  }
+  L.px.omap = L.omap;
+  return SBO_OK;
+}
+
 static int gemm_grad_deferred(GemmLaunch& L) {
   sbo_ctx* c = L.c;
   const GemmOps& g = L.g;
@@ -1180,14 +1337,15 @@
   if (L.sched_l1 && part == 0 && px.encl) {
     hipLaunchKernelGGL(k_bl_sched_tiles1, dim3((L.gx * L.gy + kSchedWaves - 1) / kSchedWaves), dim3(64 * kSchedWaves), 0, c->stream, c->mc, (const double*)px.encl, (int)(L.gx * L.gy), (int)L.gx,
                        (int)L.gy, (unsigned int)L.cnt0, L.req.fuse_b, L.gb_fused, g.gtmax, g.gkey, q, px.skip, L.sched_l1, L.sched_cap1, px.cb.Sw, px.cb.Uw,
-                       px.cb.Usum, px.cb.slots, L.lrows, rows.base, rows.cap, px.skip_safe);
+                       px.cb.Usum, px.cb.slots, L.lrows, rows.base, rows.cap, px.skip_safe, L.res_rows ? (const double*)L.lrec : (const double*)nullptr,
+                       L.res_c ? 1 : 0);
     px.tlist = L.sched_l1;
     px.tshift = kTlistShift;
     px.tcap = L.sched_cap1;
   }
   if (L.sched_l2 && part == 1) {
     hipLaunchKernelGGL(k_bl_sched_list2, dim3(1), dim3(1024), 0, c->stream, rows.base, rows.cap, (int)(L.gx * L.gy), L.sched_l2,
-                       L.lrows, L.sched_l1);
+                       L.lrows, L.sched_l1, L.res_o ? (const uint8_t*)L.omap : (const uint8_t*)nullptr, px.cb.slots);
     px.tlist = L.sched_l2;
     px.tshift = 0;
     px.tcap = (int)(L.gx * L.gy);
@@ -1196,17 +1354,31 @@
   px.tgx = (int)L.gx;
   px.tgy = (int)L.gy;
   const dim3 grid = px.tlist ? dim3((unsigned)px.tcap << px.tshift) : dim3(L.gx, L.gy, (unsigned)(colw ? 1 : q));
-  hipExtLaunchKernelGGL(kpost, grid, dim3(256), L.lds, c->stream, nullptr,
-                        (L.req.lmax_defer && last) ? c->ev[1] : ((colw && part == 0) ? c->col.ev[0] : nullptr), 0,
-                        c->mc, cs, g.BtA, g.sBtA, g.P0f, g.sP0f, g.VA, g.sVA, g.SBf, g.sSBf, g.KB0, g.KS0, g.KBm, g.KSm, g.KBm2, g.nrb, g.ncs0,
-                        L.nlines, (double*)c->mean.p, (double*)c->var.p, L.defer ? L.lrows + (size_t)L.rows_out * q : L.lrows,
-                        (const double*)c->bl_small.p , fuse ? (uint8_t*)(q > 2 ? c->fuseS.p : c->maskS.p) : (uint8_t*)nullptr,
-                        fuse ? (uint8_t*)(q > 2 ? c->fuseU.p : c->maskU.p) : (uint8_t*)nullptr, L.req.fuse_b, (unsigned long long*)c->cpart.p,
-                        c->cpart_cap, L.gb_fused, (const int*)g.eff, g.gtmax, g.gkey, g.imode, px);
+  px.front_only = 0;
+  const bool light_c = L.res_c && part == 0 && px.tlist != nullptr, light_o = L.res_o && part == 1 && px.tlist != nullptr;
+  if (light_c) {
+    hipExtLaunchKernelGGL(k_bres<1>, grid, dim3(256), 0, c->stream, nullptr, c->col.ev[0], 0, cs, (const double*)c->mean.p, (const double*)c->var.p,
+                          L.lrows, L.req.fuse_b, (unsigned long long*)c->cpart.p, c->cpart_cap, L.gb_fused, (const double*)L.lrec, px);
+  }
+  if (light_o) {
+    hipLaunchKernelGGL(k_bres<2>, grid, dim3(256), 0, c->stream, cs, (const double*)c->mean.p, (const double*)c->var.p, L.lrows, L.req.fuse_b,
+                       (unsigned long long*)c->cpart.p, c->cpart_cap, (const GuardBand*)nullptr, (const double*)nullptr, px);
+    px.front_only = 1;
+  }
+  if (!light_c) {
+    hipExtLaunchKernelGGL(kpost, grid, dim3(256), L.lds, c->stream, nullptr,
+                          (L.req.lmax_defer && last) ? c->ev[1] : ((colw && part == 0) ? c->col.ev[0] : nullptr), 0,
+                          c->mc, cs, g.BtA, g.sBtA, g.P0f, g.sP0f, g.VA, g.sVA, g.SBf, g.sSBf, g.KB0, g.KS0, g.KBm, g.KSm, g.KBm2, g.nrb, g.ncs0,
+                          L.nlines, (double*)c->mean.p, (double*)c->var.p, L.defer ? L.lrows + (size_t)L.rows_out * q : L.lrows,
+                          (const double*)c->bl_small.p , fuse ? (uint8_t*)(q > 2 ? c->fuseS.p : c->maskS.p) : (uint8_t*)nullptr,
+                          fuse ? (uint8_t*)(q > 2 ? c->fuseU.p : c->maskU.p) : (uint8_t*)nullptr, L.req.fuse_b, (unsigned long long*)c->cpart.p,
+                          c->cpart_cap, L.gb_fused, (const int*)g.eff, g.gtmax, g.gkey, g.imode, px);
+  }
   if (colw && part == 0 && L.record_encl) {
     hipLaunchKernelGGL(k_bl_enclose, dim3(L.gx, L.gy), dim3(128), 0, c->stream, (const double*)c->mean.p + (size_t)cs.n_local,
-                       (const double*)c->var.p + (size_t)cs.n_local, L.cnt0, L.encl);
+                       (const double*)c->var.p + (size_t)cs.n_local, L.cnt0, L.encl, (const double*)L.lrows + L.ntiles, L.lrec);
     c->bl.encl_ready = true;
+    c->bl.lrows_ready = L.lrec != nullptr;
   }
   if (colw && part == 0 && !L.interp && c->bl.encl_ready && !px.encl) c->bl.vals_ready = true;
 }
@@ -1222,12 +1394,14 @@
   }
   const double s1 = L.run_stage1 ? 1.0 : 0.0;
   c->last_k1_flops = (double)q * 2.0 * 1024.0 * (s1 * 4.0 * (double)g.nrb * g.KB0 * g.KB1 + tiles2 * (g.KS0 + 3 * g.KSm));
+  for (int o = 0; o < 2; ++o) c->last_k1_tile_flops[o] = 32.0 * 2.0 * 1024.0 * (g.KS0 + 3 * g.KSm);
   const int* he = c->h_back->tile_eff;
   double f = 0.0;
   for (int o = 0; o < q; ++o) {
     const int ks = he[4 * o], kb0 = he[4 * o + 1], kb1 = he[4 * o + 2];
     if (ks < 1 || ks > g.KS0 || kb0 < 1 || kb0 > g.KB0 || kb1 < 1 || kb1 > g.KB1) return;
     f += 2.0 * 1024.0 * (s1 * 4.0 * (double)g.nrb * kb0 * kb1 + tiles2 * (ks + (g.gtmax ? 1 : 3) * g.KSm));
+    if (o < 2) c->last_k1_tile_flops[o] = 32.0 * 2.0 * 1024.0 * (ks + (g.gtmax ? 1 : 3) * g.KSm);
   }
   c->last_k1_flops = f;
 }
@@ -1254,6 +1428,7 @@
     L.fuse = false;
     if (!interp && (rc = col_enclosures(L))) return rc;
     if ((rc = col_tile_lists(L))) return rc;
+    if (!interp && (rc = col_resident(L))) return rc;
   }
   if (!interp && !L.colw) post_regions_written(c);
   if (interp) gemm_stage1(L);
diff --git a/safe-bayesian-optimization_amd/csrc/internal.hpp b/safe-bayesian-optimization_amd/csrc/internal.hpp
--- a/safe-bayesian-optimization_amd/csrc/internal.hpp
+++ b/safe-bayesian-optimization_amd/csrc/internal.hpp
@@ -152,7 +152,9 @@
                     kSlotRmax1 , kSlotL0, kSlotL1 ,
                     kSlotRowMask ,
                     kSlotSkip ,
-                    kSlotSkipSafe , kColSlotFields };
+                    kSlotSkipSafe ,
+                    kSlotResC, kSlotResO ,
+                    kColSlotFields };
 __host__ __device__ inline bool col_slot_is_min(int f) { return f == kSlotUmin || f == kSlotVmin0 || f == kSlotVmin1; }
 constexpr unsigned int kTlistUnsafe = 0x80000000u, kTlistSafe = 0x40000000u;
 constexpr unsigned char kSkipUnsafe = 1, kSkipSafe = 2;
@@ -170,6 +172,8 @@
   const unsigned int* tlist;
   int tshift, tcap;
   int tgx, tgy;
+  int front_only;
+  uint8_t* omap;
 };
 
 struct GemmOps {
@@ -197,6 +201,8 @@
   GemmOps ops;
   bool encl_ready = false;
   bool vals_ready = false;
+  bool lrows_ready = false;
+  bool omap_dirty = true;
   bool bt_ready = false;
 };
 
@@ -408,6 +414,7 @@
     int lipschitz_lds = 1;
     int list_index = -1;
     int k1_sched = 1;
+    int k1_resident = 1;
     int k1_skip_safe = 1;
     int comm_events = 0;
     int col_path = 1;
@@ -463,6 +470,7 @@
   sbo::DevBuf bl_grad;
   sbo::DevBuf bl_lpart;
   sbo::DevBuf bl_encl;
+  sbo::DevBuf bl_res;
   sbo::ResetBuf bl_sched;
   sbo::Pinned h_stage;
   struct K1AuditRecord {
@@ -487,6 +495,7 @@
   bool posterior_valid = false;
   bool post_l0_missing = false;
   int last_k1 = 0;
+  double last_k1_tile_flops[2] = {0.0, 0.0};
   double last_k1_flops = 0.0;
   unsigned long long* Lmax = nullptr;
   sbo::DevBuf maskS, maskU, maskM, maskG, maskO;
@@ -629,8 +638,8 @@
 int guard_probe_gradients(sbo_ctx* c, hipStream_t st, double* ppts, double* grad_out, const sbo::ModelConst* mcp = nullptr);
 int bilinear_setup(sbo_ctx* c);
 int launch_posterior_gemm(sbo_ctx* c, bool interp, const PostRequest& req, PostOutcome& out);
-inline void post_regions_written(sbo_ctx* c) { c->bl.encl_ready = c->bl.vals_ready = false; }
-inline void post_values_patched(sbo_ctx* c) { c->bl.vals_ready = false; }
+inline void post_regions_written(sbo_ctx* c) { c->bl.encl_ready = c->bl.vals_ready = c->bl.lrows_ready = false; c->bl.omap_dirty = true; }
+inline void post_values_patched(sbo_ctx* c) { c->bl.vals_ready = false; c->bl.omap_dirty = true; }
 inline void plans_invalidate(sbo_ctx* c) {
   c->bl.valid = false;
   c->bi.valid = false;
diff --git a/safe-bayesian-optimization_amd/csrc/posterior.hip b/safe-bayesian-optimization_amd/csrc/posterior.hip
--- a/safe-bayesian-optimization_amd/csrc/posterior.hip
+++ b/safe-bayesian-optimization_amd/csrc/posterior.hip
@@ -865,6 +865,7 @@
   c->gb.active = false;
   c->k1_audit = {};
   const bool encl_kept = c->bl.valid && c->bl.encl_ready, vals_kept = encl_kept && c->bl.vals_ready;
+  const bool lrows_kept = encl_kept && c->bl.lrows_ready, omap_kept = c->bl.valid && !c->bl.omap_dirty;
   post_regions_written(c);
   const double tri_flops = (double)c->mc.q * c->mc.npad * (c->mc.npad + 16.0) * (double)c->cs.n_local;
   const PostTarget t{c->cs, c->mean.p, c->var.p, c->Lmax};
@@ -883,6 +884,8 @@
         c->last_k1 = 4;
         c->bl.encl_ready = encl_kept;
         c->bl.vals_ready = vals_kept;
+        c->bl.lrows_ready = lrows_kept;
+        c->bl.omap_dirty = !omap_kept;
         return launch_posterior_gemm(c, false, req, out);
       }
     }
diff --git a/safe-bayesian-optimization_amd/csrc/sets.hip b/safe-bayesian-optimization_amd/csrc/sets.hip
--- a/safe-bayesian-optimization_amd/csrc/sets.hip
+++ b/safe-bayesian-optimization_amd/csrc/sets.hip
@@ -32,6 +32,7 @@
   long long guard_slot[kArgSlots];
   long long tiles_skipped;
   long long tiles_skipped_safe;
+  long long tiles_resident_c, tiles_resident_o;
   unsigned long long ticket;
   long long n_guard_cls;
   long long guard_nb0;
@@ -1974,6 +1975,10 @@
   c->prof.set_path = colpath ? 1 : 0;
   c->prof.k1_tiles_skipped = colpath ? h.tiles_skipped : 0;
   c->prof.k1_tiles_skipped_safe = colpath ? h.tiles_skipped_safe : 0;
+  c->prof.k1_tiles_resident_c = colpath ? h.tiles_resident_c : 0;
+  c->prof.k1_tiles_resident_o = colpath ? h.tiles_resident_o : 0;
+  if (colpath && !reuse)
+    c->last_k1_flops = std::max(0.0, c->last_k1_flops - (double)h.tiles_resident_c * c->last_k1_tile_flops[1] - (double)h.tiles_resident_o * c->last_k1_tile_flops[0]);
 
   memset(res, 0, sizeof(*res));
   res->count_S = h.count_S;
diff --git a/safe-bayesian-optimization_amd/csrc/sets_colpath.inc.hpp b/safe-bayesian-optimization_amd/csrc/sets_colpath.inc.hpp
--- a/safe-bayesian-optimization_amd/csrc/sets_colpath.inc.hpp
+++ b/safe-bayesian-optimization_amd/csrc/sets_colpath.inc.hpp
@@ -165,7 +165,7 @@
 
 __device__ __forceinline__ unsigned long long col_slot_reduce(const unsigned long long* __restrict__ slots, int field) {
   unsigned long long v = slots[(size_t)field * kColSlots + (threadIdx.x & 63)];
-  const bool is_min = col_slot_is_min(field), is_sum = field == kSlotS || field == kSlotU || field == kSlotB || field == kSlotSkip || field == kSlotSkipSafe;
+  const bool is_min = col_slot_is_min(field), is_sum = field == kSlotS || field == kSlotU || field == kSlotB || field == kSlotSkip || field == kSlotSkipSafe || field == kSlotResC || field == kSlotResO;
 #pragma unroll
   for (int o = 32; o > 0; o >>= 1) {
     const unsigned long long y = __shfl_xor(v, o);
@@ -181,11 +181,12 @@
   if (threadIdx.x < 64) {
     const unsigned long long cS = col_slot_reduce(slots, kSlotS), cU = col_slot_reduce(slots, kSlotU), cB = col_slot_reduce(slots, kSlotB);
     const unsigned long long vmin = col_slot_reduce(slots, kSlotVmin1), rmax = col_slot_reduce(slots, kSlotRmax1), l1 = col_slot_reduce(slots, kSlotL1);
-    const unsigned long long nskip = col_slot_reduce(slots, kSlotSkip), nsafe = col_slot_reduce(slots, kSlotSkipSafe);
+    const unsigned long long nskip = col_slot_reduce(slots, kSlotSkip), nsafe = col_slot_reduce(slots, kSlotSkipSafe), nresc = col_slot_reduce(slots, kSlotResC);
     if (threadIdx.x == 0) {
       Lmax[1] = l1;
       sc->tiles_skipped = (long long)nskip;
       sc->tiles_skipped_safe = (long long)nsafe;
+      sc->tiles_resident_c = (long long)nresc;
       sc->ustar_key = ~0ull;
       sc->count_S = (long long)cS;
       sc->count_U = (long long)cU;
@@ -207,6 +208,7 @@
 struct ColScal2 {
   unsigned long long ustar_key, vmin0_key;
   double gb_du0;
+  unsigned long long res_o;
 };
 __device__ __forceinline__ void col_merge2_body(const unsigned long long* __restrict__ slots, unsigned long long& ustar_key,
                                                 unsigned long long& vmin0_key) {
@@ -357,9 +359,9 @@
     du0 = j.gb->dm[0] + (any ? j.b * gb_dsqrt(vm, j.gb->dv[0]) : 0.0);
   }
   if (blockIdx.x == 0 && threadIdx.x < 64) {
-    const unsigned long long l0 = PART == 1 ? col_slot_reduce(j.slots, kSlotL0) : 0ull;
+    const unsigned long long l0 = PART == 1 ? col_slot_reduce(j.slots, kSlotL0) : col_slot_reduce(j.slots, kSlotResO);
     if (threadIdx.x == 0) {
-      if (PART == 0) { j.sc2->ustar_key = ukey; j.sc2->vmin0_key = vkey; j.sc2->gb_du0 = du0; }
+      if (PART == 0) { j.sc2->ustar_key = ukey; j.sc2->vmin0_key = vkey; j.sc2->gb_du0 = du0; j.sc2->res_o = l0; }
       else j.Lmax[0] = l0;
     }
   }
@@ -851,6 +853,7 @@
       hm->count_M = sc->count_M;
       sc->ustar_key = sc2->ustar_key;
       hm->ustar_key = sc2->ustar_key;
+      hm->tiles_resident_o = (long long)sc2->res_o;
       for (int t = 2; t < kArgSlots; ++t) hm->guard_slot[t] = 0;
     } else {
       hm->count_set[slot - 1] = sc->count_set[slot - 1];
@@ -862,6 +865,7 @@
       hm->n_guard = sc->n_guard;
       hm->tiles_skipped = sc->tiles_skipped;
       hm->tiles_skipped_safe = sc->tiles_skipped_safe;
+      hm->tiles_resident_c = sc->tiles_resident_c;
       for (int t = 0; t < kMaxQ; ++t) {
         hm->rmax_key[t] = sc->rmax_key[t];
         reinterpret_cast<unsigned long long*>(mirror + offsetof(PinnedBack, lip_keys))[t] = Lkeys[t];
```
